# DanMcGann/loam

Measured on AMD Instinct MI355X. Metric: scan-pair registrations/sec (64x1024 Ouster), higher is better.
Workload: dtype f64; 1 GPU; batch of 1024 independent 64x1024 scan pairs per GPU (BASELINE configs[2]/[3]); step = extractFeatures x2 + registerFeatures per pair, inputs resident in HBM; pairs_per_gpu=1024, scan=64x1024, seed=20240311, input_scalar=f64, arithmetic=f64 (float input is widened on load)

## Files before the change

loam_amd/csrc/loamx_api.hip:

```cpp
#include <math.h>
#include <stdio.h>
#include <stdlib.h>
#include <string.h>

#include <mutex>
#include <utility>
#include <string>
#include <vector>

#include <dlfcn.h>
#include <rccl/rccl.h>

#include "loamx_internal.h"
#include "synth.h"

using namespace loamx;

namespace {

enum WsId {
  WS_XYZ = 0, WS_CURV, WS_MASK, WS_EDGE_STAGE, WS_PLANAR_STAGE, WS_EDGE_CNT, WS_PLANAR_CNT,
  WS_EDGE_IDX, WS_PLANAR_IDX, WS_N_EDGE, WS_N_PLANAR, WS_EDGE_XYZ, WS_PLANAR_XYZ,
  WS_GRID_DESC_E, WS_GRID_DESC_P, WS_CELLS_E, WS_CELLS_P, WS_SORTED_E, WS_SORTED_P, WS_REL_E, WS_REL_P,
  WS_SGRID_DESC_E, WS_SGRID_DESC_P, WS_SCELLS_E, WS_SCELLS_P, WS_SSORTED_E, WS_SSORTED_P, WS_SORT_SCRATCH, WS_SORT_SCRATCH_SRC, WS_ASSOC_E, WS_ASSOC_P, WS_NN_E, WS_NN_P, WS_RNN_E, WS_RNN_P, WS_NEAREST_E, WS_NEAREST_P, WS_REST_E, WS_REST_P, WS_EXACT_E, WS_EXACT_P, WS_NASSOC, WS_STATE, WS_PARTIALS, WS_MOM_PARTIALS, WS_MOMENTS, WS_FLAGGED_LIST, WS_FLAGGED_COUNT, WS_LINE_TOT, WS_EXTRACT_EVENTS, WS_BOX, WS_FINITE_FLAG,
  WS_COUNTERS, WS_ITERINFO, WS_STREAM_IN0, WS_STREAM_IN1, WS_STREAM_RES, WS_DUMP_E, WS_DUMP_P, WS_FIT_IN, WS_FIT_OUT, WS_SRC_E, WS_SRC_P, WS_TGT_E, WS_TGT_P, WS_FCOUNTS, WS_RESULTS, WS_INIT, WS_STREAM_INIT,
  WS_COUNT
};

struct Buf {
  void* p = nullptr;
  size_t cap = 0;
};

struct PendingEvent {
  int kernel;
  hipEvent_t e0, e1;
  double bytes;
  bool own_e0;
};

}

struct loamx_ctx {
  int device = 0;
  hipStream_t own_stream = nullptr, stream = nullptr;
  bool max_counts_clean = false;
  hipStream_t aux_stream = nullptr;
  hipEvent_t ev_fork = nullptr, ev_mid = nullptr, ev_join = nullptr;
  hipEvent_t ev_counts = nullptr;
  hipStream_t aux2_stream = nullptr;
  hipEvent_t ev_join2 = nullptr;
  std::string last_error;
  Buf ws[WS_COUNT];
  uint32_t* h_pinned = nullptr;
  bool timing = false;
  std::vector<PendingEvent> pending;
  std::vector<hipEvent_t> event_pool;
  hipEvent_t tail_event = nullptr;
  bool tail_fresh = false;
  loamx_kernel_stat stats[LOAMX_K_COUNT] = {};

  uint32_t extract_flags = 0;
  uint32_t reg_flags = 0;
  int map_cells_log2 = 0;
  int stream_chunk_pairs = 0;
  hipStream_t copy_stream = nullptr;
  hipEvent_t ev_up[2] = {nullptr, nullptr}, ev_free[2] = {nullptr, nullptr};

  uint32_t last_extract_route = 0;

  unsigned long long sweep_slots_base[2] = {0, 0};
  unsigned long long features_base = 0;
  std::mutex mu;
};

struct loamx_target_index {
  GridDesc* desc[2] = {nullptr, nullptr};
  uint32_t* cells[2] = {nullptr, nullptr};
  GridPoint* sorted[2] = {nullptr, nullptr};
  float* rel[2] = {nullptr, nullptr};
  double* pts[2] = {nullptr, nullptr};
  size_t n[2] = {0, 0};
  size_t cap[2] = {0, 0};
  double radius[2] = {0, 0};
  uint32_t* counts = nullptr;
  void* scratch = nullptr;
  uint32_t cells_cap[2] = {0, 0};
  size_t cells_alloc[2] = {0, 0}, scratch_alloc = 0;
  GridPoint* sorted2[2] = {nullptr, nullptr};
  float* rel2[2] = {nullptr, nullptr};
  size_t n_at_build[2] = {0, 0};
  bool grid_valid[2] = {false, false};
  uint64_t full_builds = 0, merges = 0;
};

namespace loamx {
thread_local LaunchScope* g_launch_scope = nullptr;
int g_debug_sync = getenv("LOAMX_DEBUG_SYNC") ? 1 : 0;
thread_local uint32_t g_extract_route = 0;
}

namespace {

const char* kKernelNames[LOAMX_K_COUNT] = {"curvature_valid_kernel", "select_kernel", "compact_kernel",
                                           "grid_build_kernel",      "associate_kernel", "sweep_kernel",
                                           "lm_kernels",             "moment_kernel",    "knn_plane_kernel",
                                           "extract_fused_kernel"};

struct OptionName {
  const char* name;
  bool extract;
  uint32_t bit;
};
const OptionName kOptionNames[] = {
    {"FORCE_TIE_REPLAY", true, kFlagForceReplay}, {"FORCE_SCAN_GIVEUP", true, kFlagForceGiveUp}, {"CURV_V1", true, kFlagCurvV1},
    {"NO_FUSED_COMPACT", true, kFlagNoFusedCompact}, {"NO_MIS_SELECT", true, kFlagNoMisSelect}, {"FUSED_EXTRACT", true, kFlagFusedExtract},
    {"NO_ROW_SELECT", true, kFlagNoRowSelect}, {"FUSED_ROWS", true, kFlagFusedRows}, {"NO_SPLIT_CURV", true, kFlagNoSplitCurv}, {"STAGE_ALWAYS", true, kFlagStageAlways},
    {"NO_MOMENTS", false, kRegFlagNoMoments}, {"NO_PACKED_GRID", false, kRegFlagNoPackedGrid}, {"NO_BIG_GRID", false, kRegFlagNoBigGrid},
    {"NO_GRID_SIDE", false, kRegFlagNoGridSide}, {"DEBUG_POISON", false, kRegFlagPoison},
    {"QUEUE_TWO_STAGE", false, kRegFlagQueueTwoStage}, {"QUEUE_ONE_STAGE", false, kRegFlagQueueOneStage},
    {"NO_MIXED_ASSOC", false, kRegFlagNoMixedAssoc}, {"FORCE_RCCL", false, kRegFlagForceRccl},
    {"NO_COOP_LEFT", false, kRegFlagNoCoopLeft}, {"NO_REF_MOMENTS", false, kRegFlagNoRefMoments},
    {"NO_EXTRACT_BOXES", false, kRegFlagNoExtractBoxes}, {"CHECK_FINITE", false, kRegFlagCheckFinite},
    {"NO_SMALL_SETS", false, kRegFlagNoSmallSets}};

int fail(loamx_ctx* ctx, int code, const std::string& msg) {
  if (ctx) ctx->last_error = msg;
  return code;
}

#define HIP_TRY(ctx, expr)                                                                          \
  do {                                                                                              \
    hipError_t e_ = (expr);                                                                         \
    if (e_ != hipSuccess)                                                                           \
      return fail(ctx, LOAMX_ERR_HIP, std::string(#expr) + ": " + hipGetErrorString(e_));           \
  } while (0)

int ensure(loamx_ctx* ctx, int id, size_t bytes) {
  Buf& b = ctx->ws[id];
  if (bytes == 0) bytes = 8;
  if (b.cap >= bytes) return LOAMX_OK;
  if (b.p) {
    HIP_TRY(ctx, hipStreamSynchronize(ctx->stream));
    HIP_TRY(ctx, hipFree(b.p));
    b.p = nullptr, b.cap = 0;
  }
  HIP_TRY(ctx, hipMalloc(&b.p, bytes));
  b.cap = bytes;
  return LOAMX_OK;
}
#define ENSURE(ctx, id, bytes)                       \
  do {                                               \
    int rc_ = ensure(ctx, id, bytes);                \
    if (rc_ != LOAMX_OK) return rc_;                 \
  } while (0)

const char* const kNonFiniteMsg = "non-finite coordinate in the input (the reference's behaviour is undefined there)";
bool host_all_finite(const void* p, bool f32, size_t n_scalars) {
  if (!p) return true;
  if (f32) {
    const float* v = static_cast<const float*>(p);
    float acc = 0.0f;
    for (size_t i = 0; i < n_scalars; i++) acc += v[i] * 0.0f;
    return acc == 0.0f;
  }
  const double* v = static_cast<const double*>(p);
  double acc = 0.0;
  for (size_t i = 0; i < n_scalars; i++) acc += v[i] * 0.0;
  return acc == 0.0;
}
template <typename T>
T* wsp(loamx_ctx* ctx, int id) {
  return reinterpret_cast<T*>(ctx->ws[id].p);
}

hipEvent_t take_event(loamx_ctx* ctx) {
  if (!ctx->event_pool.empty()) {
    hipEvent_t e = ctx->event_pool.back();
    ctx->event_pool.pop_back();
    return e;
  }
  hipEvent_t e = nullptr;
  (void)hipEventCreate(&e);
  return e;
}

struct TimedScope {
  loamx_ctx* ctx;
  PendingEvent pe;
  bool on, attach;
  LaunchScope ls;
  TimedScope(loamx_ctx* c, int kernel, double bytes, bool attach_ = false) : ctx(c), on(c->timing), attach(attach_) {
    if (on) {
      pe.kernel = kernel, pe.bytes = bytes;
      if (attach) {
        pe.own_e0 = true;
        pe.e0 = take_event(ctx), pe.e1 = take_event(ctx);
        ls = LaunchScope{pe.e0, pe.e1, true};
        g_launch_scope = &ls;
        return;
      }
      pe.own_e0 = !(ctx->tail_fresh && ctx->tail_event);
      pe.e0 = pe.own_e0 ? take_event(ctx) : ctx->tail_event;
      pe.e1 = take_event(ctx);
      if (pe.own_e0) (void)hipEventRecord(pe.e0, ctx->stream);
    }
  }
  ~TimedScope() {
    if (on) {
      if (attach) {
        g_launch_scope = nullptr;
        if (ls.first) {
          ctx->event_pool.push_back(pe.e0), ctx->event_pool.push_back(pe.e1);
        } else {
          ctx->pending.push_back(pe);
        }
        ctx->tail_fresh = false;
        return;
      }
      (void)hipEventRecord(pe.e1, ctx->stream);
      ctx->pending.push_back(pe);
      ctx->tail_event = pe.e1, ctx->tail_fresh = true;
    }
  }
};
inline void untimed(loamx_ctx* ctx) { ctx->tail_fresh = false; }

int finite_begin(loamx_ctx* ctx) {
  ENSURE(ctx, WS_FINITE_FLAG, 16);
  untimed(ctx);
  HIP_TRY(ctx, hipMemsetAsync(ctx->ws[WS_FINITE_FLAG].p, 0, 16, ctx->stream));
  return LOAMX_OK;
}
void finite_add(loamx_ctx* ctx, const void* d_pts, bool f32, const uint32_t* d_n, size_t n_sets, size_t stride, uint32_t pitch) {
  if (d_pts && n_sets && stride) launch_check_finite(d_pts, f32, d_n, n_sets, stride, pitch, static_cast<uint32_t*>(ctx->ws[WS_FINITE_FLAG].p), ctx->stream);
}
int finite_end(loamx_ctx* ctx) {
  uint32_t bad = 0;
  HIP_TRY(ctx, hipMemcpyAsync(&bad, ctx->ws[WS_FINITE_FLAG].p, 4, hipMemcpyDeviceToHost, ctx->stream));
  HIP_TRY(ctx, hipStreamSynchronize(ctx->stream));
  return bad ? fail(ctx, LOAMX_ERR_BAD_PARAM, kNonFiniteMsg) : LOAMX_OK;
}
int dev_check_finite(loamx_ctx* ctx, const void* d_pts, bool f32, const uint32_t* d_n, size_t n_sets, size_t stride, uint32_t pitch, bool force = false) {
  if ((!force && !(ctx->reg_flags & kRegFlagCheckFinite)) || !d_pts || n_sets == 0 || stride == 0) return LOAMX_OK;
  int rc = finite_begin(ctx);
  if (rc != LOAMX_OK) return rc;
  finite_add(ctx, d_pts, f32, d_n, n_sets, stride, pitch);
  return finite_end(ctx);
}


int check_launch(loamx_ctx* ctx, const char* what) {
  hipError_t e = hipGetLastError();
  if (e != hipSuccess) return fail(ctx, LOAMX_ERR_HIP, std::string(what) + ": " + hipGetErrorString(e));
  return LOAMX_OK;
}
#define CHECK_LAUNCH(ctx, what)                      \
  do {                                               \
    int rc_ = check_launch(ctx, what);               \
    if (rc_ != LOAMX_OK) return rc_;                 \
  } while (0)

int make_extract_params(loamx_ctx* ctx, const loamx_lidar_params* lidar, const loamx_fe_params* fe, ExtractParams& P) {
  if (!lidar || !fe) return fail(ctx, LOAMX_ERR_BAD_PARAM, "null parameter struct");
  if (fe->number_sectors == 0) return fail(ctx, LOAMX_ERR_BAD_PARAM, "number_sectors must be >= 1");
  if (fe->neighbor_points == 0)
    return fail(ctx, LOAMX_ERR_BAD_PARAM, "neighbor_points must be >= 1 (the reference reads point idx-1)");
  if (fe->neighbor_points > (uint64_t)kMaxNeighborPoints)
    return fail(ctx, LOAMX_ERR_UNSUPPORTED, "neighbor_points > 16 not supported by the kernels");
  if (lidar->points_per_line > (uint64_t)kMaxLineWidth)
    return fail(ctx, LOAMX_ERR_UNSUPPORTED, "points_per_line > 4096 not supported by the kernels");
  if (lidar->scan_lines * lidar->points_per_line > 0xFFFFFFFFull / 4)
// ... 131 lines not shown
  if (launch_extract_split_ok(P, n_scans)) Pk.flags |= kFlagSplitCurv, g_extract_route |= LOAMX_ROUTE_SPLIT_CURV;
  const bool split = (Pk.flags & kFlagSplitCurv) != 0u;
  {
    TimedScope t(ctx, LOAMX_K_CURVATURE, (double)n_scans * (double)N * ((f32 ? 21.0 : 33.0) - (split ? 1.0 : 0.0)), true);
    launch_curvature_valid(d_xyz, f32, n_scans, Pk, wsp<double>(ctx, WS_CURV), wsp<uint8_t>(ctx, WS_MASK), ctx->stream);
  }
  CHECK_LAUNCH(ctx, "curvature_valid_kernel");
  bool fused = false, rows_ran = false;
  {
    TimedScope t(ctx, LOAMX_K_SELECT, (double)n_scans * (double)N * (split ? 4.0 : 9.0), true);
    fused = launch_select(wsp<double>(ctx, WS_CURV), wsp<uint8_t>(ctx, WS_MASK), n_scans, Pk, st, &fz, ctx->stream, &rows_ran);
    launch_replay(wsp<double>(ctx, WS_CURV), wsp<uint8_t>(ctx, WS_MASK), n_scans, Pk, st, fz, ctx->stream);
    if (fused) {
      launch_compact(d_xyz, f32, n_scans, P, st, d_edge_idx, d_n_edge, d_edge_xyz, edge_capacity(P), d_planar_idx, d_n_planar,
                     d_planar_xyz, planar_capacity(P), ctx->stream, d_gave_up, d_events + 1);
      g_extract_route |= LOAMX_ROUTE_FUSED_COMPACT;
    }
  }
  CHECK_LAUNCH(ctx, "select_kernel");
  if (split && !rows_ran) return fail(ctx, LOAMX_ERR_UNSUPPORTED, "internal: split curvature form without the row selection");
  if (fused && rows_ran && boxes && fz.box_min)
    boxes->min = fz.box_min, boxes->max = fz.box_max, boxes->bad = d_gave_up, g_extract_route |= LOAMX_ROUTE_BOXES;
  if (fused) return LOAMX_OK;
  {
    TimedScope t(ctx, LOAMX_K_COMPACT, 0.0, true);
    launch_compact(d_xyz, f32, n_scans, P, st, d_edge_idx, d_n_edge, d_edge_xyz, edge_capacity(P), d_planar_idx,
                   d_n_planar, d_planar_xyz, planar_capacity(P), ctx->stream);
    g_extract_route |= LOAMX_ROUTE_COMPACT;
  }
  CHECK_LAUNCH(ctx, "compact_kernel");
  return LOAMX_OK;
}

struct RegInputs {
  size_t n_pairs, edge_stride, planar_stride;
  uint32_t in_pitch;
  const double *src_edge, *src_planar, *tgt_edge, *tgt_planar;
  const uint32_t *n_src_edge, *n_src_planar, *n_tgt_edge, *n_tgt_planar;
  const double* init;
  ExtractBoxes boxes;
  uint32_t src_box_offset;
};

typedef int (*AfterAssocHook)(loamx_ctx*, const RegBatch&, uint32_t it, void* user);

int enqueue_association(loamx_ctx* ctx, const RegBatch& B, const RegConfig& C, uint32_t what = kAssocEdges | kAssocPlanes) {
  hipStream_t s = ctx->stream;
    {
      TimedScope t(ctx, LOAMX_K_ASSOC, 0.0);
      const bool side = (size_t)B.n_pairs * B.assoc_blocks_plane >= 128;
      PendingEvent knn{};
      LaunchScope knn_ls{nullptr, nullptr, true};
      if (ctx->timing) {
        knn.kernel = LOAMX_K_KNN_PLANE, knn.bytes = 0.0, knn.own_e0 = true;
        knn.e0 = take_event(ctx), knn.e1 = take_event(ctx);
        knn_ls = LaunchScope{knn.e0, knn.e1, true};
      }
      launch_associate(B, C, s, side ? ctx->aux_stream : nullptr, side ? ctx->aux2_stream : nullptr, ctx->ev_fork, ctx->ev_mid, ctx->ev_join,
                       ctx->ev_join2, ctx->timing ? &knn_ls : nullptr, what);
      if (ctx->timing) {
        if (knn_ls.first) ctx->event_pool.push_back(knn.e0), ctx->event_pool.push_back(knn.e1);
        else ctx->pending.push_back(knn);
      }
    }
    CHECK_LAUNCH(ctx, "associate_kernel");
  return LOAMX_OK;
}

int enqueue_icf_iteration(loamx_ctx* ctx, const RegBatch& B, const RegConfig& C, uint32_t it, AfterAssocHook hook, void* hook_user) {
  hipStream_t s = ctx->stream;
    {
      const int rc_assoc = enqueue_association(ctx, B, C);
      if (rc_assoc != LOAMX_OK) return rc_assoc;
    }
#ifdef LOAMX_NN_SAME_STATS
    debug_nn_same(B, it, s);
#endif
    if (hook) {
      untimed(ctx);
      int rc = hook(ctx, B, it, hook_user);
      if (rc != LOAMX_OK) return rc;
    }
    {
      TimedScope t(ctx, LOAMX_K_LM, 0.0, true);
      launch_lm_begin(B, C, s);
    }
    const bool ref_first = it == 0 && B.ref_moments != 0u;
    if (ref_first) {
      {
        TimedScope t(ctx, LOAMX_K_SWEEP, 0.0, true);
        launch_sweep(B, s);
      }
      TimedScope t(ctx, LOAMX_K_LM, 0.0, true);
      launch_lm_step(B, s);
    }
    if (it > 0 || ref_first) {
      TimedScope t(ctx, LOAMX_K_MOMENT, 0.0, true);
      launch_moments(B, s);
    }
    if (it > 0 || ref_first) {
      TimedScope t(ctx, LOAMX_K_LM, 0.0, true);
      launch_lm_pair_loop(B, C, s);
    } else {
      for (int k = 0; k < 5; k++) {
        {
          TimedScope t(ctx, LOAMX_K_SWEEP, 0.0, true);
          launch_sweep(B, s);
        }
        {
          TimedScope t(ctx, LOAMX_K_LM, 0.0, true);
          launch_lm_step(B, s);
        }
      }
    }
    CHECK_LAUNCH(ctx, "sweep/lm kernels");
    if (it == 0 && !ref_first) {
      TimedScope t(ctx, LOAMX_K_LM, 0.0, true);
      launch_outer_update(B, C, s);
    }
    CHECK_LAUNCH(ctx, "outer_update_kernel");
  return LOAMX_OK;
}

int register_dev(loamx_ctx* ctx, const RegInputs& in, const RegConfig& C_in, loamx_reg_result* d_results, bool want_iter_info,
                 AfterAssocHook hook, void* hook_user, const loamx_target_index* prebuilt = nullptr, const loamx_assoc_dump* dump = nullptr,
                 size_t dump_n_se = 0, size_t dump_n_sp = 0) {
  if (in.n_pairs == 0) return LOAMX_OK;
  RegConfig C = C_in;
  if (dump && C.max_iterations == 0) C.max_iterations = 1;
  untimed(ctx);
  if (in.n_pairs > 0x7FFFFFFFull / 128) return fail(ctx, LOAMX_ERR_UNSUPPORTED, "too many pairs in one call");
  const size_t np = in.n_pairs, es = in.edge_stride ? in.edge_stride : 1, ps = in.planar_stride ? in.planar_stride : 1;
  if (es > 0x3FFFFFFFull || ps > 0x3FFFFFFFull) return fail(ctx, LOAMX_ERR_UNSUPPORTED, "feature set too large");
  RegBatch B{};
  B.n_pairs = np, B.edge_stride = es, B.planar_stride = ps, B.in_pitch = in.in_pitch;
  B.src_edge = in.src_edge, B.n_src_edge = in.n_src_edge, B.src_planar = in.src_planar, B.n_src_planar = in.n_src_planar;
  B.tgt_edge = in.tgt_edge, B.n_tgt_edge = in.n_tgt_edge, B.tgt_planar = in.tgt_planar, B.n_tgt_planar = in.n_tgt_planar;
  B.init = in.init;
  if (!(C.flags & kRegFlagNoExtractBoxes)) B.box_min = in.boxes.min, B.box_max = in.boxes.max, B.box_bad = in.boxes.bad, B.src_box_offset = in.src_box_offset;
  ENSURE(ctx, WS_GRID_DESC_E, np * sizeof(GridDesc));
  ENSURE(ctx, WS_GRID_DESC_P, np * sizeof(GridDesc));
  ENSURE(ctx, WS_CELLS_E, (np * (size_t)(kGridCellsCap + 1) + 4) * sizeof(uint32_t));
  ENSURE(ctx, WS_CELLS_P, (np * (size_t)(kGridCellsCap + 1) + 4) * sizeof(uint32_t));
  ENSURE(ctx, WS_SORTED_E, np * (es + kGridPad) * sizeof(GridPoint));
  ENSURE(ctx, WS_SORTED_P, np * (ps + kGridPad) * sizeof(GridPoint));
  ENSURE(ctx, WS_REL_E, np * 3 * (es + kGridPad) * sizeof(float));
  ENSURE(ctx, WS_REL_P, np * 3 * (ps + kGridPad) * sizeof(float));
  ENSURE(ctx, WS_SGRID_DESC_E, np * sizeof(GridDesc));
  ENSURE(ctx, WS_SGRID_DESC_P, np * sizeof(GridDesc));
  ENSURE(ctx, WS_SCELLS_E, np * (size_t)(kGridCellsCap + 1) * sizeof(uint32_t));
  ENSURE(ctx, WS_SCELLS_P, np * (size_t)(kGridCellsCap + 1) * sizeof(uint32_t));
  ENSURE(ctx, WS_SSORTED_E, np * es * sizeof(GridPoint));
  ENSURE(ctx, WS_SSORTED_P, np * ps * sizeof(GridPoint));
  ENSURE(ctx, WS_SORT_SCRATCH, np * (es > ps ? es : ps) * sizeof(GridPoint));
  ENSURE(ctx, WS_SORT_SCRATCH_SRC, grid_small(es > ps ? es : ps, C.flags) ? sizeof(GridPoint) : np * (es > ps ? es : ps) * sizeof(GridPoint));
  ENSURE(ctx, WS_ASSOC_E, 9 * np * es * sizeof(double));
  ENSURE(ctx, WS_ASSOC_P, 7 * np * ps * sizeof(double));
  const size_t km_e = C.k_edge <= 5 ? 5 : (C.k_edge <= 8 ? 8 : kMaxK), km_p = C.k_plane <= 5 ? 5 : (C.k_plane <= 8 ? 8 : kMaxK);
  ENSURE(ctx, WS_NN_E, (1 + km_e) * np * es * sizeof(uint32_t));
  ENSURE(ctx, WS_NN_P, (1 + km_p) * np * ps * sizeof(uint32_t));
  ENSURE(ctx, WS_RNN_E, (1 + km_e) * np * es * sizeof(uint32_t));
  ENSURE(ctx, WS_RNN_P, (1 + km_p) * np * ps * sizeof(uint32_t));
  ENSURE(ctx, WS_NEAREST_E, np * es * sizeof(uint32_t));
  ENSURE(ctx, WS_NEAREST_P, np * ps * sizeof(uint32_t));
  ENSURE(ctx, WS_REST_E, np * es * sizeof(uint32_t));
  ENSURE(ctx, WS_REST_P, np * ps * sizeof(uint32_t));
  ENSURE(ctx, WS_EXACT_E, np * es * sizeof(uint32_t));
  ENSURE(ctx, WS_EXACT_P, np * ps * sizeof(uint32_t));
  ENSURE(ctx, WS_NASSOC, np * 8 * sizeof(uint32_t));
  ENSURE(ctx, WS_STATE, np * sizeof(PairState));
  B.blocks_per_pair = (uint32_t)((es + ps + kSweepChunk - 1) / kSweepChunk);
  ENSURE(ctx, WS_PARTIALS, np * B.blocks_per_pair * kAccSize * sizeof(double));
  B.mom_blocks_per_pair = (uint32_t)((ps + kSweepChunk - 1) / kSweepChunk);
  ENSURE(ctx, WS_MOM_PARTIALS, np * B.mom_blocks_per_pair * 4 * (size_t)(kMomSize + 2) * sizeof(double));
  ENSURE(ctx, WS_MOMENTS, np * (size_t)(kMomSize + 2) * sizeof(double));
  ENSURE(ctx, WS_FLAGGED_LIST, np * (size_t)B.mom_blocks_per_pair * kSweepChunk * sizeof(uint32_t));
  ENSURE(ctx, WS_FLAGGED_COUNT, np * (size_t)B.mom_blocks_per_pair * 4 * sizeof(uint32_t));
  {
    const bool fresh = ctx->ws[WS_COUNTERS].cap == 0;
    ENSURE(ctx, WS_COUNTERS, 128);
    untimed(ctx);
    if (fresh) HIP_TRY(ctx, hipMemsetAsync(ctx->ws[WS_COUNTERS].p, 0, 128, ctx->stream));
  }
  if (C.flags & kRegFlagPoison) {
    static const int kScratch[] = {WS_GRID_DESC_E, WS_GRID_DESC_P, WS_CELLS_E, WS_CELLS_P, WS_SORTED_E, WS_SORTED_P, WS_REL_E, WS_REL_P,
                                   WS_SGRID_DESC_E, WS_SGRID_DESC_P, WS_SCELLS_E, WS_SCELLS_P, WS_SSORTED_E, WS_SSORTED_P, WS_SORT_SCRATCH, WS_SORT_SCRATCH_SRC,
                                   WS_ASSOC_E, WS_ASSOC_P, WS_NN_E, WS_NN_P, WS_RNN_E, WS_RNN_P, WS_NEAREST_E, WS_NEAREST_P, WS_REST_E,
                                   WS_REST_P, WS_EXACT_E, WS_EXACT_P, WS_NASSOC, WS_STATE, WS_PARTIALS, WS_MOM_PARTIALS, WS_MOMENTS,
                                   WS_FLAGGED_LIST, WS_FLAGGED_COUNT};
    for (int id : kScratch)
      if (ctx->ws[id].p) HIP_TRY(ctx, hipMemsetAsync(ctx->ws[id].p, 0xFF, ctx->ws[id].cap, ctx->stream));
  }
  if (want_iter_info) ENSURE(ctx, WS_ITERINFO, np * (size_t)(C.max_iterations ? C.max_iterations : 1) * sizeof(loamx_iter_info));
  B.grid_edge = GridSet{wsp<GridDesc>(ctx, WS_GRID_DESC_E), wsp<uint32_t>(ctx, WS_CELLS_E), wsp<GridPoint>(ctx, WS_SORTED_E), es + kGridPad,
                        wsp<float>(ctx, WS_REL_E)};
  B.grid_plane = GridSet{wsp<GridDesc>(ctx, WS_GRID_DESC_P), wsp<uint32_t>(ctx, WS_CELLS_P), wsp<GridPoint>(ctx, WS_SORTED_P), ps + kGridPad,
                         wsp<float>(ctx, WS_REL_P)};
  B.src_grid_edge = GridSet{wsp<GridDesc>(ctx, WS_SGRID_DESC_E), wsp<uint32_t>(ctx, WS_SCELLS_E), wsp<GridPoint>(ctx, WS_SSORTED_E), es, nullptr};
  B.src_grid_plane = GridSet{wsp<GridDesc>(ctx, WS_SGRID_DESC_P), wsp<uint32_t>(ctx, WS_SCELLS_P), wsp<GridPoint>(ctx, WS_SSORTED_P), ps, nullptr};
  B.sort_scratch = wsp<GridPoint>(ctx, WS_SORT_SCRATCH);
  B.sort_scratch_src = wsp<GridPoint>(ctx, WS_SORT_SCRATCH_SRC);
  B.assoc = AssocBuffers{wsp<double>(ctx, WS_ASSOC_E), wsp<double>(ctx, WS_ASSOC_P), wsp<uint32_t>(ctx, WS_NN_E),
                         wsp<uint32_t>(ctx, WS_NN_P), wsp<uint32_t>(ctx, WS_RNN_E), wsp<uint32_t>(ctx, WS_RNN_P),
                         wsp<uint32_t>(ctx, WS_NEAREST_E),
                         wsp<uint32_t>(ctx, WS_NEAREST_P), wsp<uint32_t>(ctx, WS_REST_E), wsp<uint32_t>(ctx, WS_REST_P),
                         wsp<uint32_t>(ctx, WS_EXACT_E), wsp<uint32_t>(ctx, WS_EXACT_P),
                         wsp<uint32_t>(ctx, WS_NASSOC)};
  B.state = wsp<PairState>(ctx, WS_STATE);
  B.partials = wsp<double>(ctx, WS_PARTIALS);
  B.mom_partials = wsp<double>(ctx, WS_MOM_PARTIALS);
  B.moments = wsp<double>(ctx, WS_MOMENTS);
  B.flagged_list = wsp<uint32_t>(ctx, WS_FLAGGED_LIST);
  B.flagged_count = wsp<uint32_t>(ctx, WS_FLAGGED_COUNT);
  B.n_active = wsp<uint32_t>(ctx, WS_COUNTERS);
  B.sweep_slots = reinterpret_cast<unsigned long long*>(wsp<unsigned char>(ctx, WS_COUNTERS) + 8);
  B.assoc_slots = B.sweep_slots + 2;
  B.grid_bytes = B.sweep_slots + 5;
  B.iter_info = want_iter_info ? wsp<loamx_iter_info>(ctx, WS_ITERINFO) : nullptr;
  B.want_nearest = hook ? 1u : 0u;
  B.ref_moments = (C.flags & (kRegFlagNoMoments | kRegFlagNoRefMoments)) ? 0u : 1u;
  B.max_counts = wsp<uint32_t>(ctx, WS_COUNTERS) + 16;
  B.assoc_blocks_edge = B.assoc_blocks_plane = 0xFFFFFFFFu;
  B.knn_mode_edge = B.knn_mode_plane = 0u;
  B.small_edge_sets = (C.flags & kRegFlagNoSmallSets) ? 0u : (!prebuilt ? 1u : (prebuilt->n[0] <= kBruteMax ? 2u : 0u));
  hipStream_t s = ctx->stream;
  untimed(ctx);
  if (!ctx->max_counts_clean) {
    const uint32_t init[6] = {0u, 0u, 0u, 0u, 0xFFFFFFFFu, 0xFFFFFFFFu};
    memcpy(&ctx->h_pinned[8], init, sizeof(init));
    HIP_TRY(ctx, hipMemcpyAsync(B.max_counts, &ctx->h_pinned[8], sizeof(init), hipMemcpyHostToDevice, s));
  }
  ctx->max_counts_clean = false;
  launch_state_init(B, C, s);
  CHECK_LAUNCH(ctx, "state_init_kernel");
  if (!ctx->ev_counts) HIP_TRY(ctx, hipEventCreateWithFlags(&ctx->ev_counts, hipEventDisableTiming));
  HIP_TRY(ctx, hipMemcpyAsync(&ctx->h_pinned[16], B.max_counts, 6 * sizeof(uint32_t), hipMemcpyDeviceToHost, s));
  HIP_TRY(ctx, hipEventRecord(ctx->ev_counts, s));

  if (prebuilt) {
    B.grid_edge = GridSet{prebuilt->desc[0], prebuilt->cells[0], prebuilt->sorted[0], prebuilt->cap[0] + kGridPad, prebuilt->rel[0], prebuilt->cells_cap[0]};
    B.grid_plane = GridSet{prebuilt->desc[1], prebuilt->cells[1], prebuilt->sorted[1], prebuilt->cap[1] + kGridPad, prebuilt->rel[1], prebuilt->cells_cap[1]};
  }
  {
    TimedScope t(ctx, LOAMX_K_GRID, 0.0);
    const bool side = !(C.flags & kRegFlagNoGridSide) && ctx->aux_stream && !prebuilt && hipStreamWaitEvent(ctx->aux_stream, ctx->ev_counts, 0) == hipSuccess;
    if (!prebuilt) launch_grid_build_targets(B, C, s);
    launch_grid_build_sources(B, C, side ? ctx->aux_stream : s);
    if (side && hipEventRecord(ctx->ev_join, ctx->aux_stream) == hipSuccess) (void)hipStreamWaitEvent(s, ctx->ev_join, 0);
  }
  CHECK_LAUNCH(ctx, "grid_build_kernel");
  HIP_TRY(ctx, hipEventSynchronize(ctx->ev_counts));
  B.assoc_blocks_edge = (ctx->h_pinned[16] + 255u) / 256u;
  B.assoc_blocks_plane = (ctx->h_pinned[17] + 255u) / 256u;
  {
    uint32_t tmax[2] = {ctx->h_pinned[18], ctx->h_pinned[19]}, tmin[2] = {ctx->h_pinned[20], ctx->h_pinned[21]};
    if (prebuilt) tmax[0] = tmin[0] = (uint32_t)prebuilt->n[0], tmax[1] = tmin[1] = (uint32_t)prebuilt->n[1];
    uint32_t* mode[2] = {&B.knn_mode_edge, &B.knn_mode_plane};
    for (int k = 0; k < 2; k++) *mode[k] = tmin[k] > tmax[k] ? 0u : (tmin[k] > kBruteMax ? 1u : (tmax[k] <= kBruteMax ? 2u : 0u));
  }
  if (dump) {
    if (np != 1) return fail(ctx, LOAMX_ERR_BAD_PARAM, "association dump: one pair at a time");
    int rc_a = enqueue_association(ctx, B, C);
    if (rc_a != LOAMX_OK) return rc_a;
    untimed(ctx);
    const size_t n[2] = {dump_n_se, dump_n_sp}, kq[2] = {(size_t)C.k_edge, (size_t)C.k_plane}, pw[2] = {6, 4};
    AssocDumpSet D[2] = {};
    for (int kind = 0; kind < 2; kind++) {
      const size_t bytes = n[kind] * (24 + 8 * pw[kind] + 4 + 4 * kq[kind] + 1) + 64;
      ENSURE(ctx, kind ? WS_DUMP_P : WS_DUMP_E, bytes);
      unsigned char* base = wsp<unsigned char>(ctx, kind ? WS_DUMP_P : WS_DUMP_E);
      HIP_TRY(ctx, hipMemsetAsync(base, 0, bytes, s));
      D[kind].moved = reinterpret_cast<double*>(base);
      D[kind].prim = D[kind].moved + 3 * n[kind];
      D[kind].nn_count = reinterpret_cast<uint32_t*>(D[kind].prim + pw[kind] * n[kind]);
      D[kind].nn_idx = D[kind].nn_count + n[kind];
      D[kind].valid = reinterpret_cast<uint8_t*>(D[kind].nn_idx + kq[kind] * n[kind]);
      if (n[kind] == 0) D[kind].nn_count = nullptr;
    }
    launch_assoc_dump(B, C, D[0], D[1], s);
    CHECK_LAUNCH(ctx, "assoc_dump_kernel");
    struct Out { void* host; const void* dev; size_t bytes; };
    const Out outs[10] = {
        {dump->edge_nn_count, D[0].nn_count, 4 * n[0]}, {dump->edge_nn_idx, D[0].nn_idx, 4 * kq[0] * n[0]}, {dump->edge_valid, D[0].valid, n[0]},
        {dump->edge_moved, D[0].moved, 24 * n[0]}, {dump->edge_lines, D[0].prim, 48 * n[0]},
        {dump->plane_nn_count, D[1].nn_count, 4 * n[1]}, {dump->plane_nn_idx, D[1].nn_idx, 4 * kq[1] * n[1]}, {dump->plane_valid, D[1].valid, n[1]},
        {dump->plane_moved, D[1].moved, 24 * n[1]}, {dump->plane_planes, D[1].prim, 32 * n[1]}};
    for (const Out& o : outs)
      if (o.host && o.bytes && o.dev) HIP_TRY(ctx, hipMemcpyAsync(o.host, o.dev, o.bytes, hipMemcpyDeviceToHost, s));
    if (dump->queue_lengths) HIP_TRY(ctx, hipMemcpyAsync(dump->queue_lengths, B.assoc.n_assoc + 2, 4 * sizeof(uint32_t), hipMemcpyDeviceToHost, s));
    HIP_TRY(ctx, hipStreamSynchronize(s));
    return LOAMX_OK;
  }
  for (uint32_t it = 0; it < C.max_iterations; it++) {
    {
      const int rc_body = enqueue_icf_iteration(ctx, B, C, it, hook, hook_user);
      if (rc_body != LOAMX_OK) return rc_body;
    }
    if (it + 1 < C.max_iterations && it > (B.n_pairs >= 256 ? 1u : 0u)) {
      untimed(ctx);
      HIP_TRY(ctx, hipMemcpyAsync(ctx->h_pinned, B.n_active, sizeof(uint32_t), hipMemcpyDeviceToHost, s));
      launch_write_results(B, d_results, s);
      CHECK_LAUNCH(ctx, "write_results_kernel");
      HIP_TRY(ctx, hipStreamSynchronize(s));
      if (ctx->h_pinned[0] == 0) {
        ctx->max_counts_clean = true;
        return LOAMX_OK;
      }
    }
  }
  untimed(ctx);
  launch_write_results(B, d_results, s);
  CHECK_LAUNCH(ctx, "write_results_kernel");
  ctx->max_counts_clean = true;
  return LOAMX_OK;
}

int resolve_events(loamx_ctx* ctx) {
  if (ctx->pending.empty()) return LOAMX_OK;
  HIP_TRY(ctx, hipStreamSynchronize(ctx->stream));
  for (PendingEvent& pe : ctx->pending) {
    float ms = 0.f;
    if (hipEventElapsedTime(&ms, pe.e0, pe.e1) == hipSuccess) {
      ctx->stats[pe.kernel].launches++;
      ctx->stats[pe.kernel].total_ms += (double)ms;
      ctx->stats[pe.kernel].algorithmic_bytes += pe.bytes;
    }
    if (pe.own_e0) ctx->event_pool.push_back(pe.e0);
    ctx->event_pool.push_back(pe.e1);
  }
  ctx->pending.clear();
  ctx->tail_fresh = false;
  return LOAMX_OK;
}

}

extern "C" {

void loamx_default_fe_params(loamx_fe_params* p) { *p = loamx_fe_params{3, 6, 10, 50, 100.0, 1.0, 0.5, 1.0}; }
void loamx_default_reg_params(loamx_reg_params* p) {
  *p = loamx_reg_params{5, 1.0, 3, 10.0, 5, 2.0, 4, 0.1, 10, 1e-3, 1e-2, 100};
}

const char* loamx_status_string(int status) {
  switch (status) {
    case LOAMX_OK: return "ok";
    case LOAMX_ERR_SCAN_SIZE: return "LOAM: provided lidar scan size does not match provided lidar parameters";
    case LOAMX_ERR_BAD_PARAM: return "bad parameter";
    case LOAMX_ERR_HIP: return "HIP error";
    case LOAMX_ERR_CAPACITY: return "output capacity too small";
    case LOAMX_ERR_UNSUPPORTED: return "unsupported parameter combination";
    case LOAMX_ERR_NO_DEVICE: return "no usable HIP device";
// ... 1329 lines not shown
```

loam_amd/csrc/loamx_internal.h:

```cpp
#pragma once
#include <hip/hip_runtime.h>
#include <hip/hip_ext.h>
#include <stdint.h>
#include <stdio.h>

#include "../../include/loamx.h"
#include "extract_math.h"
#include "reg_math.h"

namespace loamx {

struct LaunchScope {
  hipEvent_t start, stop;
  bool first;
};
extern thread_local LaunchScope* g_launch_scope;
extern int g_debug_sync;
template <typename F, typename... Args>
inline void launch_kernel_named(const char* name, F kernel, const dim3& grid, const dim3& block, size_t shmem, hipStream_t s, Args... args) {
  LaunchScope* sc = g_launch_scope;
  if (g_debug_sync) fprintf(stderr, "[loamx] launch %s grid %u x %u block %u\n", name, grid.x, grid.y, block.x), fflush(stderr);
  if (sc) {
    hipExtLaunchKernelGGL(kernel, grid, block, (uint32_t)shmem, s, sc->first ? sc->start : nullptr, sc->stop, 0, args...);
    sc->first = false;
  } else {
    hipLaunchKernelGGL(kernel, grid, block, shmem, s, args...);
  }
  if (g_debug_sync) {
    const hipError_t e = hipStreamSynchronize(s);
    fprintf(stderr, "[loamx]   done %s: %s\n", name, hipGetErrorString(e)), fflush(stderr);
  }
}
#define launch_kernel(kernel, ...) launch_kernel_named(#kernel, kernel, __VA_ARGS__)

constexpr int kMaxNeighborPoints = 16;
constexpr int kMaxLineWidth = 4096;

extern thread_local uint32_t g_extract_route;

struct ExtractStage {
  uint32_t* edge_stage;
  uint32_t* planar_stage;
  uint32_t* edge_cnt;
  uint32_t* planar_cnt;
};

struct ExtractFused {
  unsigned long long* line_tot;
  uint32_t fuse;
  const void* xyz;
  uint32_t f32;
  uint32_t* edge_idx;
  uint32_t* n_edge;
  double* edge_xyz;
  size_t edge_stride;
  uint32_t* planar_idx;
  uint32_t* n_planar;
  double* planar_xyz;
  size_t planar_stride;
  uint32_t* error;
  unsigned long long* events;
  unsigned long long* box_min;
  unsigned long long* box_max;
  uint32_t no_stage;
  const uint32_t* only_if;
};
__device__ __forceinline__ unsigned long long dbl_key(double v) {
  const unsigned long long u = (unsigned long long)__double_as_longlong(v);
  return (u >> 63) ? ~u : (u | 0x8000000000000000ull);
}
__device__ __forceinline__ double key_dbl(unsigned long long k) {
  return __longlong_as_double((long long)((k >> 63) ? (k & 0x7FFFFFFFFFFFFFFFull) : ~k));
}

void launch_curvature_valid(const void* d_xyz, bool f32, size_t n_scans, const ExtractParams& P, double* d_curv,
                            uint8_t* d_mask, hipStream_t s);
bool launch_select(const double* d_curv, const uint8_t* d_mask, size_t n_scans, const ExtractParams& P,
                   const ExtractStage& st, const ExtractFused* fz, hipStream_t s, bool* rows_ran = nullptr);
bool launch_select_takes_boxes(const ExtractParams& P);
bool launch_extract_fused(const void* d_xyz, bool f32, size_t n_scans, const ExtractParams& P, const ExtractStage& st,
                          const ExtractFused& fz, double* d_curv, uint8_t* d_mask, hipStream_t s);
bool launch_extract_rows_fused(const void* d_xyz, bool f32, size_t n_scans, const ExtractParams& P, const ExtractStage& st,
                               const ExtractFused& fz, double* d_curv, uint8_t* d_mask, hipStream_t s);
bool launch_extract_split_ok(const ExtractParams& P, size_t n_scans);
void launch_extract_init(unsigned long long* line_tot, size_t n_tot, unsigned long long* box_min, unsigned long long* box_max, size_t n_box,
                         hipStream_t s);
void launch_replay(const double* d_curv, const uint8_t* d_mask, size_t n_scans, const ExtractParams& P, const ExtractStage& st,
                   const ExtractFused& fz, hipStream_t s);
void launch_compact(const void* d_xyz, bool f32, size_t n_scans, const ExtractParams& P, const ExtractStage& st,
                    uint32_t* d_edge_idx, uint32_t* d_n_edge, double* d_edge_xyz, size_t edge_stride,
                    uint32_t* d_planar_idx, uint32_t* d_n_planar, double* d_planar_xyz, size_t planar_stride,
                    hipStream_t s, const uint32_t* only_if = nullptr, unsigned long long* fallback_counter = nullptr);

struct RegConfig {
  int k_edge, k_plane;
  int min_line_pts, min_plane_pts;
  double r_edge, r_plane;
  double pass_edge, pass_plane;
  double min_line_cond, max_avg_plane_dist;
  uint32_t max_iterations;
  double rot_thresh, pos_thresh;
  uint32_t min_associations;
  uint32_t flags;
};
constexpr uint32_t kRegFlagNoMoments = 1u;
constexpr uint32_t kRegFlagNoPackedGrid = 2u;
constexpr uint32_t kRegFlagNoBigGrid = 4u;
constexpr uint32_t kRegFlagNoGridSide = 8u;
constexpr uint32_t kRegFlagPoison = 16u;
constexpr uint32_t kRegFlagQueueTwoStage = 32u;
constexpr uint32_t kRegFlagQueueOneStage = 64u;
constexpr uint32_t kRegFlagForceRccl = 256u;
constexpr uint32_t kRegFlagNoCoopLeft = 512u;
constexpr uint32_t kRegFlagNoRefMoments = 1024u;
constexpr uint32_t kRegFlagNoSmallSets = 8192u;
constexpr uint32_t kRegFlagCheckFinite = 4096u;
constexpr uint32_t kRegFlagNoExtractBoxes = 2048u;
constexpr uint32_t kRegFlagNoMixedAssoc = 128u;

struct GridSet {
  GridDesc* desc;
  uint32_t* cell_start;
  GridPoint* sorted;
  size_t stride;
  float* rel;
  uint32_t cells_cap;
};

struct AssocBuffers {
  double* edge;
  double* plane;
  uint32_t* nn_edge;
  uint32_t* nn_plane;
  uint32_t* rnn_edge;
  uint32_t* rnn_plane;
  uint32_t* nearest_edge;
  uint32_t* nearest_plane;
  uint32_t* rest_edge;
  uint32_t* rest_plane;
  uint32_t* exact_edge;
  uint32_t* exact_plane;
  uint32_t* n_assoc;
};

struct PairState {
  double est[7];
  LmState lm;
  uint32_t active;
  uint32_t termination;
  uint32_t iterations;
  uint32_t first_sweep;
  uint32_t stream_planes;
  uint32_t use_moments;
  uint32_t mom_ref_on;
  double mom_ref[7];
};

constexpr int kSweepThreads = 256;
#ifndef LOAMX_SWEEP_ITEMS
#define LOAMX_SWEEP_ITEMS 16
#endif
constexpr int kSweepItems = LOAMX_SWEEP_ITEMS;
constexpr int kSweepChunk = kSweepThreads * kSweepItems;

struct RegBatch {
  size_t n_pairs;
  size_t edge_stride, planar_stride;
  uint32_t in_pitch;
  const double* src_edge;
  const uint32_t* n_src_edge;
  const double* src_planar;
  const uint32_t* n_src_planar;
  const double* tgt_edge;
  const uint32_t* n_tgt_edge;
  const double* tgt_planar;
  const uint32_t* n_tgt_planar;
  const double* init;
  GridSet grid_edge, grid_plane;
  GridSet src_grid_edge, src_grid_plane;
  GridPoint* sort_scratch;
  GridPoint* sort_scratch_src;
  AssocBuffers assoc;
  PairState* state;
  double* partials;
  double* mom_partials;
  double* moments;
  uint32_t mom_blocks_per_pair;
  uint32_t* flagged_list;
  uint32_t* flagged_count;
  uint32_t blocks_per_pair;
  uint32_t* n_active;
  unsigned long long* sweep_slots;
  unsigned long long* assoc_slots;
  unsigned long long* grid_bytes;
  loamx_iter_info* iter_info;
  uint32_t* max_counts;
  uint32_t knn_mode_edge, knn_mode_plane;
  uint32_t assoc_blocks_edge, assoc_blocks_plane;
  uint32_t want_nearest;
  uint32_t ref_moments;
  const unsigned long long* box_min;
  const unsigned long long* box_max;
  const uint32_t* box_bad;
  uint32_t src_box_offset;
  uint32_t small_edge_sets;
};

constexpr size_t kGridBigScratchBytes = 64 + ((size_t)kGridCellsCap + kGridCellsCap / 4096 + 8) * sizeof(uint32_t);
constexpr uint32_t kGridSmallCap = 20480;
constexpr uint32_t kBruteMax = 512;
constexpr uint32_t kGridMapCellsCap = 1u << 18;
inline bool grid_small(size_t stride, uint32_t reg_flags) { return stride <= kGridSmallCap && !(reg_flags & kRegFlagNoPackedGrid); }
void launch_grid_build_targets(const RegBatch& B, const RegConfig& C, hipStream_t s);
void launch_grid_build_sources(const RegBatch& B, const RegConfig& C, hipStream_t s);
void launch_grid_build_target(const RegBatch& B, const RegConfig& C, bool plane, hipStream_t s);
void launch_grid_build_source(const RegBatch& B, const RegConfig& C, bool plane, hipStream_t s);
void launch_state_init(const RegBatch& B, const RegConfig& C, hipStream_t s);
constexpr uint32_t kAssocEdges = 1u, kAssocPlanes = 2u;
void launch_associate(const RegBatch& B, const RegConfig& C, hipStream_t s, hipStream_t aux, hipStream_t aux2, hipEvent_t ev_fork,
                      hipEvent_t ev_mid, hipEvent_t ev_join, hipEvent_t ev_join2, LaunchScope* knn_scope = nullptr,
                      uint32_t what = kAssocEdges | kAssocPlanes);
#ifdef LOAMX_NN_SAME_STATS
void debug_nn_same(const RegBatch& B, uint32_t it, hipStream_t s);
#endif
void launch_lm_begin(const RegBatch& B, const RegConfig& C, hipStream_t s);
void launch_sweep(const RegBatch& B, hipStream_t s);
void launch_lm_pair_loop(const RegBatch& B, const RegConfig& C, hipStream_t s);
void launch_lm_step(const RegBatch& B, hipStream_t s);
void launch_moments(const RegBatch& B, hipStream_t s);
void launch_outer_update(const RegBatch& B, const RegConfig& C, hipStream_t s);
void launch_write_results(const RegBatch& B, loamx_reg_result* d_results, hipStream_t s);

size_t index_insert_ws_bytes(size_t cells, size_t n_add);
void launch_index_insert_count(const GridSet& gs, size_t cells, const double* d_add, uint32_t n_add, void* ws, hipStream_t s);
void launch_index_insert_merge(const GridSet& gs, size_t cells, uint32_t n_old, const double* d_add, uint32_t n_add, void* ws,
                               GridPoint* sorted2, float* rel2, hipStream_t s);

constexpr int kFitMaxK = 32;
struct AssocDumpSet {
  uint32_t* nn_count;
  uint32_t* nn_idx;
  uint8_t* valid;
  double* moved;
  double* prim;
};
void launch_fit_sets(bool plane, const double* d_pts, size_t n_sets, int k, double* d_prim, double* d_aux, hipStream_t s);
void launch_knn_queries(const GridSet& gs, const double* d_q, size_t n_q, int k, double max_dist, uint32_t* d_idx, uint32_t* d_count,
                        hipStream_t s);
void launch_assoc_dump(const RegBatch& B, const RegConfig& C, const AssocDumpSet& edge, const AssocDumpSet& plane, hipStream_t s);

void launch_check_finite(const void* d_pts, bool f32, const uint32_t* d_n, size_t n_sets, size_t stride, uint32_t pitch, uint32_t* d_flag,
                         hipStream_t s);
void launch_check_finite_scalars(const double* d_v, size_t n_scalars, uint32_t* d_flag, hipStream_t s);

void launch_deskew(const void* d_xyz, void* d_out, bool f32, size_t n_scans, uint32_t H, uint32_t W, const double* d_motion, double rho,
                   hipStream_t s);
void launch_trajectory(const loamx_reg_result* d_results, size_t n_pairs, const double origin[7], double* d_world_T_scan, hipStream_t s);

void launch_synth_pairs(uint64_t seed, uint64_t first_pair, size_t n_pairs, uint32_t H, uint32_t W, double sigma,
                        double* d_xyz, hipStream_t s);

}
```

loam_amd/csrc/register_kernels.hip:

```cpp
#include "loamx_internal.h"

namespace loamx {

namespace {

__device__ __forceinline__ double wave_min(double v) {
#pragma unroll
  for (int off = 32; off >= 1; off >>= 1) v = fmin(v, __shfl_xor(v, off));
  return v;
}
__device__ __forceinline__ double wave_max(double v) {
#pragma unroll
  for (int off = 32; off >= 1; off >>= 1) v = fmax(v, __shfl_xor(v, off));
  return v;
}

#ifndef LOAMX_BUILD_THREADS
#define LOAMX_BUILD_THREADS 1024
#endif
constexpr int kBuildThreads = LOAMX_BUILD_THREADS;

template <bool ORDERED, bool PACKED>
__global__ __launch_bounds__(kBuildThreads) void grid_build_kernel(const double* __restrict__ pts_base,
                                                                   const uint32_t* __restrict__ n_pts, size_t stride,
// ... 23 lines not shown
  const uint32_t n = n_raw < stride ? n_raw : (uint32_t)stride;
  const double* __restrict__ pts = pts_base + pair * in_pitch * stride * 3;
#ifdef LOAMX_BUILD_PROFILE
  unsigned long long stamp[12];
  int ns = 0;
#define STAMP() do { __syncthreads(); stamp[ns++] = wall_clock64(); } while (0)
#else
#define STAMP() do {} while (0)
#endif
  STAMP();

  const bool have_box = box_min != nullptr && __hip_atomic_load(box_bad, __ATOMIC_RELAXED, __HIP_MEMORY_SCOPE_AGENT) == 0u;
  if (!have_box) {
    double lx = kDblMax, ly = kDblMax, lz = kDblMax, hx = -kDblMax, hy = -kDblMax, hz = -kDblMax;
#pragma unroll 4
    for (uint32_t i = tid; i < n; i += kBuildThreads) {
      const double x = pts[3 * (size_t)i], y = pts[3 * (size_t)i + 1], z = pts[3 * (size_t)i + 2];
      lx = fmin(lx, x), ly = fmin(ly, y), lz = fmin(lz, z);
      hx = fmax(hx, x), hy = fmax(hy, y), hz = fmax(hz, z);
    }
    lx = wave_min(lx), ly = wave_min(ly), lz = wave_min(lz);
    hx = wave_max(hx), hy = wave_max(hy), hz = wave_max(hz);
    if (lane == 0) {
      s_red[0][wave] = lx, s_red[1][wave] = ly, s_red[2][wave] = lz;
      s_red[3][wave] = hx, s_red[4][wave] = hy, s_red[5][wave] = hz;
    }
  }
  STAMP();
  __syncthreads();
  if (tid == 0) {
    double a[6];
    if (have_box) {
      for (int k = 0; k < 3; k++) {
        a[k] = n ? key_dbl(box_min[(pair * in_pitch) * 6 + k]) : kDblMax;
        a[3 + k] = n ? key_dbl(box_max[(pair * in_pitch) * 6 + k]) : -kDblMax;
      }
    } else {
      for (int k = 0; k < 6; k++) {
        a[k] = s_red[k][0];
        for (int w = 1; w < kBuildThreads / 64; w++) a[k] = k < 3 ? fmin(a[k], s_red[k][w]) : fmax(a[k], s_red[k][w]);
      }
    }
    GridDesc g;
    if (ORDERED) grid_choose_morton(g, v3(a[0], a[1], a[2]), v3(a[3], a[4], a[5]), n);
    else grid_choose(g, v3(a[0], a[1], a[2]), v3(a[3], a[4], a[5]), n, max_dist, kGridCellsCap);
    s_g = g;
    gs.desc[pair] = g;
  }
  __syncthreads();
  const GridDesc g = s_g;
  STAMP();
  const uint32_t ncell = (uint32_t)(g.nx * g.ny * g.nz);
  uint32_t* __restrict__ cs = gs.cell_start + pair * (size_t)(kGridCellsCap + 1);
  GridPoint* __restrict__ sp = gs.sorted + pair * gs.stride;
  GridPoint* __restrict__ dst = ORDERED ? scratch + pair * gs.stride : sp;
  uint32_t carry = 0;
  if (PACKED) {
#pragma unroll 4
    for (uint32_t i = tid; i < n; i += kBuildThreads) {
      const Vec3 pt = v3(pts[3 * (size_t)i], pts[3 * (size_t)i + 1], pts[3 * (size_t)i + 2]);
      s_cellof[i] = (uint16_t)(ORDERED ? grid_morton_of_point(g, pt) : grid_cell_of_point(g, pt));
    }
  }
  for (uint32_t c_lo = 0; c_lo < ncell; c_lo += kGridLdsCells) {
    const uint32_t nc = ncell - c_lo < kGridLdsCells ? ncell - c_lo : kGridLdsCells;
    for (uint32_t c = tid; c < (PACKED ? (nc + 1) / 2 : nc); c += kBuildThreads) s_cells[c] = 0;
    __syncthreads();
    if (PACKED) {
      for (uint32_t i = tid; i < n; i += kBuildThreads) {
        const uint32_t cell = (uint32_t)s_cellof[i] - c_lo;
        if (cell < nc) (void)cell_add(cell);
      }
    } else {
#pragma unroll 4
      for (uint32_t i = tid; i < n; i += kBuildThreads) {
        const Vec3 pt = v3(pts[3 * (size_t)i], pts[3 * (size_t)i + 1], pts[3 * (size_t)i + 2]);
        const uint32_t cell = (ORDERED ? grid_morton_of_point(g, pt) : grid_cell_of_point(g, pt)) - c_lo;
        if (cell < nc) (void)cell_add(cell);
      }
    }
    __syncthreads();
    STAMP();
    const uint32_t per = PACKED ? 2u * (((nc + 2 * kBuildThreads - 1) / (2 * kBuildThreads)) | 1u) : ((nc + kBuildThreads - 1) / kBuildThreads) | 1u;
    const uint32_t c0 = tid * per < nc ? tid * per : nc, c1 = c0 + per < nc ? c0 + per : nc;
    uint32_t local = 0;
    if (PACKED) {
      for (uint32_t w = c0 >> 1; c0 < c1 && 2 * w < c1; w++) local += (s_cells[w] & 0xFFFFu) + (s_cells[w] >> 16);
    } else {
      for (uint32_t c = c0; c < c1; c++) local += s_cells[c];
    }
    uint32_t incl = local;
#pragma unroll
    for (int off = 1; off < 64; off <<= 1) {
      const uint32_t t = __shfl_up(incl, off);
      if (lane >= off) incl += t;
    }
    if (lane == 63) s_wave_sum[wave] = incl;
    __syncthreads();
    uint32_t wave_off = carry;
    for (int w = 0; w < wave; w++) wave_off += s_wave_sum[w];
    uint32_t pass_total = 0;
    for (int w = 0; w < kBuildThreads / 64; w++) pass_total += s_wave_sum[w];
    uint32_t run = wave_off + incl - local;
    if (PACKED) {
      for (uint32_t w = c0 >> 1; c0 < c1 && 2 * w < c1; w++) {
        const uint32_t v = s_cells[w], lo = v & 0xFFFFu, hi = v >> 16;
        s_cells[w] = run | ((run + lo) << 16);
        run += lo + hi;
      }
    } else {
      for (uint32_t c = c0; c < c1; c++) {
        const uint32_t cnt = s_cells[c];
        s_cells[c] = run;
        run += cnt;
      }
    }
    __syncthreads();
    STAMP();
    if (!(ORDERED && PACKED) && (ORDERED || n > kBruteMax))
      for (uint32_t c = tid; c < nc; c += kBuildThreads) cs[c_lo + c] = cell_get(c);
    __syncthreads();
    STAMP();
    if (PACKED) {
      for (uint32_t i = tid; i < n; i += kBuildThreads) {
        const uint32_t cell = (uint32_t)s_cellof[i] - c_lo;
        if (cell < nc) s_inv[cell_add(cell)] = (uint16_t)i;
      }
    } else {
#pragma unroll 4
      for (uint32_t i = tid; i < n; i += kBuildThreads) {
        const double x = pts[3 * (size_t)i], y = pts[3 * (size_t)i + 1], z = pts[3 * (size_t)i + 2];
        const uint32_t cell = (ORDERED ? grid_morton_of_point(g, v3(x, y, z)) : grid_cell_of_point(g, v3(x, y, z))) - c_lo;
        if (cell < nc) dst[cell_add(cell)] = GridPoint{x, y, z, i, 0u};
      }
    }
    carry += pass_total;
    __syncthreads();
    STAMP();
  }
  if (tid == 0) cs[ncell] = n;
  if (tid == 0 && bytes)
    atomicAdd(bytes, (unsigned long long)n * (ORDERED ? 56ull : (gs.rel ? 68ull : 56ull)) +
                         ((!(ORDERED && PACKED) && (ORDERED || n > kBruteMax)) ? 4ull * (ncell + 1) : 0ull));
  if (PACKED && ORDERED) {
#pragma unroll 2
    for (uint32_t p = tid; p < n; p += kBuildThreads) {
      const uint32_t i = s_inv[p];
      const uint32_t cell = s_cellof[i];
      const uint32_t b = cell ? cell_get(cell - 1) : 0u, en = cell_get(cell);
      const double x = pts[3 * (size_t)i], y = pts[3 * (size_t)i + 1], z = pts[3 * (size_t)i + 2];
      uint32_t rank = 0;
      for (uint32_t j = b; j < en; j++) rank += s_inv[j] < i ? 1u : 0u;
      sp[b + rank] = GridPoint{x, y, z, i, 0u};
    }
  } else if (PACKED) {
    const uint16_t* order = s_inv;
    STAMP();
    float* __restrict__ rel = gs.rel ? gs.rel + pair * 3 * gs.stride : nullptr;
#pragma unroll 4
    for (uint32_t p = tid; p < n; p += kBuildThreads) {
      const uint32_t i = order[p];
      const double x = pts[3 * (size_t)i], y = pts[3 * (size_t)i + 1], z = pts[3 * (size_t)i + 2];
      sp[p] = GridPoint{x, y, z, i, 0u};
      if (!ORDERED && rel) rel[p] = (float)(x - g.ox), rel[gs.stride + p] = (float)(y - g.oy), rel[2 * gs.stride + p] = (float)(z - g.oz);
    }
    if (!ORDERED && rel && (uint32_t)tid < kGridPad) rel[n + tid] = kRelPad, rel[gs.stride + n + tid] = kRelPad, rel[2 * gs.stride + n + tid] = kRelPad;
  } else if (!ORDERED && gs.rel) {
    __syncthreads();
    __threadfence_block();
    float* __restrict__ rel = gs.rel + pair * 3 * gs.stride;
    for (uint32_t p = tid; p < n; p += kBuildThreads) {
      const GridPoint e = sp[p];
      rel[p] = (float)(e.x - g.ox), rel[gs.stride + p] = (float)(e.y - g.oy), rel[2 * gs.stride + p] = (float)(e.z - g.oz);
    }
    if ((uint32_t)tid < kGridPad) rel[n + tid] = kRelPad, rel[gs.stride + n + tid] = kRelPad, rel[2 * gs.stride + n + tid] = kRelPad;
  }
#ifdef LOAMX_BUILD_PROFILE
  STAMP();
  if (tid == 0 && pair == 700 && n > 2000 && ns >= 8)
    printf("build ORDERED=%d n=%u ncell=%u ns=%d: bbox %llu choice %llu count %llu scan %llu table %llu scatter %llu rank %llu out %llu (x10 ns)\n", (int)ORDERED, n, ncell, ns,
           stamp[1] - stamp[0], stamp[2] - stamp[1], stamp[3] - stamp[2], stamp[4] - stamp[3], stamp[5] - stamp[4], stamp[6] - stamp[5], stamp[ns - 2] - stamp[ns - 3], stamp[ns - 1] - stamp[ns - 2]);
#endif
#undef STAMP
}

constexpr int kSmallThreads = 256;
__global__ __launch_bounds__(kSmallThreads) void small_sets_build_kernel(const double* __restrict__ tgt_base, const uint32_t* __restrict__ n_tgt,
                                                                         const double* __restrict__ src_base, const uint32_t* __restrict__ n_src,
                                                                         size_t stride, uint32_t in_pitch, double max_dist, GridSet tgt_gs, GridSet src_gs,
                                                                         unsigned long long* __restrict__ bytes, const unsigned long long* __restrict__ box_min,
                                                                         const unsigned long long* __restrict__ box_max, const uint32_t* __restrict__ box_bad) {
  __shared__ double s_red[6][kSmallThreads / 64];
  __shared__ GridDesc s_g;
  const int tid = threadIdx.x, lane = tid & 63, wave = tid >> 6;
  const size_t pair = blockIdx.x;
  if (n_tgt == nullptr) {
    const uint32_t ns_raw = n_src[pair * in_pitch];
    const uint32_t ns = ns_raw < stride ? ns_raw : (uint32_t)stride;
    const double* __restrict__ qp = src_base + pair * in_pitch * stride * 3;
    GridPoint* __restrict__ ssp = src_gs.sorted + pair * src_gs.stride;
    for (uint32_t i = tid; i < ns; i += kSmallThreads) ssp[i] = GridPoint{qp[3 * (size_t)i], qp[3 * (size_t)i + 1], qp[3 * (size_t)i + 2], i, 0u};
    if (tid == 0 && bytes) atomicAdd(bytes, (unsigned long long)ns * 56ull);
    return;
  }
  const uint32_t nt_raw = n_tgt[pair * in_pitch];
  if (nt_raw > kBruteMax) return;
  const uint32_t nt = nt_raw < stride ? nt_raw : (uint32_t)stride;
  const double* __restrict__ tp = tgt_base + pair * in_pitch * stride * 3;
  const bool have_box = box_min != nullptr && __hip_atomic_load(box_bad, __ATOMIC_RELAXED, __HIP_MEMORY_SCOPE_AGENT) == 0u;
  if (!have_box) {
    double lx = kDblMax, ly = kDblMax, lz = kDblMax, hx = -kDblMax, hy = -kDblMax, hz = -kDblMax;
    for (uint32_t i = tid; i < nt; i += kSmallThreads) {
      const double x = tp[3 * (size_t)i], y = tp[3 * (size_t)i + 1], z = tp[3 * (size_t)i + 2];
      lx = fmin(lx, x), ly = fmin(ly, y), lz = fmin(lz, z);
      hx = fmax(hx, x), hy = fmax(hy, y), hz = fmax(hz, z);
    }
    lx = wave_min(lx), ly = wave_min(ly), lz = wave_min(lz);
    hx = wave_max(hx), hy = wave_max(hy), hz = wave_max(hz);
    if (lane == 0) {
      s_red[0][wave] = lx, s_red[1][wave] = ly, s_red[2][wave] = lz;
      s_red[3][wave] = hx, s_red[4][wave] = hy, s_red[5][wave] = hz;
    }
  }
  __syncthreads();
  if (tid == 0) {
    double a[6];
    if (have_box) {
      for (int k = 0; k < 3; k++) {
        a[k] = nt ? key_dbl(box_min[(pair * in_pitch) * 6 + k]) : kDblMax;
        a[3 + k] = nt ? key_dbl(box_max[(pair * in_pitch) * 6 + k]) : -kDblMax;
      }
    } else {
      for (int k = 0; k < 6; k++) {
        a[k] = s_red[k][0];
        for (int w = 1; w < kSmallThreads / 64; w++) a[k] = k < 3 ? fmin(a[k], s_red[k][w]) : fmax(a[k], s_red[k][w]);
      }
    }
    GridDesc g;
    grid_choose(g, v3(a[0], a[1], a[2]), v3(a[3], a[4], a[5]), nt, max_dist, kGridCellsCap);
    s_g = g;
    tgt_gs.desc[pair] = g;
  }
  __syncthreads();
  const GridDesc g = s_g;
  GridPoint* __restrict__ sp = tgt_gs.sorted + pair * tgt_gs.stride;
  float* __restrict__ rel = tgt_gs.rel ? tgt_gs.rel + pair * 3 * tgt_gs.stride : nullptr;
  for (uint32_t p = tid; p < nt; p += kSmallThreads) {
    const double x = tp[3 * (size_t)p], y = tp[3 * (size_t)p + 1], z = tp[3 * (size_t)p + 2];
    sp[p] = GridPoint{x, y, z, p, 0u};
    if (rel) rel[p] = (float)(x - g.ox), rel[tgt_gs.stride + p] = (float)(y - g.oy), rel[2 * tgt_gs.stride + p] = (float)(z - g.oz);
  }
  if (rel && (uint32_t)tid < kGridPad) rel[nt + tid] = kRelPad, rel[tgt_gs.stride + nt + tid] = kRelPad, rel[2 * tgt_gs.stride + nt + tid] = kRelPad;
  const uint32_t ns_raw = n_src[pair * in_pitch];
  const uint32_t ns = ns_raw < stride ? ns_raw : (uint32_t)stride;
  const double* __restrict__ qp = src_base + pair * in_pitch * stride * 3;
  GridPoint* __restrict__ ssp = src_gs.sorted + pair * src_gs.stride;
  for (uint32_t i = tid; i < ns; i += kSmallThreads) ssp[i] = GridPoint{qp[3 * (size_t)i], qp[3 * (size_t)i + 1], qp[3 * (size_t)i + 2], i, 0u};
  if (tid == 0 && bytes) atomicAdd(bytes, (unsigned long long)nt * (rel ? 68ull : 56ull) + (unsigned long long)ns * 56ull);
}

constexpr int kBigThreads = 256, kBigItems = 16, kBigChunk = kBigThreads * kBigItems;
constexpr size_t kBigScratchBytes = kGridBigScratchBytes;

__device__ __forceinline__ unsigned char* big_scratch(GridPoint* scratch, size_t pair, size_t stride) {
  return reinterpret_cast<unsigned char*>(scratch + pair * stride);
}

__global__ void gridbig_init_kernel(GridPoint* scratch, size_t stride) {
  unsigned long long* box = reinterpret_cast<unsigned long long*>(big_scratch(scratch, blockIdx.x, stride));
  if (threadIdx.x < 6) box[threadIdx.x] = threadIdx.x < 3 ? ~0ull : 0ull;
}

__global__ __launch_bounds__(kBigThreads) void gridbig_bbox_kernel(const double* __restrict__ pts_base, const uint32_t* __restrict__ n_pts,
                                                                   size_t stride, uint32_t in_pitch, GridPoint* scratch) {
  const size_t pair = blockIdx.y;
  const uint32_t n_raw = n_pts[pair * in_pitch], n = n_raw < stride ? n_raw : (uint32_t)stride;
  const uint32_t base = blockIdx.x * kBigChunk;
  if (base >= n) return;
  const double* __restrict__ pts = pts_base + pair * in_pitch * stride * 3;
  double lx = kDblMax, ly = kDblMax, lz = kDblMax, hx = -kDblMax, hy = -kDblMax, hz = -kDblMax;
#pragma unroll 4
  for (int k = 0; k < kBigItems; k++) {
    const uint32_t i = base + k * kBigThreads + threadIdx.x;
    if (i < n) {
      const double x = pts[3 * (size_t)i], y = pts[3 * (size_t)i + 1], z = pts[3 * (size_t)i + 2];
      lx = fmin(lx, x), ly = fmin(ly, y), lz = fmin(lz, z);
      hx = fmax(hx, x), hy = fmax(hy, y), hz = fmax(hz, z);
    }
  }
  lx = wave_min(lx), ly = wave_min(ly), lz = wave_min(lz);
  hx = wave_max(hx), hy = wave_max(hy), hz = wave_max(hz);
  if ((threadIdx.x & 63) == 0) {
    unsigned long long* box = reinterpret_cast<unsigned long long*>(big_scratch(scratch, pair, stride));
    atomicMin(&box[0], dbl_key(lx)), atomicMin(&box[1], dbl_key(ly)), atomicMin(&box[2], dbl_key(lz));
    atomicMax(&box[3], dbl_key(hx)), atomicMax(&box[4], dbl_key(hy)), atomicMax(&box[5], dbl_key(hz));
  }
}

__global__ void gridbig_choose_kernel(const uint32_t* __restrict__ n_pts, size_t stride, uint32_t in_pitch, double max_dist,
                                      GridSet gs, GridPoint* scratch, size_t n_pairs) {
  const size_t pair = (size_t)blockIdx.x * blockDim.x + threadIdx.x;
  if (pair >= n_pairs) return;
  const uint32_t n_raw = n_pts[pair * in_pitch], n = n_raw < stride ? n_raw : (uint32_t)stride;
  const unsigned long long* box = reinterpret_cast<const unsigned long long*>(big_scratch(scratch, pair, stride));
  GridDesc g;
  grid_choose(g, v3(key_dbl(box[0]), key_dbl(box[1]), key_dbl(box[2])), v3(key_dbl(box[3]), key_dbl(box[4]), key_dbl(box[5])), n, max_dist,
// ... 93 lines not shown
  uint32_t cnt[kScanPer], local = 0;
#pragma unroll
  for (uint32_t u = 0; u < kScanPer; u++) cnt[u] = c0 + u < ncell ? cs[c0 + u] : 0u, local += cnt[u];
  const uint32_t tile_base = blockIdx.x * kScanTile < ncell ? big_tile_sums(scratch, pair, stride, gs)[blockIdx.x] : n;
  uint32_t run = tile_base + block_incl_scan_256(local, s_wave, nullptr) - local;
#pragma unroll
  for (uint32_t u = 0; u < kScanPer; u++) {
    const uint32_t c = c0 + u;
    if (c < ncell) cs[c] = run, cursor[c] = run;
    else if (c == ncell) cs[c] = n;
    run += cnt[u];
  }
}

__global__ __launch_bounds__(kBigThreads) void gridbig_rel_kernel(const uint32_t* __restrict__ n_pts, size_t stride, uint32_t in_pitch,
                                                                  GridSet gs) {
  const size_t pair = blockIdx.y;
  const uint32_t n_raw = n_pts[pair * in_pitch], n = n_raw < stride ? n_raw : (uint32_t)stride;
  const uint32_t p = blockIdx.x * kBigThreads + threadIdx.x;
  float* __restrict__ rel = gs.rel + pair * 3 * gs.stride;
  if (p >= n) {
    if (p < n + kGridPad) rel[p] = kRelPad, rel[gs.stride + p] = kRelPad, rel[2 * gs.stride + p] = kRelPad;
    return;
  }
  const GridDesc g = gs.desc[pair];
  const GridPoint e = gs.sorted[pair * gs.stride + p];
  rel[p] = (float)(e.x - g.ox), rel[gs.stride + p] = (float)(e.y - g.oy), rel[2 * gs.stride + p] = (float)(e.z - g.oz);
}

__global__ __launch_bounds__(256) void index_insert_count_kernel(const double* __restrict__ add, uint32_t n_add, const GridDesc* __restrict__ desc,
                                                                 uint32_t* __restrict__ flag, uint32_t* __restrict__ add_count,
                                                                 uint32_t* __restrict__ cell_of) {
  const uint32_t i = blockIdx.x * 256 + threadIdx.x;
  if (i >= n_add) return;
  const GridDesc g = *desc;
  const Vec3 p = v3(add[3 * (size_t)i], add[3 * (size_t)i + 1], add[3 * (size_t)i + 2]);
  const int32_t cx = grid_cell_coord(p.x, g.ox, g.inv_h), cy = grid_cell_coord(p.y, g.oy, g.inv_h), cz = grid_cell_coord(p.z, g.oz, g.inv_h);
  const bool inside = cx >= 0 && cx < g.nx && cy >= 0 && cy < g.ny && cz >= 0 && cz < g.nz && p.x - p.x == 0.0 && p.y - p.y == 0.0 && p.z - p.z == 0.0;
  if (!inside) {
    atomicOr(flag, 1u);
    cell_of[i] = 0u;
    return;
  }
  const uint32_t cell = (uint32_t)((cz * g.ny + cy) * g.nx + cx);
  cell_of[i] = cell;
  atomicAdd(&add_count[cell], 1u);
}

__global__ __launch_bounds__(kScanThreads) void index_insert_tile_sum_kernel(const GridDesc* __restrict__ desc, const uint32_t* __restrict__ shift,
                                                                             uint32_t* __restrict__ tile_sum) {
  __shared__ uint32_t s_wave[kScanThreads / 64];
  const uint32_t ncell = (uint32_t)(desc->nx * desc->ny * desc->nz);
  const uint32_t c0 = blockIdx.x * kScanTile + threadIdx.x * kScanPer;
  uint32_t local = 0;
#pragma unroll
  for (uint32_t u = 0; u < kScanPer; u++)
    if (c0 + u < ncell) local += shift[c0 + u];
  uint32_t total = 0;
  (void)block_incl_scan_256(local, s_wave, &total);
  if (threadIdx.x == 0) tile_sum[blockIdx.x] = total;
}
__global__ __launch_bounds__(kScanThreads) void index_insert_tile_scan_kernel(uint32_t* __restrict__ tile_sum, uint32_t n_tiles) {
  __shared__ uint32_t s_wave[kScanThreads / 64];
  uint32_t carry = 0;
  for (uint32_t t0 = 0; t0 < n_tiles; t0 += kScanThreads) {
    const uint32_t t = t0 + threadIdx.x;
    const uint32_t v = t < n_tiles ? tile_sum[t] : 0u;
    uint32_t total = 0;
    const uint32_t incl = block_incl_scan_256(v, s_wave, &total);
    if (t < n_tiles) tile_sum[t] = carry + incl - v;
    carry += total;
  }
}
__global__ __launch_bounds__(kScanThreads) void index_insert_scan_kernel(const GridDesc* __restrict__ desc, const uint32_t* __restrict__ cell_start,
                                                                         const uint32_t* __restrict__ tile_sum, uint32_t* __restrict__ shift,
                                                                         uint32_t* __restrict__ cursor) {
  __shared__ uint32_t s_wave[kScanThreads / 64];
  const uint32_t ncell = (uint32_t)(desc->nx * desc->ny * desc->nz);
  const uint32_t c0 = blockIdx.x * kScanTile + threadIdx.x * kScanPer;
  uint32_t cnt[kScanPer], local = 0;
#pragma unroll
  for (uint32_t u = 0; u < kScanPer; u++) cnt[u] = c0 + u < ncell ? shift[c0 + u] : 0u, local += cnt[u];
  uint32_t run = tile_sum[blockIdx.x] + block_incl_scan_256(local, s_wave, nullptr) - local;
#pragma unroll
  for (uint32_t u = 0; u < kScanPer; u++) {
    const uint32_t c = c0 + u;
    if (c < ncell) {
      shift[c] = run;
      cursor[c] = cell_start[c + 1] + run;
    } else if (c == ncell) {
      shift[c] = run;
    }
    run += cnt[u];
  }
}

__global__ __launch_bounds__(256) void index_insert_move_kernel(const GridDesc* __restrict__ desc, uint32_t n_old, size_t stride,
                                                                const GridPoint* __restrict__ sorted, const float* __restrict__ rel,
                                                                const uint32_t* __restrict__ shift, GridPoint* __restrict__ sorted2,
                                                                float* __restrict__ rel2) {
  const uint32_t p = blockIdx.x * 256 + threadIdx.x;
  if (p >= n_old) return;
  const GridDesc g = *desc;
  const GridPoint e = sorted[p];
  const uint32_t np = p + shift[grid_cell_of_point(g, v3(e.x, e.y, e.z))];
  sorted2[np] = e;
  rel2[np] = rel[p], rel2[stride + np] = rel[stride + p], rel2[2 * stride + np] = rel[2 * stride + p];
}

__global__ __launch_bounds__(256) void index_insert_scatter_kernel(const double* __restrict__ add, uint32_t n_add, uint32_t first_index,
                                                                   const GridDesc* __restrict__ desc, size_t stride,
                                                                   const uint32_t* __restrict__ cell_of, uint32_t* __restrict__ cursor,
                                                                   GridPoint* __restrict__ sorted2, float* __restrict__ rel2) {
  const uint32_t i = blockIdx.x * 256 + threadIdx.x;
  if (i >= n_add) return;
  const GridDesc g = *desc;
  const double x = add[3 * (size_t)i], y = add[3 * (size_t)i + 1], z = add[3 * (size_t)i + 2];
  const uint32_t pos = atomicAdd(&cursor[cell_of[i]], 1u);
  sorted2[pos] = GridPoint{x, y, z, first_index + i, 0u};
  rel2[pos] = (float)(x - g.ox), rel2[stride + pos] = (float)(y - g.oy), rel2[2 * stride + pos] = (float)(z - g.oz);
}

__global__ __launch_bounds__(256) void index_insert_table_kernel(GridDesc* __restrict__ desc, uint32_t* __restrict__ cell_start,
                                                                 const uint32_t* __restrict__ shift, uint32_t n_new, size_t stride,
                                                                 float* __restrict__ rel2) {
  const uint32_t ncell = (uint32_t)(desc->nx * desc->ny * desc->nz);
  const uint32_t c = blockIdx.x * 256 + threadIdx.x;
  if (c <= ncell) cell_start[c] += shift[c];
  if (c < kGridPad) rel2[n_new + c] = kRelPad, rel2[stride + n_new + c] = kRelPad, rel2[2 * stride + n_new + c] = kRelPad;
  if (c == 0) desc->n_points = n_new;
}

constexpr int kRankThreads = 256;
__global__ __launch_bounds__(kRankThreads) void grid_rank_kernel(const uint32_t* __restrict__ n_pts, size_t stride,
                                                                 uint32_t in_pitch, GridSet gs,
                                                                 const GridPoint* __restrict__ scratch, const uint32_t* __restrict__ small_if) {
  const size_t pair = blockIdx.y;
  if (small_if && small_if[pair * in_pitch] <= kBruteMax) return;
  const uint32_t n_raw = n_pts[pair * in_pitch];
  const uint32_t n = n_raw < stride ? n_raw : (uint32_t)stride;
  const uint32_t p = blockIdx.x * kRankThreads + threadIdx.x;
  if (p >= n) return;
  const GridDesc g = gs.desc[pair];
  const uint32_t* __restrict__ cs = gs.cell_start + pair * (size_t)(kGridCellsCap + 1);
  const GridPoint* __restrict__ src = scratch + pair * gs.stride;
  GridPoint* __restrict__ sp = gs.sorted + pair * gs.stride;
  const GridPoint e = src[p];
  const uint32_t cell = grid_morton_of_point(g, v3(e.x, e.y, e.z));
  const uint32_t b = cs[cell], en = cs[cell + 1];
  uint32_t rank = 0;
#pragma unroll 4
  for (uint32_t j = b; j < en; j++) rank += src[j].orig < e.orig ? 1u : 0u;
  sp[b + rank] = e;
}

__global__ void state_init_kernel(RegBatch B, RegConfig C) {
  const size_t pair = (size_t)blockIdx.x * blockDim.x + threadIdx.x;
  if (pair >= B.n_pairs) return;
  PairState& S = B.state[pair];
  for (int i = 0; i < 7; i++) S.est[i] = B.init ? B.init[pair * 7 + i] : (i == 3 ? 1.0 : 0.0);
  S.active = C.max_iterations > 0 ? 1u : 0u;
  S.termination = LOAMX_MAX_ITER;
  S.iterations = 0;
  S.first_sweep = 0;
  S.stream_planes = 1;
  S.use_moments = 0;
  S.mom_ref_on = 0;
  S.lm.active = 0;
  for (int c = 0; c < 6; c++) B.assoc.n_assoc[8 * pair + c] = 0;
  if (B.max_counts) {
    const uint32_t ne = B.n_src_edge[pair * B.in_pitch], np = B.n_src_planar[pair * B.in_pitch];
    atomicMax(&B.max_counts[0], ne < B.edge_stride ? ne : (uint32_t)B.edge_stride);
    atomicMax(&B.max_counts[1], np < B.planar_stride ? np : (uint32_t)B.planar_stride);
    if (B.n_tgt_edge && B.n_tgt_planar) {
      uint32_t te = B.n_tgt_edge[pair * B.in_pitch], tp = B.n_tgt_planar[pair * B.in_pitch];
      te = te < B.edge_stride ? te : (uint32_t)B.edge_stride, tp = tp < B.planar_stride ? tp : (uint32_t)B.planar_stride;
      atomicMax(&B.max_counts[2], te), atomicMax(&B.max_counts[3], tp);
      atomicMin(&B.max_counts[4], te), atomicMin(&B.max_counts[5], tp);
    }
  }
}

constexpr int kAssocThreads = 256;
#ifndef LOAMX_ASSOC_WAVES
#define LOAMX_ASSOC_WAVES 4
#endif
#ifndef LOAMX_KNN_REQUERY
#define LOAMX_KNN_REQUERY 1
#endif
#ifndef LOAMX_ASSOC_WAVES5
#define LOAMX_ASSOC_WAVES5 (LOAMX_KNN_REQUERY ? 6 : 4)
#endif

__device__ __forceinline__ bool xcd_pair_map(uint32_t block, uint32_t blocks_per_pair, size_t n_pairs, size_t& pair,
                                             uint32_t& chunk) {
  if (n_pairs < 8) {
    pair = block / blocks_per_pair;
    chunk = block % blocks_per_pair;
  } else {
    const uint32_t xcd = block & 7u, slot = block >> 3;
    pair = (size_t)xcd + 8u * (size_t)(slot / blocks_per_pair);
    chunk = slot % blocks_per_pair;
  }
  return pair < n_pairs;
}

constexpr int kBruteTile = 256;
constexpr size_t kBruteLdsBytes = (kBruteTile + kGridPad) * sizeof(GridPoint) + ((3 * (kBruteTile + kGridPad) * sizeof(float) + 31) / 32) * 32;

template <class Coll>
__device__ __forceinline__ void brute_scan_tile(Coll& c, int k, Vec3 q, const GridPoint* s_tile, uint32_t tile, uint32_t tn) {
  for (uint32_t u = 0; u < tn; u += 4) {
    const GridPoint t0 = s_tile[u], t1 = s_tile[u + 1], t2 = s_tile[u + 2], t3 = s_tile[u + 3];
    double dx = q.x - t0.x, dy = q.y - t0.y, dz = q.z - t0.z;
    const double d0 = dx * dx + dy * dy + dz * dz;
    dx = q.x - t1.x, dy = q.y - t1.y, dz = q.z - t1.z;
    const double d1 = dx * dx + dy * dy + dz * dz;
    dx = q.x - t2.x, dy = q.y - t2.y, dz = q.z - t2.z;
    const double d2 = dx * dx + dy * dy + dz * dz;
    dx = q.x - t3.x, dy = q.y - t3.y, dz = q.z - t3.z;
    const double d3 = dx * dx + dy * dy + dz * dz;
    knn_offer4(c, k, d0, d1, d2, d3, tile + u, tn - u, t0.orig, t1.orig, t2.orig, t3.orig);
  }
}

template <bool PLANE, int KM>
__device__ __forceinline__ void knn_brute_body(const RegBatch& B, const RegConfig& C, uint32_t blocks_per_pair, uint32_t block,
                                               GridPoint* s_tile) {
  size_t pair;
  uint32_t chunk;
  if (!xcd_pair_map(block, blocks_per_pair, B.n_pairs, pair, chunk)) return;
  const PairState& S = B.state[pair];
  if (!S.active) return;
  const GridSet& gs = PLANE ? B.grid_plane : B.grid_edge;
  const uint32_t n_tgt = gs.desc[pair].n_points;
  if (n_tgt > kBruteMax) return;
  const size_t stride = PLANE ? B.planar_stride : B.edge_stride;
  const uint32_t n_src = PLANE ? B.n_src_planar[pair * B.in_pitch] : B.n_src_edge[pair * B.in_pitch];
  if ((PLANE ? B.knn_mode_plane : B.knn_mode_edge) == 2u && chunk == 0 && threadIdx.x == 0 && B.assoc_slots)
    atomicAdd(&B.assoc_slots[PLANE ? 1 : 0], (unsigned long long)(n_src < stride ? n_src : stride));
  if (chunk * kAssocThreads >= n_src || chunk * kAssocThreads >= stride) return;
  const uint32_t i = chunk * kAssocThreads + threadIdx.x;
  const bool has = i < n_src && i < stride;
  const GridSet& src_gs = PLANE ? B.src_grid_plane : B.src_grid_edge;
  const GridPoint* __restrict__ sp = gs.sorted + pair * gs.stride;
  Vec3 p = v3(0, 0, 0);
  if (has) {
    const GridPoint sq = src_gs.sorted[pair * src_gs.stride + i];
    p = pose_act(S.est, v3(sq.x, sq.y, sq.z));
  }
  int k = PLANE ? C.k_plane : C.k_edge;
  k = k < KM ? k : KM;
  const double max_dist = PLANE ? C.r_plane : C.r_edge;
  uint32_t pos[KM];
#pragma unroll
  for (int j = 0; j < KM; j++) pos[j] = 0;
  int kept = 0;
  if (k > 0 && n_tgt > 0) {
    const double pass_max = PLANE ? C.pass_plane : C.pass_edge;
    kept = has ? -1 : 0;
    const GridDesc g = gs.desc[pair];
    if (gs.rel != nullptr && g.h > 0.0) {
      float* s_f = reinterpret_cast<float*>(s_tile + kBruteTile + kGridPad);
      constexpr int kRow = kBruteTile + kGridPad;
      const float* __restrict__ rel = gs.rel + pair * 3 * gs.stride;
      const double a = knn_f32_err_unit(g);
      const bool inside = has && grid_outside_distance(g, grid_cell_coord(p.x, g.ox, g.inv_h), grid_cell_coord(p.y, g.oy, g.inv_h),
                                                       grid_cell_coord(p.z, g.oz, g.inv_h)) <= 1;
      const float qx = (float)(p.x - g.ox), qy = (float)(p.y - g.oy), qz = (float)(p.z - g.oz);
      constexpr uint32_t imask = 0x1FFu;
      static_assert(kBruteMax <= 512, "nine position bits");
      KnnKeys32<KM> c;
      knn_init(c, k);
      for (uint32_t tile = 0; tile < n_tgt; tile += kBruteTile) {
        const uint32_t tn = n_tgt - tile < (uint32_t)kBruteTile ? n_tgt - tile : (uint32_t)kBruteTile;
        __syncthreads();
        for (uint32_t t = threadIdx.x; t < tn + kGridPad; t += kAssocThreads) {
          s_f[t] = rel[tile + t], s_f[kRow + t] = rel[gs.stride + tile + t], s_f[2 * kRow + t] = rel[2 * gs.stride + tile + t];
        }
        __syncthreads();
        if (inside)
          for (uint32_t u = 0; u < tn; u += 4)
            knn_collect_batch_f32<KM>(c, qx, qy, qz, *reinterpret_cast<const KnnF4*>(s_f + u), *reinterpret_cast<const KnnF4*>(s_f + kRow + u),
                                      *reinterpret_cast<const KnnF4*>(s_f + 2 * kRow + u), tn - u, tile + u, ~imask);
      }
      if (inside) {
        int count = 0, kk = 0;
        bool undecided = false, open = true;
        double prev = -1.0, d5 = 0.0;
        GridPoint tp[KM];
#pragma unroll
        for (int j = 0; j < KM; j++) {
          const uint32_t pp = c.key[j] & imask;
          pos[j] = j >= KM - k && c.key[j] != 0xFFFFFFFFu ? pp : 0u;
          tp[j] = sp[pp < n_tgt ? pp : 0u];
        }
#pragma unroll
        for (int j = 0; j < KM; j++) {
          const uint32_t key = c.key[j];
          if (j >= KM - k && key != 0xFFFFFFFFu) {
            if (key >= 0x7F800000u) undecided = true;
            const double dx = p.x - tp[j].x, dy = p.y - tp[j].y, dz = p.z - tp[j].z;
            const double d2 = dx * dx + dy * dy + dz * dz;
            if (!(d2 > prev) || !(d2 <= kDblMax)) undecided = true;
            prev = d2, d5 = d2;
            count++;
            if (open) {
              if (d2 <= pass_max) kk++;
              else open = false;
            }
          }
        }
        const uint32_t k6 = c.key[KM];
        if (count == k && k6 != 0xFFFFFFFFu) {
          const double t6 = (double)knn_bits_f32(k6 & ~imask);
          const double err = 2.0 * (3.4641016151377544 * a * sqrt(d5) + 3.0 * a * a + 2.384185791015625e-7 * d5);
          if (!(t6 > d5 + err)) undecided = true;
        }
        if (!undecided) kept = kk;
      }
    }
    if (__syncthreads_or(kept < 0)) {
      KnnKeys<KM> c;
      knn_init(c, k, n_tgt);
      for (uint32_t tile = 0; tile < n_tgt; tile += kBruteTile) {
        const uint32_t tn = n_tgt - tile < (uint32_t)kBruteTile ? n_tgt - tile : (uint32_t)kBruteTile;
        __syncthreads();
        for (uint32_t t = threadIdx.x; t < tn + kGridPad; t += kAssocThreads) s_tile[t] = sp[tile + t];
        __syncthreads();
        if (kept < 0) brute_scan_tile(c, k, p, s_tile, tile, tn);
      }
      if (kept < 0) kept = knn_keys_finish(c, k, pass_max, pos);
    }
    if (__syncthreads_or(kept < 0)) {
      KnnResult<KM> r;
      knn_init(r);
      for (uint32_t tile = 0; tile < n_tgt; tile += kBruteTile) {
        const uint32_t tn = n_tgt - tile < (uint32_t)kBruteTile ? n_tgt - tile : (uint32_t)kBruteTile;
        __syncthreads();
        for (uint32_t t = threadIdx.x; t < tn + kGridPad; t += kAssocThreads) s_tile[t] = sp[tile + t];
        __syncthreads();
        if (kept < 0) brute_scan_tile(r, k, p, s_tile, tile, tn);
      }
      if (kept < 0) {
        kept = knn_finish(r, k, max_dist);
        knn_shift_positions<KM>(r.pos, k, pos);
      }
    }
  }
  if (!has) return;
  const size_t field = B.n_pairs * stride, slot = pair * stride + i;
  uint32_t* __restrict__ nn = PLANE ? B.assoc.nn_plane : B.assoc.nn_edge;
  nn[slot] = (uint32_t)kept;
#pragma unroll
  for (int j = 0; j < KM; j++) nn[(1 + j) * field + slot] = pos[j];
}
template <bool PLANE, int KM>
__global__ __launch_bounds__(kAssocThreads) void associate_knn_brute_kernel(RegBatch B, RegConfig C, uint32_t blocks_per_pair) {
  __shared__ GridPoint s_tile[kBruteLdsBytes / sizeof(GridPoint)];
  knn_brute_body<PLANE, KM>(B, C, blocks_per_pair, blockIdx.x, s_tile);
}

constexpr uint32_t kQueueIndex = 0x3FFFFFFFu, kQueueWide = 0x80000000u, kQueueTied = 0x40000000u;

template <bool PLANE, int KM>
__device__ __forceinline__ void knn_round1_body(const RegBatch& B, const RegConfig& C, uint32_t blocks_per_pair, uint32_t block,
                                                uint32_t* s_rows) {
  size_t pair;
  uint32_t chunk;
  if (!xcd_pair_map(block, blocks_per_pair, B.n_pairs, pair, chunk)) return;
  const uint32_t i = chunk * kAssocThreads + threadIdx.x;
  const PairState& S = B.state[pair];
  if (!S.active) return;
  const size_t stride = PLANE ? B.planar_stride : B.edge_stride;
  const uint32_t n_src = PLANE ? B.n_src_planar[pair * B.in_pitch] : B.n_src_edge[pair * B.in_pitch];
  const GridSet& gs = PLANE ? B.grid_plane : B.grid_edge;
  const GridSet& src_gs = PLANE ? B.src_grid_plane : B.src_grid_edge;
  if (chunk == 0 && threadIdx.x == 0 && B.assoc_slots)
    atomicAdd(&B.assoc_slots[PLANE ? 1 : 0], (unsigned long long)(n_src < stride ? n_src : stride));
  const GridDesc g = gs.desc[pair];
  if (g.n_points <= kBruteMax) return;
  if (i >= n_src || i >= stride) return;
  const GridPoint sq = src_gs.sorted[pair * src_gs.stride + i];
  const Vec3 p = pose_act(S.est, v3(sq.x, sq.y, sq.z));
  const uint32_t* __restrict__ cs = gs.cell_start + pair * (size_t)(kGridCellsCap + 1);
  const GridPoint* __restrict__ sp = gs.sorted + pair * gs.stride;
  uint32_t pos[KM];
  const float* __restrict__ rel = gs.rel + pair * 3 * gs.stride;
#if LOAMX_KNN_REQUERY
  const GridPoint* __restrict__ src_pts = src_gs.sorted + pair * src_gs.stride;
  auto requery = [&](const Vec3&) -> Vec3 {
    uint32_t ii = i;
    asm volatile("" : "+v"(ii));
    const GridPoint s2 = src_pts[ii];
    return pose_act(S.est, v3(s2.x, s2.y, s2.z));
  };
  const int kept = knn_search_f32_round1<KM, false, decltype(requery)>(g, cs, sp, rel, (uint32_t)gs.stride, p, PLANE ? C.k_plane : C.k_edge,
                                             PLANE ? C.r_plane : C.r_edge, PLANE ? C.pass_plane : C.pass_edge, pos,
                                             s_rows + threadIdx.x, kAssocThreads, requery);
#else
  const int kept = knn_search_f32_round1<KM>(g, cs, sp, rel, (uint32_t)gs.stride, p, PLANE ? C.k_plane : C.k_edge,
                                             PLANE ? C.r_plane : C.r_edge, PLANE ? C.pass_plane : C.pass_edge, pos,
                                             s_rows + threadIdx.x, kAssocThreads);
#endif
  const size_t field = B.n_pairs * stride, slot = pair * stride + i;
  uint32_t* __restrict__ nn = PLANE ? B.assoc.nn_plane : B.assoc.nn_edge;
  nn[slot] = kept < 0 ? 0xFFFFFFFFu : (uint32_t)kept;
  if (kept < 0) {
    const uint32_t at = atomicAdd(&B.assoc.n_assoc[8 * pair + (PLANE ? 3 : 2)], 1u);
    (PLANE ? B.assoc.rest_plane : B.assoc.rest_edge)[pair * stride + at] = i | (kept == -2 ? kQueueWide : kept == -3 ? kQueueTied : 0u);
  }
#pragma unroll
  for (int j = 0; j < KM; j++) nn[(1 + j) * field + slot] = pos[j];
}
template <bool PLANE, int KM>
__global__ __launch_bounds__(kAssocThreads, KM <= 5 ? LOAMX_ASSOC_WAVES5 : LOAMX_ASSOC_WAVES) void associate_knn_kernel(RegBatch B, RegConfig C,
                                                                                         uint32_t blocks_per_pair) {
  __shared__ uint32_t s_rows[kLeanRowWords * kAssocThreads];
  knn_round1_body<PLANE, KM>(B, C, blocks_per_pair, blockIdx.x, s_rows);
}
template <int KME, int KMP>
__global__ __launch_bounds__(kAssocThreads, (KME <= 5 && KMP <= 5) ? LOAMX_ASSOC_WAVES5 : LOAMX_ASSOC_WAVES) void associate_knn_mixed_kernel(RegBatch B, RegConfig C, uint32_t blocks_edge,
                                                                                               uint32_t blocks_plane, uint32_t edge_blocks) {
  constexpr size_t kRowBytes = sizeof(uint32_t) * kLeanRowWords * kAssocThreads, kTileBytes = kBruteLdsBytes;
  __shared__ __attribute__((aligned(16))) unsigned char s_raw[kRowBytes > kTileBytes ? kRowBytes : kTileBytes];
  if (blockIdx.x < edge_blocks) knn_brute_body<false, KME>(B, C, blocks_edge, blockIdx.x, reinterpret_cast<GridPoint*>(s_raw));
  else knn_round1_body<true, KMP>(B, C, blocks_plane, blockIdx.x - edge_blocks, reinterpret_cast<uint32_t*>(s_raw));
}

#ifndef LOAMX_REST_THREADS
#define LOAMX_REST_THREADS 64
#endif
constexpr int kRestThreads = LOAMX_REST_THREADS;
__host__ __device__ inline bool queue_leftovers_coop(const RegConfig& C, bool plane) {
  return !(C.flags & kRegFlagNoCoopLeft) && (plane ? C.r_plane : C.r_edge) > 0.0;
}
#ifndef LOAMX_COOP_WAVES
#define LOAMX_COOP_WAVES 4
#endif
#ifndef LOAMX_REST_WAVES
#define LOAMX_REST_WAVES(KM) ((KM) <= 8 ? 3 : 2)
#endif
template <bool PLANE, int KM, bool ONE_STAGE>
__global__ __launch_bounds__(kRestThreads, LOAMX_REST_WAVES(KM)) void associate_knn_rest_kernel(RegBatch B, RegConfig C,
                                                                                              uint32_t blocks_per_pair) {
  constexpr bool one_stage = ONE_STAGE;
  size_t pair;
  uint32_t chunk0;
  if (!xcd_pair_map(blockIdx.x, blocks_per_pair, B.n_pairs, pair, chunk0)) return;
  const PairState& S = B.state[pair];
  if (!S.active) return;
  const uint32_t queued = B.assoc.n_assoc[8 * pair + (PLANE ? 3 : 2)];
  if (queued == 0u) return;
  __shared__ uint32_t s_rows[(ONE_STAGE ? kLeanRowWords : kLean2RowWords) * kRestThreads];
  const size_t stride = PLANE ? B.planar_stride : B.edge_stride;
  const size_t field = B.n_pairs * stride;
  uint32_t* __restrict__ rnn = PLANE ? B.assoc.rnn_plane : B.assoc.rnn_edge;
  const uint32_t* __restrict__ rest = (PLANE ? B.assoc.rest_plane : B.assoc.rest_edge) + pair * stride;
  uint32_t* __restrict__ left = (PLANE ? B.assoc.exact_plane : B.assoc.exact_edge) + pair * stride;
  const GridSet& gs = PLANE ? B.grid_plane : B.grid_edge;
  const GridSet& src_gs = PLANE ? B.src_grid_plane : B.src_grid_edge;
  const GridDesc g = gs.desc[pair];
  const uint32_t* __restrict__ cs = gs.cell_start + pair * (size_t)(kGridCellsCap + 1);
  const GridPoint* __restrict__ sp = gs.sorted + pair * gs.stride;
  const bool spread = B.n_pairs < 8 && (size_t)queued * 4 <= (size_t)blocks_per_pair * kRestThreads;
  const uint32_t t0 = spread ? chunk0 + blocks_per_pair * threadIdx.x : chunk0 * kRestThreads + threadIdx.x;
  const uint32_t dt = spread ? 0xFFFFFFFFu - t0 : blocks_per_pair * kRestThreads;
  const bool lean_set = g.n_points <= kLeanMaxPoints;
  const int kq = PLANE ? C.k_plane : C.k_edge;
  const double max_dist = PLANE ? C.r_plane : C.r_edge, pass_max = PLANE ? C.pass_plane : C.pass_edge;
  for (uint32_t t = t0; t < queued; t += dt) {
    const uint32_t entry = rest[t], i = entry & kQueueIndex;
    const size_t slot = pair * stride + t;
    uint32_t pos[KM];
#pragma unroll
    for (int j = 0; j < KM; j++) pos[j] = 0;
    int kept = -1;
    const bool coop = !one_stage && queue_leftovers_coop(C, PLANE);
    if (one_stage || (!(entry & kQueueTied) && ((lean_set && !(entry & kQueueWide)) || ((entry & kQueueWide) && !coop)))) {
      const GridPoint sq = src_gs.sorted[pair * src_gs.stride + i];
      const Vec3 p = pose_act(S.est, v3(sq.x, sq.y, sq.z));
      if (entry & kQueueWide)
        kept = knn_search_f32_round1<KM, true>(g, cs, sp, gs.rel + pair * 3 * gs.stride, (uint32_t)gs.stride, p, kq, max_dist, pass_max, pos,
                                                s_rows + threadIdx.x, kRestThreads);
      else if (!one_stage)
        kept = knn_lean_round2<KM>(g, cs, sp, gs.rel + pair * 3 * gs.stride, (uint32_t)gs.stride, p, kq, max_dist, pass_max, pos,
                                   s_rows + threadIdx.x, kRestThreads);
      if (one_stage && kept < 0)
        kept = knn_search_keyed<KM>(g, cs, sp, p, kq, max_dist, pass_max, pos, s_rows + threadIdx.x, kRestThreads);
    }
    rnn[slot] = (uint32_t)kept;
    if (kept < 0) left[atomicAdd(&B.assoc.n_assoc[8 * pair + (PLANE ? 5 : 4)], 1u)] = t;
#pragma unroll
    for (int j = 0; j < KM; j++) rnn[(1 + j) * field + slot] = pos[j];
  }
}

template <bool PLANE, int KM>
__global__ __launch_bounds__(kRestThreads, 5) void associate_knn_left_kernel(RegBatch B, RegConfig C,
                                                                                              uint32_t blocks_per_pair) {
  size_t pair;
  uint32_t chunk0;
  if (!xcd_pair_map(blockIdx.x, blocks_per_pair, B.n_pairs, pair, chunk0)) return;
  const PairState& S = B.state[pair];
  if (!S.active) return;
  const uint32_t listed = B.assoc.n_assoc[8 * pair + (PLANE ? 5 : 4)];
  if (listed == 0u) return;
  __shared__ uint32_t s_rows[kLeanRowWords * kRestThreads];
  const size_t stride = PLANE ? B.planar_stride : B.edge_stride;
  const size_t field = B.n_pairs * stride;
  uint32_t* __restrict__ rnn = PLANE ? B.assoc.rnn_plane : B.assoc.rnn_edge;
  const uint32_t* __restrict__ rest = (PLANE ? B.assoc.rest_plane : B.assoc.rest_edge) + pair * stride;
  const uint32_t* __restrict__ left = (PLANE ? B.assoc.exact_plane : B.assoc.exact_edge) + pair * stride;
  const GridSet& gs = PLANE ? B.grid_plane : B.grid_edge;
  const GridSet& src_gs = PLANE ? B.src_grid_plane : B.src_grid_edge;
  const GridDesc g = gs.desc[pair];
  const uint32_t* __restrict__ cs = gs.cell_start + pair * (size_t)(kGridCellsCap + 1);
  const GridPoint* __restrict__ sp = gs.sorted + pair * gs.stride;
  const bool spread = B.n_pairs < 8 && (size_t)listed * 4 <= (size_t)blocks_per_pair * kRestThreads;
  const uint32_t t0 = spread ? chunk0 + blocks_per_pair * threadIdx.x : chunk0 * kRestThreads + threadIdx.x;
  const uint32_t dt = spread ? 0xFFFFFFFFu - t0 : blocks_per_pair * kRestThreads;
  for (uint32_t t = t0; t < listed; t += dt) {
    const uint32_t qpos = left[t], i = rest[qpos] & kQueueIndex;
    const size_t slot = pair * stride + qpos;
    const GridPoint sq = src_gs.sorted[pair * src_gs.stride + i];
    const Vec3 p = pose_act(S.est, v3(sq.x, sq.y, sq.z));
    uint32_t pos[KM];
    const int kept = knn_search_keyed<KM>(g, cs, sp, p, PLANE ? C.k_plane : C.k_edge, PLANE ? C.r_plane : C.r_edge,
                                          PLANE ? C.pass_plane : C.pass_edge, pos, s_rows + threadIdx.x, kRestThreads);
    rnn[slot] = (uint32_t)kept;
#pragma unroll
    for (int j = 0; j < KM; j++) rnn[(1 + j) * field + slot] = pos[j];
  }
}

constexpr int32_t kCoopMaxShell = 64;

__device__ __forceinline__ double wave_min_all(double v) {
#pragma unroll
  for (int off = 32; off >= 1; off >>= 1) {
    const double o = __shfl_xor(v, off);
    v = knn_key_min(v, o);
  }
  return v;
}

template <int KM>
__device__ __forceinline__ int knn_coop_search(const GridDesc& g, const uint32_t* __restrict__ cell_start, const GridPoint* __restrict__ sp,
                                               Vec3 q, int k, double max_dist, double pass_max, uint32_t pos[KM]) {
  const int lane = threadIdx.x & 63;
#pragma unroll
  for (int j = 0; j < KM; j++) pos[j] = 0;
  if (g.n_points == 0 || k <= 0) return 0;
  if (k > KM) k = KM;
  const int32_t cx = grid_cell_coord(q.x, g.ox, g.inv_h), cy = grid_cell_coord(q.y, g.oy, g.inv_h), cz = grid_cell_coord(q.z, g.oz, g.inv_h);
  const int32_t out = grid_outside_distance(g, cx, cy, cz);
  if (max_dist > 0.0 && out >= 1 && (double)(out - 1) * g.h >= max_dist) return 0;
  int32_t W = 0x7FFFFFFF;
  if (max_dist > 0.0) {
    const double wf = ceil(max_dist * g.inv_h) + 1.0 + (double)out;
    if (wf < 1.0e6) W = (int32_t)wf;
  }
  if (W > kCoopMaxShell) {
    const int32_t span = (g.nx > g.ny ? (g.nx > g.nz ? g.nx : g.nz) : (g.ny > g.nz ? g.ny : g.nz)) + out;
    if (span > kCoopMaxShell) return -2;
    W = span;
  }
  const double r2 = knn_radius_bound(max_dist);
  double bound = r2;
  KnnKeys<KM> c;
  knn_init(c, k, g.n_points);
  bool done = false;
  double kth = knn_key_empty();
  bool fresh = false;
  for (int32_t w = 1; w <= W && !done; w++) {
    const int ring_rows = w == 1 ? 9 : 8 * w;
    const int inner_rows = w == 1 ? 0 : (2 * w - 1) * (2 * w - 1);
    const int pieces = ring_rows + 2 * inner_rows;
    for (int u0 = 0; u0 < pieces; u0 += 64) {
      uint32_t rb = 0, re = 0;
      double s2 = kDblMax;
      {
        const int u = u0 + lane;
        int32_t dy = 0, dz = 0, xlo = cx - w, xhi = cx + w;
        bool cap = false;
        if (w == 1) {
          constexpr int kOrder[9] = {4, 1, 3, 5, 7, 0, 2, 6, 8};
          const int j = kOrder[u < 9 ? u : 0];
          dy = j % 3 - 1, dz = j / 3 - 1;
        } else if (u < ring_rows) {
          const int side = 2 * w + 1, inner = 2 * w - 1;
          if (u < side) dy = u - w, dz = -w;
          else if (u < 2 * side) dy = u - side - w, dz = w;
          else if (u < 2 * side + inner) dy = -w, dz = u - 2 * side - (w - 1);
          else dy = w, dz = u - 2 * side - inner - (w - 1);
        } else {
          const int v = u - ring_rows, ri = v >> 1, inner = 2 * w - 1;
          dy = ri % inner - (w - 1), dz = ri / inner - (w - 1);
          xlo = xhi = (v & 1) ? cx + w : cx - w;
          cap = true;
        }
        const int32_t iy = cy + dy, iz = cz + dz;
        if (u < pieces && iy >= 0 && iy <= g.ny - 1 && iz >= 0 && iz <= g.nz - 1) {
          const double sy = dy == 0 ? 0.0 : slab_dist(q.y, g.oy, g.h, iy), sz = dz == 0 ? 0.0 : slab_dist(q.z, g.oz, g.h, iz);
          double pmin2 = sy * sy + sz * sz;
          if (cap) {
            const double sx = slab_dist(q.x, g.ox, g.h, xlo);
            pmin2 += sx * sx;
          }
          if (pmin2 <= bound) {
            if (!cap) {
              if (xlo < 0) xlo = 0;
              if (xhi > g.nx - 1) xhi = g.nx - 1;
              if (bound < kDblMax) {
                const double reach = sqrt(bound - pmin2) + 1e-9 * g.h;
                const int32_t xl = grid_cell_coord(q.x - reach, g.ox, g.inv_h), xh = grid_cell_coord(q.x + reach, g.ox, g.inv_h);
                if (xl > xlo) xlo = xl;
                if (xh < xhi) xhi = xh;
              }
            }
            if (xlo <= xhi && xlo >= 0 && xhi <= g.nx - 1) {
              const uint32_t row = (uint32_t)((iz * g.ny + iy) * g.nx);
              rb = cell_start_at(cell_start, row + (uint32_t)xlo);
              re = cell_start_at(cell_start, row + (uint32_t)xhi + 1u);
              s2 = pmin2;
            }
          }
        }
      }
      unsigned long long rows = __ballot(rb < re);
      while (rows) {
        const int b = __ffsll(rows) - 1;
        rows &= rows - 1;
        const uint32_t begin = (uint32_t)__builtin_amdgcn_readlane((int)rb, b), end = (uint32_t)__builtin_amdgcn_readlane((int)re, b);
        const double rs2 = __hiloint2double(__builtin_amdgcn_readlane(__double2hiint(s2), b), __builtin_amdgcn_readlane(__double2loint(s2), b));
        if (rs2 > bound) continue;
        fresh = true;
        for (uint32_t p0 = begin; p0 < end; p0 += 64) {
          const uint32_t p = p0 + (uint32_t)lane;
          const bool real = p < end;
          const GridPoint t = sp[real ? p : begin];
          const double dx = q.x - t.x, dy = q.y - t.y, dz = q.z - t.z;
          const double d2 = dx * dx + dy * dy + dz * dz;
          knn_key_insert(c, knn_key_pack(d2, p, c.mask, real));
        }
        if (end - begin >= 256u) {
          const double wb = wave_min_all(knn_bound(c, k));
          bound = wb < bound ? wb : bound;
        }
      }
    }
    {
      if (fresh) {
      fresh = false;
      KnnKeys<KM> cc = c;
      kth = knn_key_empty();
      for (int t = 0; t < k; t++) {
        double head = knn_key_empty();
#pragma unroll
        for (int j = KM; j >= 0; j--)
          if (j >= KM - k) head = cc.key[j] < head ? cc.key[j] : head;
        const double best = wave_min_all(head);
        kth = best;
        if (head == best && best < knn_key_empty()) {
#pragma unroll
          for (int j = 0; j < KM; j++)
            if (j >= KM - k) cc.key[j] = cc.key[j + 1];
          cc.key[KM] = knn_key_empty();
        }
      }
      }
      KnnKeys<KM> probe;
      probe.mask = c.mask;
#pragma unroll
      for (int j = 0; j <= KM; j++) probe.key[j] = kth;
      if (kth < knn_key_empty()) {
        const double ub = knn_bound(probe, k);
        bound = ub < bound ? ub : bound;
      }
      done = knn_done(g, q, k, max_dist, cx, cy, cz, probe, w);
    }
  }
  if (!done) return -1;
  KnnKeys<KM> m;
  knn_init(m, k, g.n_points);
#pragma unroll
  for (int t = 0; t <= KM; t++) {
    if (t >= KM - k) {
      double head = knn_key_empty();
#pragma unroll
      for (int j = KM; j >= 0; j--)
        if (j >= KM - k) head = c.key[j] < head ? c.key[j] : head;
      const double best = wave_min_all(head);
      m.key[t] = best;
      if (head == best && best < knn_key_empty()) {
#pragma unroll
        for (int j = 0; j < KM; j++)
          if (j >= KM - k) c.key[j] = c.key[j + 1];
        c.key[KM] = knn_key_empty();
      }
    }
  }
  return knn_keys_finish(m, k, pass_max, pos);
}

static_assert(kRestThreads == 64, "associate_knn_coop_kernel is written for one wavefront per workgroup");
template <bool PLANE, int KM>
__global__ __launch_bounds__(kRestThreads, LOAMX_COOP_WAVES) void associate_knn_coop_kernel(RegBatch B, RegConfig C, uint32_t blocks_per_pair) {
  size_t pair;
  uint32_t chunk0;
  if (!xcd_pair_map(blockIdx.x, blocks_per_pair, B.n_pairs, pair, chunk0)) return;
  const PairState& S = B.state[pair];
  if (!S.active) return;
  const uint32_t listed = B.assoc.n_assoc[8 * pair + (PLANE ? 5 : 4)];
  if (listed == 0u) return;
  __shared__ uint32_t s_rows[kLeanRowWords];
  const size_t stride = PLANE ? B.planar_stride : B.edge_stride;
  const size_t field = B.n_pairs * stride;
  uint32_t* __restrict__ rnn = PLANE ? B.assoc.rnn_plane : B.assoc.rnn_edge;
  const uint32_t* __restrict__ rest = (PLANE ? B.assoc.rest_plane : B.assoc.rest_edge) + pair * stride;
  const uint32_t* __restrict__ left = (PLANE ? B.assoc.exact_plane : B.assoc.exact_edge) + pair * stride;
  const GridSet& gs = PLANE ? B.grid_plane : B.grid_edge;
  const GridSet& src_gs = PLANE ? B.src_grid_plane : B.src_grid_edge;
  const GridDesc g = gs.desc[pair];
  const uint32_t* __restrict__ cs = gs.cell_start + pair * (size_t)(kGridCellsCap + 1);
  const GridPoint* __restrict__ sp = gs.sorted + pair * gs.stride;
  const int kq = PLANE ? C.k_plane : C.k_edge;
  const double max_dist = PLANE ? C.r_plane : C.r_edge, pass_max = PLANE ? C.pass_plane : C.pass_edge;
  for (uint32_t t = chunk0; t < listed; t += blocks_per_pair) {
    const uint32_t qpos = left[t], i = rest[qpos] & kQueueIndex;
    const size_t slot = pair * stride + qpos;
    const GridPoint sq = src_gs.sorted[pair * src_gs.stride + i];
    const Vec3 p = pose_act(S.est, v3(sq.x, sq.y, sq.z));
    uint32_t pos[KM];
    int kept = knn_coop_search<KM>(g, cs, sp, p, kq, max_dist, pass_max, pos);
    if (kept == -2) {
      if ((threadIdx.x & 63) == 0) kept = knn_search_keyed<KM>(g, cs, sp, p, kq, max_dist, pass_max, pos, s_rows, 1);
      kept = __builtin_amdgcn_readfirstlane(kept);
#pragma unroll
      for (int j = 0; j < KM; j++) pos[j] = (uint32_t)__builtin_amdgcn_readfirstlane((int)pos[j]);
    }
    if ((threadIdx.x & 63) == 0) {
      rnn[slot] = (uint32_t)kept;
#pragma unroll
      for (int j = 0; j < KM; j++) rnn[(1 + j) * field + slot] = pos[j];
    }
  }
}

template <bool PLANE, int KM>
__device__ __forceinline__ void knn_exact_one(const RegBatch& B, const RegConfig& C, const PairState& S, size_t pair, uint32_t i,
                                              size_t slot, uint32_t* rnn, uint32_t* s_rows, int rows_stride) {
  const size_t stride = PLANE ? B.planar_stride : B.edge_stride;
  const size_t field = B.n_pairs * stride;
  const GridSet& gs = PLANE ? B.grid_plane : B.grid_edge;
  const GridSet& src_gs = PLANE ? B.src_grid_plane : B.src_grid_edge;
  const GridDesc g = gs.desc[pair];
  const uint32_t* __restrict__ cs = gs.cell_start + pair * (size_t)(kGridCellsCap + 1);
  const GridPoint* __restrict__ sp = gs.sorted + pair * gs.stride;
  int k = PLANE ? C.k_plane : C.k_edge;
  k = k < KM ? k : KM;
  const GridPoint sq = src_gs.sorted[pair * src_gs.stride + i];
  const Vec3 p = pose_act(S.est, v3(sq.x, sq.y, sq.z));
  KnnResult<KM> r;
  const int kept = knn_search(g, cs, sp, p, k, PLANE ? C.r_plane : C.r_edge, r, s_rows, rows_stride);
  uint32_t pos[KM];
  knn_shift_positions<KM>(r.pos, k, pos);
  rnn[slot] = (uint32_t)kept;
#pragma unroll
  for (int j = 0; j < KM; j++) rnn[(size_t)(1 + j) * field + slot] = pos[j];
}

template <bool PLANE, int KM, bool QUEUED = false>
__device__ __forceinline__ bool fit_one(const RegBatch& B, const RegConfig& C, const PairState& S, size_t pair, uint32_t i,
                                        const uint32_t* __restrict__ nnsrc, size_t nidx) {
  const size_t stride = PLANE ? B.planar_stride : B.edge_stride;
  const GridSet& gs = PLANE ? B.grid_plane : B.grid_edge;
  const GridSet& src_gs = PLANE ? B.src_grid_plane : B.src_grid_edge;
  const GridPoint sq = src_gs.sorted[pair * src_gs.stride + i];
  const Vec3 p = pose_act(S.est, v3(sq.x, sq.y, sq.z));
  const GridPoint* __restrict__ sp = gs.sorted + pair * gs.stride;
  const size_t field = B.n_pairs * stride, slot = pair * stride + i;
  const int kept = (int)nnsrc[nidx];
  const int kq = PLANE ? C.k_plane : C.k_edge;
  const int shift = KM - (kq < KM ? kq : KM);
  double prim[6] = {0, 0, 0, 0, 0, 0};
  uint32_t nearest = 0xFFFFFFFFu;
  bool valid = false;
  uint32_t at[KM];
#pragma unroll
  for (int j = 0; j < KM; j++) at[j] = shift + j < KM ? nnsrc[(size_t)(1 + shift + j) * field + nidx] : 0u;
  if (!QUEUED && kept == -1) return false;
  GridPoint tp[KM];
#pragma unroll
  for (int j = 0; j < KM; j++) tp[j] = sp[at[j] < (uint32_t)gs.stride ? at[j] : 0u];
  if (kept >= (PLANE ? C.min_plane_pts : C.min_line_pts)) {
    Vec3 nb[KM];
#pragma unroll
    for (int j = 0; j < KM; j++) nb[j] = j < kept ? v3(tp[j].x, tp[j].y, tp[j].z) : v3(0, 0, 0);
    if (kept > 0) nearest = tp[0].orig;
    if (PLANE) {
      Vec3 nrm;
      double d;
      const double avg = fit_plane<KM>(nb, kept, nrm, d);
      valid = !(avg > C.max_avg_plane_dist);
      prim[0] = nrm.x, prim[1] = nrm.y, prim[2] = nrm.z, prim[3] = d;
    } else {
      Vec3 a, b;
      fit_line<KM>(nb, kept, a, b);
      valid = !(kDblMax < C.min_line_cond);
      prim[0] = a.x, prim[1] = a.y, prim[2] = a.z, prim[3] = b.x, prim[4] = b.y, prim[5] = b.z;
    }
  }
  double* __restrict__ rec = PLANE ? B.assoc.plane : B.assoc.edge;
  rec[slot] = valid ? p.x : __longlong_as_double(0x7FF8000000000000ll);
  rec[field + slot] = p.y;
  rec[2 * field + slot] = p.z;
#pragma unroll
  for (int f = 0; f < (PLANE ? 4 : 6); f++) rec[(3 + f) * field + slot] = prim[f];
  if (B.want_nearest) (PLANE ? B.assoc.nearest_plane : B.assoc.nearest_edge)[pair * stride + sq.orig] = valid ? nearest : 0xFFFFFFFFu;
  return valid;
}

#ifndef LOAMX_FIT_WAVES
#define LOAMX_FIT_WAVES 4
#endif
template <bool PLANE, int KM>
__device__ __forceinline__ void fit_body(const RegBatch& B, const RegConfig& C, uint32_t blocks_per_pair, uint32_t block) {
  size_t pair;
  uint32_t chunk;
  if (!xcd_pair_map(block, blocks_per_pair, B.n_pairs, pair, chunk)) return;
  const uint32_t i = chunk * kAssocThreads + threadIdx.x;
  const PairState& S = B.state[pair];
  if (!S.active) return;
  const size_t stride = PLANE ? B.planar_stride : B.edge_stride;
  const uint32_t n_src = PLANE ? B.n_src_planar[pair * B.in_pitch] : B.n_src_edge[pair * B.in_pitch];
  const uint32_t* __restrict__ nn = PLANE ? B.assoc.nn_plane : B.assoc.nn_edge;
  bool valid = false;
  if (i < n_src && i < stride) valid = fit_one<PLANE, KM>(B, C, S, pair, i, nn, pair * stride + i);
  const unsigned long long m = __ballot(valid);
  if ((threadIdx.x & 63) == 0 && m) atomicAdd(&B.assoc.n_assoc[8 * pair + (PLANE ? 1 : 0)], (uint32_t)__popcll(m));
}
template <bool PLANE, int KM>
__global__ __launch_bounds__(kAssocThreads, LOAMX_FIT_WAVES) void associate_fit_kernel(RegBatch B, RegConfig C,
                                                                                        uint32_t blocks_per_pair) {
  fit_body<PLANE, KM>(B, C, blocks_per_pair, blockIdx.x);
}
template <int KME, int KMP>
__global__ __launch_bounds__(kAssocThreads, LOAMX_FIT_WAVES) void associate_fit_mixed_kernel(RegBatch B, RegConfig C, uint32_t blocks_edge,
                                                                                              uint32_t blocks_plane, uint32_t edge_blocks) {
  if (blockIdx.x < edge_blocks) fit_body<false, KME>(B, C, blocks_edge, blockIdx.x);
  else fit_body<true, KMP>(B, C, blocks_plane, blockIdx.x - edge_blocks);
}

template <bool PLANE, int KM>
__global__ __launch_bounds__(kRestThreads, 3) void associate_fit_queued_kernel(RegBatch B, RegConfig C, uint32_t blocks_per_pair) {
  size_t pair;
  uint32_t chunk0;
  if (!xcd_pair_map(blockIdx.x, blocks_per_pair, B.n_pairs, pair, chunk0)) return;
  const PairState& S = B.state[pair];
  if (!S.active) return;
  const uint32_t queued = B.assoc.n_assoc[8 * pair + (PLANE ? 3 : 2)];
  if (queued == 0u) return;
  __shared__ uint32_t s_rows[18 * kRestThreads];
  const size_t stride = PLANE ? B.planar_stride : B.edge_stride;
  uint32_t* rnn = PLANE ? B.assoc.rnn_plane : B.assoc.rnn_edge;
  const uint32_t* __restrict__ rest = (PLANE ? B.assoc.rest_plane : B.assoc.rest_edge) + pair * stride;
  uint32_t count = 0;
  for (uint32_t t = chunk0 * kRestThreads + threadIdx.x; t < queued; t += blocks_per_pair * kRestThreads) {
    const uint32_t i = rest[t] & kQueueIndex;
    if ((int)rnn[pair * stride + t] < 0)
      knn_exact_one<PLANE, KM>(B, C, S, pair, i, pair * stride + t, rnn, s_rows + threadIdx.x, kRestThreads);
    count += fit_one<PLANE, KM, true>(B, C, S, pair, i, rnn, pair * stride + t) ? 1u : 0u;
  }
#pragma unroll
  for (int off = 32; off >= 1; off >>= 1) count += __shfl_xor(count, off);
  if ((threadIdx.x & 63) == 0 && count) atomicAdd(&B.assoc.n_assoc[8 * pair + (PLANE ? 1 : 0)], count);
}

__global__ __launch_bounds__(64) void lm_begin_kernel(RegBatch B, RegConfig C) {
  const size_t pair = (size_t)blockIdx.x * blockDim.x + threadIdx.x;
  if (pair >= B.n_pairs) return;
  if (pair == 0) *B.n_active = 0u;
  PairState& S = B.state[pair];
  if (!S.active) return;
  const uint32_t iteration = S.iterations;
  const uint32_t ne = B.assoc.n_assoc[8 * pair], np = B.assoc.n_assoc[8 * pair + 1];
  for (int c = 0; c < 6; c++) B.assoc.n_assoc[8 * pair + c] = 0;
  if ((uint64_t)ne + np < C.min_associations) {
    S.termination = LOAMX_INSUFFICIENT_ASSOCIATIONS;
    S.active = 0;
    S.lm.active = 0;
    return;
  }
  lm_init(S.lm);
  S.first_sweep = 1;
  S.mom_ref_on = 0;
  if (B.iter_info) {
    loamx_iter_info& I = B.iter_info[pair * C.max_iterations + iteration];
    for (int i = 0; i < 7; i++) I.target_T_source_init[i] = S.est[i];
    I.n_edge_associations = ne;
    I.n_plane_associations = np;
  }
}

#ifndef LOAMX_SWEEP_WAVES
#define LOAMX_SWEEP_WAVES 3
#endif
__global__ __launch_bounds__(kSweepThreads, LOAMX_SWEEP_WAVES) void sweep_kernel(RegBatch B) {
  __shared__ double s_part[kSweepThreads / 64][kAccSize];
  const size_t pair = blockIdx.x / B.blocks_per_pair;
  const uint32_t blk = blockIdx.x % B.blocks_per_pair;
  const PairState& S = B.state[pair];
  if (!S.active || !S.lm.active) return;
  double x[7];
#pragma unroll
  for (int i = 0; i < 7; i++) x[i] = S.lm.xeval[i];
  const uint32_t n_se_raw = B.n_src_edge[pair * B.in_pitch], n_sp_raw = B.n_src_planar[pair * B.in_pitch];
  const uint32_t n_se = n_se_raw < B.edge_stride ? n_se_raw : (uint32_t)B.edge_stride;
  const uint32_t n_sp = n_sp_raw < B.planar_stride ? n_sp_raw : (uint32_t)B.planar_stride;
  const size_t efield = B.n_pairs * B.edge_stride, pfield = B.n_pairs * B.planar_stride;
  const double* __restrict__ E = B.assoc.edge + pair * B.edge_stride;
  const double* __restrict__ Pl = B.assoc.plane + pair * B.planar_stride;
  double acc[kAccSize];
#pragma unroll
  for (int j = 0; j < kAccSize; j++) acc[j] = 0.0;
  if (S.stream_planes == 0u) return;
  const uint32_t total = n_se + n_sp;
  const uint32_t base = blk * kSweepChunk;
  if (base >= total) return;
  if (blk == 0 && threadIdx.x == 0 && B.sweep_slots) {
    atomicAdd(&B.sweep_slots[0], (unsigned long long)n_se);
    atomicAdd(&B.sweep_slots[1], (unsigned long long)n_sp);
  }
  {
  struct Rec {
    double f[9];
    int kind;
  };
  auto load_rec = [&](uint32_t v) {
    Rec R;
    R.kind = 0;
#pragma unroll
    for (int f = 0; f < 9; f++) R.f[f] = 0.0;
    if (v < total) {
      if (v < n_se) {
        R.kind = 1;
#pragma unroll
        for (int f = 0; f < 9; f++) R.f[f] = E[f * efield + v];
      } else {
        const uint32_t q = v - n_se;
        R.kind = 2;
#pragma unroll
        for (int f = 0; f < 7; f++) R.f[f] = Pl[f * pfield + q];
      }
    }
    return R;
  };
  Rec cur = load_rec(base + threadIdx.x);
#pragma unroll 1
  for (int it = 0; it < kSweepItems; it++) {
    const Rec nxt = (it + 1 < kSweepItems) ? load_rec(base + (it + 1) * kSweepThreads + threadIdx.x) : Rec{{0, 0, 0, 0, 0, 0, 0, 0, 0}, 0};
    if (cur.kind != 0 && cur.f[0] == cur.f[0]) {
      double prim[6];
#pragma unroll
      for (int f = 0; f < 6; f++) prim[f] = cur.f[3 + f];
      residual_accumulate(cur.kind == 2, v3(cur.f[0], cur.f[1], cur.f[2]), prim, x, acc);
    }
    cur = nxt;
  }
  }
#pragma unroll
  for (int j = 0; j < kAccSize; j++) {
    double v = acc[j];
#pragma unroll
    for (int off = 32; off >= 1; off >>= 1) v += __shfl_down(v, off);
    acc[j] = v;
  }
  const int lane = threadIdx.x & 63, wave = threadIdx.x >> 6;
  if (lane == 0) {
#pragma unroll
    for (int j = 0; j < kAccSize; j++) s_part[wave][j] = acc[j];
  }
  __syncthreads();
  if (threadIdx.x < kAccSize) {
    double v = s_part[0][threadIdx.x];
    for (int w = 1; w < kSweepThreads / 64; w++) v += s_part[w][threadIdx.x];
    B.partials[(pair * B.blocks_per_pair + blk) * kAccSize + threadIdx.x] = v;
  }
}

struct LightLds {
  double T[kMomDim][7], Z[kMomDim][7];
};
__device__ __forceinline__ void wave_lds_fence() { __builtin_amdgcn_fence(__ATOMIC_ACQ_REL, "wavefront"); __builtin_amdgcn_wave_barrier(); }
constexpr uint32_t kEdgeCache = 320;
constexpr uint32_t kListCache = 64;
constexpr uint32_t kFlatCache = 192;
__device__ __forceinline__ double light_eval(const RegBatch& B, size_t pair, const double x[7], uint32_t n_se, uint32_t n_sp,
                                             const double* mom, LightLds& L, const double (*s_edge)[kEdgeCache], const uint32_t* s_listed,
                                             const double (*s_frec)[kFlatCache], uint32_t n_flat) {
  const int lane = threadIdx.x;
  const size_t efield = B.n_pairs * B.edge_stride, pfield = B.n_pairs * B.planar_stride;
  const double* __restrict__ E = B.assoc.edge + pair * B.edge_stride;
  const double* __restrict__ Pl = B.assoc.plane + pair * B.planar_stride;
  double acc[kAccSize];
#pragma unroll
  for (int j = 0; j < kAccSize; j++) acc[j] = 0.0;
  for (uint32_t v = lane; v < n_se; v += 64) {
    const bool cached = v < kEdgeCache;
    const double f0 = cached ? s_edge[0][v] : E[v];
    if (f0 == f0) {
      double prim[6];
#pragma unroll
      for (int f = 0; f < 6; f++) prim[f] = cached ? s_edge[3 + f][v] : E[(3 + f) * efield + v];
      residual_accumulate(false, v3(f0, cached ? s_edge[1][v] : E[efield + v], cached ? s_edge[2][v] : E[2 * efield + v]), prim, x, acc);
    }
  }
  if (n_flat != 0xFFFFFFFFu) {
    for (uint32_t e = lane; e < n_flat; e += 64) {
      const double prim[6] = {s_frec[3][e], s_frec[4][e], s_frec[5][e], s_frec[6][e], 0.0, 0.0};
      residual_accumulate(true, v3(s_frec[0][e], s_frec[1][e], s_frec[2][e]), prim, x, acc);
    }
  } else {
    uint32_t off = 0;
    for (uint32_t lb = 0; lb < B.mom_blocks_per_pair * 4 && (lb / 4) * kSweepChunk < n_sp; lb++) {
      const uint32_t cnt = lb < kListCache ? s_listed[lb] : B.flagged_count[pair * B.mom_blocks_per_pair * 4 + lb];
      if (cnt == 0u) continue;
      const uint32_t* __restrict__ fl = B.flagged_list + (pair * B.mom_blocks_per_pair * 4 + lb) * (size_t)(kSweepChunk / 4);
      for (uint32_t k = ((uint32_t)lane + 64u - (off & 63u)) & 63u; k < cnt; k += 64) {
        const uint32_t q = fl[k];
        const double prim[6] = {Pl[3 * pfield + q], Pl[4 * pfield + q], Pl[5 * pfield + q], Pl[6 * pfield + q], 0.0, 0.0};
        residual_accumulate(true, v3(Pl[q], Pl[pfield + q], Pl[2 * pfield + q]), prim, x, acc);
      }
      off += cnt;
    }
  }
#pragma unroll
  for (int j = 0; j < kAccSize; j++) {
    double v = acc[j];
#pragma unroll
    for (int off = 32; off >= 1; off >>= 1) v += __shfl_xor(v, off);
    acc[j] = v;
  }
  wave_lds_fence();
  for (int idx = lane; idx < kMomDim * 7; idx += 64) {
    const int j = idx / 7, a = idx % 7;
    const double ux = x[0], uy = x[1], uz = x[2], w = x[3];
    double val;
    if (a == 6) {
      const double phi[kMomDim] = {1.0, 2.0 * w * ux, 2.0 * w * uy, 2.0 * w * uz, ux * ux, uy * uy, uz * uz,
                                   ux * uy, ux * uz, uy * uz, x[4], x[5], x[6]};
      val = 0.0;
#pragma unroll
      for (int jj = 0; jj < kMomDim; jj++)
        if (jj == j) val = phi[jj];
    } else {
      double A[kMomDim][4];
#pragma unroll
      for (int jj = 0; jj < kMomDim; jj++) A[jj][0] = A[jj][1] = A[jj][2] = A[jj][3] = 0.0;
      A[1][0] = 2.0 * w, A[1][3] = 2.0 * ux;
      A[2][1] = 2.0 * w, A[2][3] = 2.0 * uy;
      A[3][2] = 2.0 * w, A[3][3] = 2.0 * uz;
      A[4][0] = 2.0 * ux, A[5][1] = 2.0 * uy, A[6][2] = 2.0 * uz;
      A[7][0] = uy, A[7][1] = ux;
      A[8][0] = uz, A[8][2] = ux;
      A[9][1] = uz, A[9][2] = uy;
      double g[4] = {0, 0, 0, 0};
#pragma unroll
      for (int jj = 0; jj < kMomDim; jj++)
        if (jj == j) g[0] = A[jj][0], g[1] = A[jj][1], g[2] = A[jj][2], g[3] = A[jj][3];
      const double W = x[0], X = x[1], Y = x[2], Zq = x[3];
      const double z0 = g[0] * (-X) + g[1] * W + g[2] * (-Zq) + g[3] * Y;
      const double z1 = g[0] * (-Y) + g[1] * Zq + g[2] * W + g[3] * (-X);
      const double z2 = g[0] * (-Zq) + g[1] * (-Y) + g[2] * X + g[3] * W;
      val = a == 0 ? z0 : (a == 1 ? z1 : (a == 2 ? z2 : ((j == 10 + (a - 3)) ? 1.0 : 0.0)));
    }
    L.Z[j][a] = val;
  }
  wave_lds_fence();
  for (int idx = lane; idx < kMomDim * 7; idx += 64) {
    const int i = idx / 7, a = idx % 7;
    double t = 0.0;
#pragma unroll
    for (int j = 0; j < kMomDim; j++) t += mom[i * kMomStride + j] * L.Z[j][a];
    L.T[i][a] = t;
  }
  wave_lds_fence();
  double v = 0.0;
  if (lane < kAccSize) {
    const int o = lane;
    v = 0.0;
#pragma unroll
    for (int j = 0; j < kAccSize; j++)
      if (j == o) v = acc[j];
    if (o < 21) {
      int a = 0, rem = o;
      while (rem >= 6 - a) rem -= 6 - a, a++;
      const int b = a + rem;
      double sum = 0.0;
#pragma unroll
      for (int i = 0; i < kMomDim; i++) sum += L.Z[i][a] * L.T[i][b];
      v += sum;
    } else if (o < 27) {
      const int a = o - 21;
      double sum = 0.0;
#pragma unroll
      for (int i = 0; i < kMomDim; i++) sum += L.Z[i][a] * L.T[i][6];
      v += sum;
    } else {
      double cost = 0.0;
#pragma unroll
      for (int i = 0; i < kMomDim; i++) cost += L.Z[i][6] * L.T[i][6];
      if (o == 27) v += 0.5 * cost;
      else if (!(cost - cost == 0.0)) v += 1.0;
    }
  }
  return v;
}

__device__ __forceinline__ double stream_eval_wave(const RegBatch& B, size_t pair, const double x[7], uint32_t n_se, uint32_t n_sp) {
  const int lane = threadIdx.x;
  const size_t efield = B.n_pairs * B.edge_stride, pfield = B.n_pairs * B.planar_stride;
  const double* __restrict__ E = B.assoc.edge + pair * B.edge_stride;
  const double* __restrict__ Pl = B.assoc.plane + pair * B.planar_stride;
  double acc[kAccSize];
#pragma unroll
  for (int j = 0; j < kAccSize; j++) acc[j] = 0.0;
  for (uint32_t v = lane; v < n_se; v += 64) {
    const double f0 = E[v];
    if (f0 == f0) {
      double prim[6];
#pragma unroll
      for (int f = 0; f < 6; f++) prim[f] = E[(3 + f) * efield + v];
      residual_accumulate(false, v3(f0, E[efield + v], E[2 * efield + v]), prim, x, acc);
    }
  }
  for (uint32_t q = lane; q < n_sp; q += 64) {
    const double f0 = Pl[q];
    if (f0 == f0) {
      const double prim[6] = {Pl[3 * pfield + q], Pl[4 * pfield + q], Pl[5 * pfield + q], Pl[6 * pfield + q], 0.0, 0.0};
      residual_accumulate(true, v3(f0, Pl[pfield + q], Pl[2 * pfield + q]), prim, x, acc);
    }
  }
  double mine = 0.0;
#pragma unroll
  for (int j = 0; j < kAccSize; j++) {
    double v = acc[j];
#pragma unroll
    for (int off = 32; off >= 1; off >>= 1) v += __shfl_xor(v, off);
    if (lane == j) mine = v;
  }
  return mine;
}

__device__ __forceinline__ void lm_step_pair(const RegBatch& B, size_t pair, PairState& S, const double* acc) {
  const double* __restrict__ mom = B.moments + pair * (size_t)(kMomSize + 2);
  LmState lm = S.lm;
  const bool first = S.first_sweep != 0;
  lm_consume(lm, acc, first);
  S.lm = lm;
  S.first_sweep = 0;
  if (first && B.ref_moments && !S.use_moments && lm.active) {
    S.use_moments = 1u, S.mom_ref_on = 1u;
    for (int i = 0; i < 7; i++) S.mom_ref[i] = lm.xeval[i];
    S.stream_planes = 1u;
    return;
  }
  const bool valid = S.mom_ref_on ? plane_moments_valid_rel(mom[kMomSize], mom[kMomSize + 1], lm.xeval, S.mom_ref)
                                  : plane_moments_valid_at(mom[kMomSize], mom[kMomSize + 1], lm.xeval);
  S.stream_planes = (!S.use_moments || (lm.active && !valid)) ? 1u : 0u;
}

__global__ __launch_bounds__(64) void lm_step_kernel(RegBatch B) {
  const size_t pair = (size_t)blockIdx.x * blockDim.x + threadIdx.x;
  if (pair >= B.n_pairs) return;
  PairState& S = B.state[pair];
  if (!S.active || !S.lm.active) return;
  const uint32_t n_se_raw = B.n_src_edge[pair * B.in_pitch], n_sp_raw = B.n_src_planar[pair * B.in_pitch];
  const uint32_t n_se = n_se_raw < B.edge_stride ? n_se_raw : (uint32_t)B.edge_stride;
  const uint32_t n_sp = n_sp_raw < B.planar_stride ? n_sp_raw : (uint32_t)B.planar_stride;
  const uint32_t used = S.stream_planes ? (n_se + n_sp + kSweepChunk - 1) / kSweepChunk : 1u;
  double acc[kAccSize];
  for (int j = 0; j < kAccSize; j++) acc[j] = 0.0;
  for (uint32_t b = 0; b < used && b < B.blocks_per_pair; b++) {
    const double* __restrict__ p = B.partials + (pair * B.blocks_per_pair + b) * kAccSize;
    for (int j = 0; j < kAccSize; j++) acc[j] += p[j];
  }
  lm_step_pair(B, pair, S, acc);
}

__device__ __forceinline__ void outer_update_pair(const RegBatch& B, const RegConfig& C, size_t pair, PairState& S) {
  const uint32_t iteration = S.iterations;
  double upd[7];
  for (int i = 0; i < 7; i++) upd[i] = S.lm.x_user[i];
  if (B.iter_info) {
    loamx_iter_info& I = B.iter_info[pair * C.max_iterations + iteration];
    for (int i = 0; i < 7; i++) I.estimate_update[i] = upd[i];
  }
  S.iterations = iteration + 1;
  double est[7];
  for (int i = 0; i < 7; i++) est[i] = S.est[i];
  const bool converged = outer_update(est, upd, C.rot_thresh, C.pos_thresh);
  S.use_moments = (C.flags & kRegFlagNoMoments) ? 0u : 1u;
  for (int i = 0; i < 7; i++) S.est[i] = est[i];
  if (converged) {
    S.termination = LOAMX_CONVERGED;
    S.active = 0;
  } else if (iteration + 1 >= C.max_iterations) {
    S.active = 0;
  } else {
    atomicAdd(B.n_active, 1u);
  }
}

__global__ __launch_bounds__(64) void lm_pair_loop_kernel(RegBatch B, RegConfig C) {
  __shared__ LightLds L;
  __shared__ double s_mom[kMomSize + 2];
  __shared__ double s_acc[kAccSize];
  __shared__ double s_edge[9][kEdgeCache];
  __shared__ double s_frec[7][kFlatCache];
  __shared__ uint32_t s_listed[kListCache], s_pref[kListCache];
  const int lane = threadIdx.x;
  const size_t pair = blockIdx.x;
  PairState& S_global = B.state[pair];
  if (!S_global.active) return;
  if (!S_global.lm.active) {
    if (lane == 0) outer_update_pair(B, C, pair, S_global);
    return;
  }
  __shared__ PairState s_S;
  static_assert(sizeof(PairState) % 8 == 0, "copied as 64-bit words");
  {
    const unsigned long long* __restrict__ src = reinterpret_cast<const unsigned long long*>(&S_global);
    unsigned long long* dst = reinterpret_cast<unsigned long long*>(&s_S);
    for (int w = lane; w < (int)(sizeof(PairState) / 8); w += 64) dst[w] = src[w];
  }
  wave_lds_fence();
  PairState& S = s_S;
  const uint32_t n_se_raw = B.n_src_edge[pair * B.in_pitch], n_sp_raw = B.n_src_planar[pair * B.in_pitch];
  const uint32_t n_se = n_se_raw < B.edge_stride ? n_se_raw : (uint32_t)B.edge_stride;
  const uint32_t n_sp = n_sp_raw < B.planar_stride ? n_sp_raw : (uint32_t)B.planar_stride;
  {
    const size_t efield = B.n_pairs * B.edge_stride;
    const double* __restrict__ E = B.assoc.edge + pair * B.edge_stride;
    const uint32_t nc = n_se < kEdgeCache ? n_se : kEdgeCache;
    for (uint32_t v = lane; v < nc; v += 64) {
#pragma unroll
      for (int f = 0; f < 9; f++) s_edge[f][v] = E[f * efield + v];
    }
    static_assert(kListCache == 64, "one lane per tile");
    s_listed[lane] = (uint32_t)lane < B.mom_blocks_per_pair * 4 ? B.flagged_count[pair * B.mom_blocks_per_pair * 4 + lane] : 0u;
  }
  uint32_t stream = 1u;
  if (S.use_moments) {
    uint32_t used = (n_sp + kSweepChunk - 1) / kSweepChunk;
    used = used < B.mom_blocks_per_pair ? used : B.mom_blocks_per_pair;
    const double* __restrict__ part = B.mom_partials + pair * B.mom_blocks_per_pair * 4 * (size_t)(kMomSize + 2);
    double* __restrict__ mom = B.moments + pair * (size_t)(kMomSize + 2);
    double v[kMomSize / 64];
#pragma unroll
    for (int c = 0; c < kMomSize / 64; c++) v[c] = 0.0;
    double s0max = 0.0, v2max = 0.0;
    constexpr uint32_t kTileBatch = 4;
    for (uint32_t t0 = 0; t0 < used * 4; t0 += kTileBatch) {
      double w[kTileBatch][kMomSize / 64], m0[kTileBatch], m1[kTileBatch];
#pragma unroll
      for (uint32_t b = 0; b < kTileBatch; b++) {
        const bool in = t0 + b < used * 4;
        const size_t off = (in ? t0 + b : t0) * (size_t)(kMomSize + 2);
#pragma unroll
        for (int c = 0; c < kMomSize / 64; c++) w[b][c] = in ? part[off + c * 64 + lane] : 0.0;
        m0[b] = in ? part[off + kMomSize] : 0.0, m1[b] = in ? part[off + kMomSize + 1] : 0.0;
      }
#pragma unroll
      for (uint32_t b = 0; b < kTileBatch; b++) {
#pragma unroll
        for (int c = 0; c < kMomSize / 64; c++) v[c] += w[b][c];
        s0max = fmax(s0max, m0[b]), v2max = fmax(v2max, m1[b]);
      }
    }
#pragma unroll
    for (int c = 0; c < kMomSize / 64; c++) mom[c * 64 + lane] = v[c], s_mom[c * 64 + lane] = v[c];
    if (lane == 0) mom[kMomSize] = s0max, mom[kMomSize + 1] = v2max, s_mom[kMomSize] = s0max, s_mom[kMomSize + 1] = v2max;
    const double ident[7] = {0, 0, 0, 1, 0, 0, 0};
    stream = (S.mom_ref_on ? plane_moments_valid_rel(s0max, v2max, S.lm.xeval, S.mom_ref) : plane_moments_valid_at(s0max, v2max, ident)) ? 0u : 1u;
  }
  if (lane == 0) S.stream_planes = stream;
  uint32_t n_flat = 0xFFFFFFFFu;
  if (S.use_moments && B.mom_blocks_per_pair * 4 <= kListCache) {
    const uint32_t tiles = B.mom_blocks_per_pair * 4;
    const uint32_t mine = ((uint32_t)lane < tiles && ((uint32_t)lane / 4) * kSweepChunk < n_sp) ? s_listed[lane] : 0u;
    uint32_t incl = mine;
#pragma unroll
    for (int off = 1; off < 64; off <<= 1) {
      const uint32_t t = __shfl_up(incl, off);
      if (lane >= off) incl += t;
    }
    const uint32_t total = (uint32_t)__builtin_amdgcn_readlane((int)incl, 63);
    if (total <= kFlatCache) {
      s_pref[lane] = incl - mine;
      wave_lds_fence();
      const size_t pfield = B.n_pairs * B.planar_stride;
      const double* __restrict__ Pl = B.assoc.plane + pair * B.planar_stride;
      for (uint32_t e = lane; e < total; e += 64) {
        uint32_t lb = 0;
        for (uint32_t t = 1; t < tiles; t++) lb = s_pref[t] <= e ? t : lb;
        const uint32_t k = e - s_pref[lb];
        const uint32_t q = B.flagged_list[(pair * B.mom_blocks_per_pair * 4 + lb) * (size_t)(kSweepChunk / 4) + k];
#pragma unroll
        for (int f = 0; f < 7; f++) s_frec[f][e] = Pl[f * pfield + q];
      }
      n_flat = total;
    }
  }
  uint32_t lm_active = 1u;
  double x[7];
#pragma unroll
  for (int i = 0; i < 7; i++) x[i] = S.lm.xeval[i];
  wave_lds_fence();
  for (int k = 0; k < 5 && lm_active; k++) {
    const double v = stream ? stream_eval_wave(B, pair, x, n_se, n_sp) : light_eval(B, pair, x, n_se, n_sp, s_mom, L, s_edge, s_listed, s_frec, n_flat);
    if (lane < kAccSize) s_acc[lane] = 0.0 + v;
    wave_lds_fence();
    if (lane == 0) {
      double acc[kAccSize];
      for (int j = 0; j < kAccSize; j++) acc[j] = s_acc[j];
      lm_step_pair(B, pair, S, acc);
    }
    wave_lds_fence();
    __builtin_amdgcn_fence(__ATOMIC_ACQ_REL, "workgroup");
    lm_active = __builtin_amdgcn_readfirstlane((int)(lane == 0 ? S.lm.active : 0u));
    stream = __builtin_amdgcn_readfirstlane((int)(lane == 0 ? S.stream_planes : 0u));
#pragma unroll
    for (int i = 0; i < 7; i++) {
      const double xi = lane == 0 ? S.lm.xeval[i] : 0.0;
      x[i] = __longlong_as_double(((long long)__builtin_amdgcn_readfirstlane((int)(__double_as_longlong(xi) >> 32)) << 32) |
                                  (unsigned int)__builtin_amdgcn_readfirstlane((int)(__double_as_longlong(xi) & 0xFFFFFFFFll)));
    }
  }
  if (lane == 0) outer_update_pair(B, C, pair, S);
  wave_lds_fence();
  {
    const unsigned long long* src = reinterpret_cast<const unsigned long long*>(&s_S);
    unsigned long long* __restrict__ dst = reinterpret_cast<unsigned long long*>(&S_global);
    for (int w = lane; w < (int)(sizeof(PairState) / 8); w += 64) dst[w] = src[w];
  }
}

typedef double v4f64 __attribute__((ext_vector_type(4)));
constexpr int kMomLdsRow = 65;

__global__ __launch_bounds__(64) void moment_kernel(RegBatch B) {
  __shared__ double s_c[kMomStride][kMomLdsRow];
  const int wave = (int)(blockIdx.x & 3u), lane = (int)threadIdx.x;
  const int tix = wave * 64 + lane;
  const size_t pair = (blockIdx.x >> 2) / B.mom_blocks_per_pair;
  const uint32_t blk = (blockIdx.x >> 2) % B.mom_blocks_per_pair;
  const PairState& S = B.state[pair];
  if (!S.active || !S.lm.active || !S.use_moments) return;
  const uint32_t n_sp_raw = B.n_src_planar[pair * B.in_pitch];
  const uint32_t n_sp = n_sp_raw < B.planar_stride ? n_sp_raw : (uint32_t)B.planar_stride;
  const uint32_t base = blk * kSweepChunk;
  if (base >= n_sp) return;
  if (blk == 0 && tix == 0 && B.sweep_slots) atomicAdd(&B.sweep_slots[4], (unsigned long long)n_sp);
  const size_t pfield = B.n_pairs * B.planar_stride;
  const double* __restrict__ Pl = B.assoc.plane + pair * B.planar_stride;
  double(*tile)[kMomLdsRow] = s_c;
#pragma unroll
  for (int j = kMomDim; j < kMomStride; j++) tile[j][lane] = 0.0;
  v4f64 acc = {0.0, 0.0, 0.0, 0.0};
  double s0max = 0.0, v2max = 0.0;
  const bool ref_on = S.mom_ref_on != 0u;
  double phi_ref[kMomDim];
  {
    double xr[7];
#pragma unroll
    for (int i = 0; i < 7; i++) xr[i] = ref_on ? S.mom_ref[i] : (i == 3 ? 1.0 : 0.0);
    plane_phi(xr, phi_ref);
  }
  uint32_t* __restrict__ flist = B.flagged_list + ((pair * B.mom_blocks_per_pair + blk) * 4 + wave) * (size_t)(kSweepChunk / 4);
  uint32_t n_flagged = 0;
  struct Rec {
    double f[7];
    bool in;
  };
  auto load_rec = [&](uint32_t q) {
    Rec R;
    R.in = q < n_sp;
#pragma unroll
    for (int f = 0; f < 7; f++) R.f[f] = R.in ? Pl[f * pfield + q] : 0.0;
    return R;
  };
  constexpr int kIters = kSweepChunk / kSweepThreads;
  Rec cur = load_rec(base + tix);
#pragma unroll 1
  for (int it = 0; it < kIters; it++) {
    const Rec nxt = (it + 1 < kIters) ? load_rec(base + (it + 1) * kSweepThreads + tix) : Rec{{0, 0, 0, 0, 0, 0, 0}, false};
    double c[kMomDim];
#pragma unroll
    for (int j = 0; j < kMomDim; j++) c[j] = 0.0;
    bool flagged = false;
    if (cur.in && cur.f[0] == cur.f[0]) {
      const Vec3 v = v3(cur.f[0], cur.f[1], cur.f[2]);
      plane_coeffs(v, v3(cur.f[3], cur.f[4], cur.f[5]), cur.f[6], c);
      double sref = c[0];
      if (ref_on) {
        sref = 0.0;
#pragma unroll
        for (int j = 0; j < kMomDim; j++) sref += c[j] * phi_ref[j];
      }
      const double a0 = fabs(sref), vv = vdot(v, v);
      flagged = !(a0 <= kMomInlier);
      if (flagged) {
#pragma unroll
        for (int j = 0; j < kMomDim; j++) c[j] = 0.0;
      } else {
        s0max = a0 > s0max ? a0 : s0max;
        v2max = vv > v2max ? vv : v2max;
      }
    }
    const unsigned long long fm = __ballot(flagged);
    if (flagged) flist[n_flagged + (uint32_t)__popcll(fm & ((1ull << lane) - 1ull))] = base + it * kSweepThreads + tix;
    n_flagged += (uint32_t)__popcll(fm);
    __builtin_amdgcn_fence(__ATOMIC_RELEASE, "wavefront");
    __builtin_amdgcn_wave_barrier();
#pragma unroll
    for (int j = 0; j < kMomDim; j++) tile[j][lane] = c[j];
    __builtin_amdgcn_fence(__ATOMIC_RELEASE, "wavefront");
    __builtin_amdgcn_wave_barrier();
    __builtin_amdgcn_fence(__ATOMIC_ACQUIRE, "wavefront");
#pragma unroll
    for (int t = 0; t < 16; t++) {
      const double a = tile[lane & 15][4 * t + (lane >> 4)];
      acc = __builtin_amdgcn_mfma_f64_16x16x4f64(a, a, acc, 0, 0, 0);
    }
    cur = nxt;
  }
  double* __restrict__ out = B.mom_partials + ((pair * B.mom_blocks_per_pair + blk) * 4 + wave) * (size_t)(kMomSize + 2);
#pragma unroll
  for (int r = 0; r < 4; r++) out[((lane >> 4) + 4 * r) * kMomStride + (lane & 15)] = acc[r];
  s0max = wave_max(s0max), v2max = wave_max(v2max);
  if (lane == 0) out[kMomSize] = s0max, out[kMomSize + 1] = v2max;
  if (lane == 0) B.flagged_count[(pair * B.mom_blocks_per_pair + blk) * 4 + wave] = n_flagged;
}

__global__ void outer_update_kernel(RegBatch B, RegConfig C) {
  const size_t pair = (size_t)blockIdx.x * blockDim.x + threadIdx.x;
  if (pair >= B.n_pairs) return;
  PairState& S = B.state[pair];
  if (!S.active) return;
  outer_update_pair(B, C, pair, S);
}

__global__ void write_results_kernel(RegBatch B, loamx_reg_result* __restrict__ out) {
  const size_t pair = (size_t)blockIdx.x * blockDim.x + threadIdx.x;
  if (pair >= B.n_pairs) return;
  if (pair == 0 && B.max_counts) {
    for (int c = 0; c < 4; c++) B.max_counts[c] = 0u;
    B.max_counts[4] = B.max_counts[5] = 0xFFFFFFFFu;
  }
  const PairState& S = B.state[pair];
  for (int i = 0; i < 7; i++) out[pair].pose[i] = S.est[i];
  out[pair].termination = S.termination;
  out[pair].iterations = S.iterations;
}

inline unsigned per_pair_grid(size_t n_pairs) { return (unsigned)((n_pairs + 63) / 64); }

template <bool PLANE, int KM>
__global__ __launch_bounds__(64) void fit_sets_kernel(const double* __restrict__ pts, size_t n_sets, int k, double* __restrict__ prim_out,
                                                      double* __restrict__ aux_out) {
  const size_t s = (size_t)blockIdx.x * 64 + threadIdx.x;
  if (s >= n_sets) return;
  Vec3 nb[KM];
#pragma unroll
  for (int j = 0; j < KM; j++) {
    const size_t at = (s * (size_t)k + (size_t)(j < k ? j : 0)) * 3;
    nb[j] = j < k ? v3(pts[at], pts[at + 1], pts[at + 2]) : v3(0, 0, 0);
  }
  if (PLANE) {
    Vec3 nrm;
    double d;
    aux_out[s] = fit_plane<KM>(nb, k, nrm, d);
    prim_out[4 * s] = nrm.x, prim_out[4 * s + 1] = nrm.y, prim_out[4 * s + 2] = nrm.z, prim_out[4 * s + 3] = d;
  } else {
    Vec3 a, b;
    fit_line<KM>(nb, k, a, b);
    aux_out[s] = kDblMax;
    prim_out[6 * s] = a.x, prim_out[6 * s + 1] = a.y, prim_out[6 * s + 2] = a.z;
    prim_out[6 * s + 3] = b.x, prim_out[6 * s + 4] = b.y, prim_out[6 * s + 5] = b.z;
  }
}

template <int KM>
__global__ __launch_bounds__(64) void knn_queries_kernel(GridSet gs, const double* __restrict__ q, size_t n_q, int k, double max_dist,
                                                         double pass_max, uint32_t* __restrict__ idx_out, uint32_t* __restrict__ count_out) {
  __shared__ uint32_t s_rows[kLeanRowWords * 64];
  const size_t i = (size_t)blockIdx.x * 64 + threadIdx.x;
  if (i >= n_q) return;
  const GridDesc g = gs.desc[0];
  uint32_t pos[KM];
  const int kk = k < KM ? k : KM;
  const Vec3 p = v3(q[3 * i], q[3 * i + 1], q[3 * i + 2]);
  int kept;
  if (g.n_points <= kBruteMax) {
    KnnResult<KM> r;
    knn_init(r);
    brute_scan_tile(r, kk, p, gs.sorted, 0u, g.n_points);
    kept = knn_finish(r, kk, max_dist);
    knn_shift_positions<KM>(r.pos, kk, pos);
  } else {
    kept = knn_search_positions<KM>(g, gs.cell_start, gs.sorted, p, kk, max_dist, pass_max, pos, s_rows + threadIdx.x, 64);
  }
  count_out[i] = (uint32_t)kept;
#pragma unroll
  for (int u = 0; u < KM; u++) {
    const int j = u - (KM - kk);
    if (j >= 0) idx_out[i * (size_t)k + j] = j < kept ? gs.sorted[pos[u]].orig : 0xFFFFFFFFu;
  }
  for (int j = KM; j < k; j++) idx_out[i * (size_t)k + j] = 0xFFFFFFFFu;
}

template <bool PLANE, int KM>
__global__ __launch_bounds__(256) void assoc_dump_kernel(RegBatch B, RegConfig C, AssocDumpSet D) {
  const size_t stride = PLANE ? B.planar_stride : B.edge_stride;
  const uint32_t n_raw = PLANE ? B.n_src_planar[0] : B.n_src_edge[0];
  const uint32_t n_src = n_raw < stride ? n_raw : (uint32_t)stride;
  const uint32_t queued = B.assoc.n_assoc[PLANE ? 3 : 2];
  const uint32_t t = blockIdx.x * 256 + threadIdx.x;
  if (t >= n_src + queued) return;
  const GridSet& gs = PLANE ? B.grid_plane : B.grid_edge;
  const GridSet& src_gs = PLANE ? B.src_grid_plane : B.src_grid_edge;
  const uint32_t* __restrict__ nn = PLANE ? B.assoc.nn_plane : B.assoc.nn_edge;
  const uint32_t* __restrict__ rnn = PLANE ? B.assoc.rnn_plane : B.assoc.rnn_edge;
  const uint32_t* __restrict__ rest = PLANE ? B.assoc.rest_plane : B.assoc.rest_edge;
  uint32_t i, at;
  const uint32_t* __restrict__ src;
  if (t < n_src) {
    i = t, at = t, src = nn;
    if (nn[t] == 0xFFFFFFFFu) return;
  } else {
    at = t - n_src, i = rest[at] & kQueueIndex, src = rnn;
  }
  const uint32_t orig = src_gs.sorted[i].orig;
  const int kq = PLANE ? C.k_plane : C.k_edge, kk = kq < KM ? kq : KM, shift = KM - kk;
  const uint32_t kept = src[at];
  D.nn_count[orig] = kept;
  for (int j = 0; j < kk; j++) {
    const uint32_t pos = src[(size_t)(1 + shift + j) * stride + at];
    D.nn_idx[(size_t)orig * (size_t)kq + j] = (uint32_t)j < kept && pos < gs.stride ? gs.sorted[pos].orig : 0xFFFFFFFFu;
  }
  const double* __restrict__ rec = PLANE ? B.assoc.plane : B.assoc.edge;
  const double f0 = rec[i];
  D.valid[orig] = f0 == f0 ? 1 : 0;
  const GridPoint sq = src_gs.sorted[i];
  const Vec3 p = pose_act(B.state[0].est, v3(sq.x, sq.y, sq.z));
  D.moved[3 * (size_t)orig] = p.x, D.moved[3 * (size_t)orig + 1] = rec[stride + i], D.moved[3 * (size_t)orig + 2] = rec[2 * stride + i];
  for (int f = 0; f < (PLANE ? 4 : 6); f++) D.prim[(size_t)orig * (PLANE ? 4 : 6) + f] = rec[(size_t)(3 + f) * stride + i];
}

}

void launch_fit_sets(bool plane, const double* d_pts, size_t n_sets, int k, double* d_prim, double* d_aux, hipStream_t s) {
  if (n_sets == 0) return;
  const dim3 grid((unsigned)((n_sets + 63) / 64));
  if (k <= 5) {
    if (plane) launch_kernel((fit_sets_kernel<true, 5>), grid, dim3(64), 0, s, d_pts, n_sets, k, d_prim, d_aux);
    else launch_kernel((fit_sets_kernel<false, 5>), grid, dim3(64), 0, s, d_pts, n_sets, k, d_prim, d_aux);
  } else if (k <= 8) {
    if (plane) launch_kernel((fit_sets_kernel<true, 8>), grid, dim3(64), 0, s, d_pts, n_sets, k, d_prim, d_aux);
    else launch_kernel((fit_sets_kernel<false, 8>), grid, dim3(64), 0, s, d_pts, n_sets, k, d_prim, d_aux);
  } else {
    if (plane) launch_kernel((fit_sets_kernel<true, kFitMaxK>), grid, dim3(64), 0, s, d_pts, n_sets, k, d_prim, d_aux);
    else launch_kernel((fit_sets_kernel<false, kFitMaxK>), grid, dim3(64), 0, s, d_pts, n_sets, k, d_prim, d_aux);
  }
}

void launch_knn_queries(const GridSet& gs, const double* d_q, size_t n_q, int k, double max_dist, uint32_t* d_idx, uint32_t* d_count,
                        hipStream_t s) {
  if (n_q == 0) return;
  const dim3 grid((unsigned)((n_q + 63) / 64));
  const double pass_max = knn_radius_pass_max(max_dist);
  if (k <= 5) launch_kernel((knn_queries_kernel<5>), grid, dim3(64), 0, s, gs, d_q, n_q, k, max_dist, pass_max, d_idx, d_count);
  else if (k <= 8) launch_kernel((knn_queries_kernel<8>), grid, dim3(64), 0, s, gs, d_q, n_q, k, max_dist, pass_max, d_idx, d_count);
  else launch_kernel((knn_queries_kernel<16>), grid, dim3(64), 0, s, gs, d_q, n_q, k, max_dist, pass_max, d_idx, d_count);
}

void launch_assoc_dump(const RegBatch& B, const RegConfig& C, const AssocDumpSet& edge, const AssocDumpSet& plane, hipStream_t s) {
  const dim3 ge((unsigned)((2 * B.edge_stride + 255) / 256)), gp((unsigned)((2 * B.planar_stride + 255) / 256));
  if (edge.nn_count) {
    if (C.k_edge <= 5) launch_kernel((assoc_dump_kernel<false, 5>), ge, dim3(256), 0, s, B, C, edge);
    else if (C.k_edge <= 8) launch_kernel((assoc_dump_kernel<false, 8>), ge, dim3(256), 0, s, B, C, edge);
    else launch_kernel((assoc_dump_kernel<false, 16>), ge, dim3(256), 0, s, B, C, edge);
  }
  if (plane.nn_count) {
    if (C.k_plane <= 5) launch_kernel((assoc_dump_kernel<true, 5>), gp, dim3(256), 0, s, B, C, plane);
    else if (C.k_plane <= 8) launch_kernel((assoc_dump_kernel<true, 8>), gp, dim3(256), 0, s, B, C, plane);
    else launch_kernel((assoc_dump_kernel<true, 16>), gp, dim3(256), 0, s, B, C, plane);
  }
}

static bool grid_big(size_t stride, const GridPoint* scratch, uint32_t flags) {
  return !grid_small(stride, flags) && scratch != nullptr && stride * sizeof(GridPoint) >= kBigScratchBytes && !(flags & kRegFlagNoBigGrid);
}
static void launch_grid_build_big(size_t n_pairs, const double* pts, const uint32_t* n_pts, size_t stride, uint32_t in_pitch,
                                  double max_dist, const GridSet& gs, GridPoint* scratch, hipStream_t s) {
  const dim3 chunks((unsigned)((stride + kBigChunk - 1) / kBigChunk), (unsigned)n_pairs);
  launch_kernel(gridbig_init_kernel, dim3((unsigned)n_pairs), dim3(64), 0, s, scratch, stride);
  launch_kernel(gridbig_bbox_kernel, chunks, dim3(kBigThreads), 0, s, pts, n_pts, stride, in_pitch, scratch);
  launch_kernel(gridbig_choose_kernel, dim3((unsigned)((n_pairs + 63) / 64)), dim3(64), 0, s, n_pts, stride, in_pitch, max_dist, gs,
                     scratch, n_pairs);
  (void)hipMemsetAsync(gs.cell_start, 0, (gs.cells_cap ? (size_t)gs.cells_cap + 1 : n_pairs * (size_t)(kGridCellsCap + 1)) * sizeof(uint32_t), s);
  launch_kernel(gridbig_pass_kernel<false>, chunks, dim3(kBigThreads), 0, s, pts, n_pts, stride, in_pitch, gs, scratch);
  const unsigned n_tiles = (unsigned)(((gs.cells_cap ? gs.cells_cap : kGridCellsCap) + 1 + kScanTile - 1) / kScanTile);
  launch_kernel(gridbig_tile_sum_kernel, dim3(n_tiles, (unsigned)n_pairs), dim3(kScanThreads), 0, s, stride, gs, scratch);
  launch_kernel(gridbig_tile_scan_kernel, dim3((unsigned)n_pairs), dim3(kScanThreads), 0, s, stride, gs, scratch);
  launch_kernel(gridbig_scan_kernel, dim3(n_tiles, (unsigned)n_pairs), dim3(kScanThreads), 0, s, n_pts, stride, in_pitch, gs, scratch);
  launch_kernel(gridbig_pass_kernel<true>, chunks, dim3(kBigThreads), 0, s, pts, n_pts, stride, in_pitch, gs, scratch);
  if (gs.rel)
    launch_kernel(gridbig_rel_kernel, dim3((unsigned)((stride + kGridPad + kBigThreads - 1) / kBigThreads), (unsigned)n_pairs), dim3(kBigThreads), 0,
                       s, n_pts, stride, in_pitch, gs);
}

size_t index_insert_ws_bytes(size_t cells, size_t n_add) {
  return 16 + (2 * (cells + 1) + n_add + (cells + 1 + kScanTile - 1) / kScanTile) * sizeof(uint32_t);
}
void launch_index_insert_count(const GridSet& gs, size_t cells, const double* d_add, uint32_t n_add, void* ws, hipStream_t s) {
  uint32_t* flag = static_cast<uint32_t*>(ws);
  uint32_t* shift = flag + 4;
  uint32_t* cell_of = shift + 2 * (cells + 1);
  (void)hipMemsetAsync(ws, 0, 16 + (cells + 1) * sizeof(uint32_t), s);
  launch_kernel(index_insert_count_kernel, dim3((n_add + 255) / 256), dim3(256), 0, s, d_add, n_add, gs.desc, flag, shift, cell_of);
}
void launch_index_insert_merge(const GridSet& gs, size_t cells, uint32_t n_old, const double* d_add, uint32_t n_add, void* ws,
                               GridPoint* sorted2, float* rel2, hipStream_t s) {
  uint32_t* shift = static_cast<uint32_t*>(ws) + 4;
  uint32_t* cursor = shift + (cells + 1);
  uint32_t* cell_of = shift + 2 * (cells + 1);
  uint32_t* tile_sum = cell_of + n_add;
  const uint32_t n_tiles = (uint32_t)((cells + 1 + kScanTile - 1) / kScanTile);
  launch_kernel(index_insert_tile_sum_kernel, dim3(n_tiles), dim3(kScanThreads), 0, s, gs.desc, shift, tile_sum);
  launch_kernel(index_insert_tile_scan_kernel, dim3(1), dim3(kScanThreads), 0, s, tile_sum, n_tiles);
  launch_kernel(index_insert_scan_kernel, dim3(n_tiles), dim3(kScanThreads), 0, s, gs.desc, gs.cell_start, tile_sum, shift, cursor);
  if (n_old) launch_kernel(index_insert_move_kernel, dim3((n_old + 255) / 256), dim3(256), 0, s, gs.desc, n_old, gs.stride, gs.sorted, gs.rel, shift, sorted2, rel2);
  launch_kernel(index_insert_scatter_kernel, dim3((n_add + 255) / 256), dim3(256), 0, s, d_add, n_add, n_old, gs.desc, gs.stride, cell_of, cursor, sorted2, rel2);
  launch_kernel(index_insert_table_kernel, dim3((unsigned)((cells + 1 + 255) / 256)), dim3(256), 0, s, gs.desc, gs.cell_start, shift, n_old + n_add, gs.stride, rel2);
}

static void debug_ptr(const char* what, const void* p, size_t need) {
  size_t size = 0;
  hipDeviceptr_t base = nullptr;
  const hipError_t e = hipMemGetAddressRange(&base, &size, const_cast<void*>(p));
  const size_t off = e == hipSuccess ? (size_t)((const char*)p - (const char*)base) : 0;
  fprintf(stderr, "[loamx]     %-10s %p need %zu: %s, allocation %p + %zu of %zu%s\n", what, p, need, hipGetErrorString(e), base, off, size,
          (e != hipSuccess || off + need > size) ? "  <-- TOO SMALL / INVALID" : "");
}

template <bool ORDERED>
static void launch_grid_build(size_t n_pairs, const double* pts, const uint32_t* n_pts, size_t stride, uint32_t in_pitch,
                              double max_dist, const GridSet& gs, GridPoint* scratch, uint32_t flags, hipStream_t s, unsigned long long* bytes,
                              const unsigned long long* box_min = nullptr, const unsigned long long* box_max = nullptr, const uint32_t* box_bad = nullptr,
                              const uint32_t* small_if = nullptr) {
  if (g_debug_sync) {
    fprintf(stderr, "[loamx]   grid build ORDERED=%d n_pairs %zu stride %zu in_pitch %u gs.stride %zu\n", (int)ORDERED, n_pairs, stride, in_pitch, gs.stride);
    debug_ptr("pts", pts, n_pairs * in_pitch * stride * 24);
    debug_ptr("n_pts", n_pts, ((n_pairs - 1) * in_pitch + 1) * 4);
    debug_ptr("desc", gs.desc, n_pairs * sizeof(GridDesc));
    debug_ptr("cell_start", gs.cell_start, n_pairs * (size_t)(kGridCellsCap + 1) * 4);
    debug_ptr("sorted", gs.sorted, n_pairs * gs.stride * sizeof(GridPoint));
    if (gs.rel) debug_ptr("rel", gs.rel, n_pairs * 3 * gs.stride * 4);
    if (scratch) debug_ptr("scratch", scratch, n_pairs * gs.stride * sizeof(GridPoint));
  }
  if (!ORDERED && grid_big(stride, scratch, flags)) {
    launch_grid_build_big(n_pairs, pts, n_pts, stride, in_pitch, max_dist, gs, scratch, s);
    return;
  }
  if (grid_small(stride, flags))
    launch_kernel((grid_build_kernel<ORDERED, true>), dim3((unsigned)n_pairs), dim3(kBuildThreads), 0, s, pts, n_pts, stride,
                       in_pitch, max_dist, gs, scratch, bytes, box_min, box_max, box_bad, small_if);
  else
    launch_kernel((grid_build_kernel<ORDERED, false>), dim3((unsigned)n_pairs), dim3(kBuildThreads), 0, s, pts, n_pts, stride,
                       in_pitch, max_dist, gs, scratch, bytes, box_min, box_max, box_bad, small_if);
}

void launch_grid_build_target(const RegBatch& B, const RegConfig& C, bool plane, hipStream_t s) {
  if (B.n_pairs == 0) return;
  const unsigned long long* bmin = B.box_min ? B.box_min + (plane ? 3 : 0) : nullptr;
  const unsigned long long* bmax = B.box_max ? B.box_max + (plane ? 3 : 0) : nullptr;
  if (plane) launch_grid_build<false>(B.n_pairs, B.tgt_planar, B.n_tgt_planar, B.planar_stride, B.in_pitch, C.r_plane, B.grid_plane, B.sort_scratch, C.flags, s, B.grid_bytes, bmin, bmax, B.box_bad);
  else {
    launch_grid_build<false>(B.n_pairs, B.tgt_edge, B.n_tgt_edge, B.edge_stride, B.in_pitch, C.r_edge, B.grid_edge, B.sort_scratch, C.flags, s, B.grid_bytes, bmin, bmax, B.box_bad,
                             B.small_edge_sets == 1u ? B.n_tgt_edge : nullptr);
    if (B.small_edge_sets == 1u)
      launch_kernel(small_sets_build_kernel, dim3((unsigned)B.n_pairs), dim3(kSmallThreads), 0, s, B.tgt_edge, B.n_tgt_edge, B.src_edge, B.n_src_edge, B.edge_stride,
                    B.in_pitch, C.r_edge, B.grid_edge, B.src_grid_edge, B.grid_bytes, bmin, bmax, B.box_bad);
  }
}
void launch_grid_build_targets(const RegBatch& B, const RegConfig& C, hipStream_t s) {
  launch_grid_build_target(B, C, false, s);
  launch_grid_build_target(B, C, true, s);
}

void launch_grid_build_source(const RegBatch& B, const RegConfig& C, bool plane, hipStream_t s) {
  if (B.n_pairs == 0) return;
  const size_t stride = plane ? B.planar_stride : B.edge_stride;
  const uint32_t* n_src = plane ? B.n_src_planar : B.n_src_edge;
  const GridSet& gs = plane ? B.src_grid_plane : B.src_grid_edge;
  if (!plane && B.small_edge_sets == 2u) {
    launch_kernel(small_sets_build_kernel, dim3((unsigned)B.n_pairs), dim3(kSmallThreads), 0, s, static_cast<const double*>(nullptr), static_cast<const uint32_t*>(nullptr),
                  B.src_edge, B.n_src_edge, B.edge_stride, B.in_pitch, C.r_edge, B.grid_edge, B.src_grid_edge, B.grid_bytes, static_cast<const unsigned long long*>(nullptr),
                  static_cast<const unsigned long long*>(nullptr), static_cast<const uint32_t*>(nullptr));
    return;
  }
  const unsigned long long* bmin = (B.box_min && B.src_box_offset) ? B.box_min + 6 * B.src_box_offset + (plane ? 3 : 0) : nullptr;
  const unsigned long long* bmax = (B.box_max && B.src_box_offset) ? B.box_max + 6 * B.src_box_offset + (plane ? 3 : 0) : nullptr;
  launch_grid_build<true>(B.n_pairs, plane ? B.src_planar : B.src_edge, n_src, stride, B.in_pitch, plane ? C.r_plane : C.r_edge, gs,
                          B.sort_scratch_src, C.flags, s, B.grid_bytes, bmin, bmax, B.box_bad, (!plane && B.small_edge_sets == 1u) ? B.n_tgt_edge : nullptr);
  if (stride && !grid_small(stride, C.flags))
    launch_kernel(grid_rank_kernel, dim3((unsigned)((stride + kRankThreads - 1) / kRankThreads), (unsigned)B.n_pairs), dim3(kRankThreads), 0, s,
                  n_src, stride, B.in_pitch, gs, B.sort_scratch_src, (!plane && B.small_edge_sets == 1u) ? B.n_tgt_edge : nullptr);
}
void launch_grid_build_sources(const RegBatch& B, const RegConfig& C, hipStream_t s) {
  launch_grid_build_source(B, C, false, s);
  launch_grid_build_source(B, C, true, s);
}

void launch_state_init(const RegBatch& B, const RegConfig& C, hipStream_t s) {
  if (B.n_pairs == 0) return;
  launch_kernel(state_init_kernel, dim3(per_pair_grid(B.n_pairs)), dim3(64), 0, s, B, C);
}

#ifndef LOAMX_REST_BLOCKS
#define LOAMX_REST_BLOCKS 32u
#endif
constexpr size_t kQueueTwoStageMin = 16u << 20;
static bool queue_one_stage(const RegBatch& B, const RegConfig& C, bool plane) {
  if (C.flags & kRegFlagQueueTwoStage) return false;
  if (C.flags & kRegFlagQueueOneStage) return true;
  if (!(C.flags & kRegFlagNoCoopLeft)) return false;
  return B.n_pairs * (plane ? B.planar_stride : B.edge_stride) < kQueueTwoStageMin;
}
static uint32_t coop_blocks(size_t n_pairs) {
  const size_t want = 32768 / (n_pairs ? n_pairs : 1);
  return (uint32_t)(want < 32 ? 32 : (want > 4096 ? 4096 : want));
}
static uint32_t rest_blocks(size_t n_pairs, uint32_t nblk) {
  const uint32_t cover = nblk * (uint32_t)(kAssocThreads / kRestThreads);
  uint32_t want = (uint32_t)(4096 / (n_pairs ? n_pairs : 1));
  if (want < LOAMX_REST_BLOCKS) want = LOAMX_REST_BLOCKS;
  return want < cover ? want : cover;
}
void launch_associate(const RegBatch& B, const RegConfig& C, hipStream_t s, hipStream_t aux, hipStream_t aux2, hipEvent_t ev_fork,
                      hipEvent_t ev_mid, hipEvent_t ev_join, hipEvent_t ev_join2, LaunchScope* knn_scope, uint32_t what) {
  if (B.n_pairs == 0) return;
  const uint32_t be = B.assoc_blocks_edge != 0xFFFFFFFFu ? B.assoc_blocks_edge : (uint32_t)((B.edge_stride + kAssocThreads - 1) / kAssocThreads);
  const uint32_t bp = B.assoc_blocks_plane != 0xFFFFFFFFu ? B.assoc_blocks_plane : (uint32_t)((B.planar_stride + kAssocThreads - 1) / kAssocThreads);
  const size_t pair_groups = (B.n_pairs + 7) / 8;
#define LOAMX_ASSOC_A1(PL, KMV, nblk, st)                                                                         \
  do {                                                                                                            \
    const dim3 grid_((unsigned)(pair_groups * 8 * (nblk)));                                                       \
    const uint32_t mode_ = (PL) ? B.knn_mode_plane : B.knn_mode_edge;    \
    if (mode_ != 2u) {                                                                                            \
      LaunchScope* outer_ = g_launch_scope;                                                                       \
      if ((PL) && knn_scope) g_launch_scope = knn_scope;                                                          \
      launch_kernel((associate_knn_kernel<PL, KMV>), grid_, dim3(kAssocThreads), 0, (st), B, C, (nblk));     \
      g_launch_scope = outer_;                                                                                    \
    }                                                                                                             \
    if (mode_ != 1u)                                                                                              \
      launch_kernel((associate_knn_brute_kernel<PL, KMV>), grid_, dim3(kAssocThreads), 0, (st), B, C, (nblk)); \
  } while (0)
#define LOAMX_ASSOC_A2(PL, KMV, nblk, st)                                                                         \
  launch_kernel((associate_fit_kernel<PL, KMV>), dim3((unsigned)(pair_groups * 8 * (nblk))), dim3(kAssocThreads), 0, \
                     (st), B, C, (nblk))
#define LOAMX_ASSOC_B(PL, KMV, nblk, st)                                                                          \
  do {                                                                                                            \
    const uint32_t rblk_ = rest_blocks(B.n_pairs, (nblk));                                                        \
    const uint32_t one_ = queue_one_stage(B, C, (PL)) ? 1u : 0u;                                                  \
    if (one_) {                                                                                                   \
      launch_kernel((associate_knn_rest_kernel<PL, KMV, true>), dim3((unsigned)(pair_groups * 8 * rblk_)),   \
                         dim3(kRestThreads), 0, (st), B, C, rblk_);                                               \
    } else {                                                                                                      \
      launch_kernel((associate_knn_rest_kernel<PL, KMV, false>), dim3((unsigned)(pair_groups * 8 * rblk_)),  \
                         dim3(kRestThreads), 0, (st), B, C, rblk_);                                               \
      if (!queue_leftovers_coop(C, (PL))) {                                                                       \
        launch_kernel((associate_knn_left_kernel<PL, KMV>), dim3((unsigned)(pair_groups * 8 * rblk_)),       \
                           dim3(kRestThreads), 0, (st), B, C, rblk_);                                             \
      } else {                                                                                                    \
        const uint32_t cblk_ = coop_blocks(B.n_pairs);                                                            \
        launch_kernel((associate_knn_coop_kernel<PL, KMV>), dim3((unsigned)(pair_groups * 8 * cblk_)),       \
                           dim3(kRestThreads), 0, (st), B, C, cblk_);                                             \
      }                                                                                                           \
    }                                                                                                             \
    launch_kernel((associate_fit_queued_kernel<PL, KMV>), dim3((unsigned)(pair_groups * 8 * rblk_)),         \
                       dim3(kRestThreads), 0, (st), B, C, rblk_);                                                 \
  } while (0)
#define LOAMX_ASSOC_K(STEP, PL, nblk, st)                \
  do {                                                   \
    if ((PL ? C.k_plane : C.k_edge) <= 5) STEP(PL, 5, nblk, st); \
    else if ((PL ? C.k_plane : C.k_edge) <= 8) STEP(PL, 8, nblk, st); \
    else STEP(PL, 16, nblk, st);                         \
  } while (0)
  const bool edges = (what & kAssocEdges) != 0u && be != 0u, planes = (what & kAssocPlanes) != 0u && bp != 0u;
  if (edges && planes && B.knn_mode_edge == 2u && B.knn_mode_plane == 1u && C.k_edge <= 5 && C.k_plane <= 5 &&
      !(C.flags & kRegFlagNoMixedAssoc)) {
    const uint32_t edge_blocks = (uint32_t)(pair_groups * 8 * be);
    const dim3 grid((unsigned)(edge_blocks + pair_groups * 8 * bp));
    LaunchScope* outer = g_launch_scope;
    if (knn_scope) g_launch_scope = knn_scope;
    launch_kernel((associate_knn_mixed_kernel<5, 5>), grid, dim3(kAssocThreads), 0, s, B, C, be, bp, edge_blocks);
    g_launch_scope = outer;
    hipStream_t sb = aux2 ? aux2 : aux;
    const bool fork2 = sb != nullptr && hipEventRecord(ev_mid, s) == hipSuccess && hipStreamWaitEvent(sb, ev_mid, 0) == hipSuccess;
    launch_kernel((associate_fit_mixed_kernel<5, 5>), grid, dim3(kAssocThreads), 0, s, B, C, be, bp, edge_blocks);
    LOAMX_ASSOC_B(true, 5, bp, (fork2 ? sb : s));
    if (fork2 && hipEventRecord(aux2 ? ev_join2 : ev_join, sb) == hipSuccess) (void)hipStreamWaitEvent(s, aux2 ? ev_join2 : ev_join, 0);
    return;
  }
  const bool use_aux = aux != nullptr && planes;
  const bool fork = use_aux && (edges || !aux2) && hipEventRecord(ev_fork, s) == hipSuccess &&
                    hipStreamWaitEvent(aux, ev_fork, 0) == hipSuccess;
  hipStream_t sa = fork ? aux : s;
  if (edges) {
    LOAMX_ASSOC_K(LOAMX_ASSOC_A1, false, be, sa);
    LOAMX_ASSOC_K(LOAMX_ASSOC_A2, false, be, sa);
    if (B.knn_mode_edge != 2u) LOAMX_ASSOC_K(LOAMX_ASSOC_B, false, be, sa);
  }
  if (planes) {
    LOAMX_ASSOC_K(LOAMX_ASSOC_A1, true, bp, s);
    hipStream_t sb = aux2 ? aux2 : aux;
    const bool fork2 = use_aux && (aux2 || fork) && hipEventRecord(ev_mid, s) == hipSuccess && hipStreamWaitEvent(sb, ev_mid, 0) == hipSuccess;
    LOAMX_ASSOC_K(LOAMX_ASSOC_A2, true, bp, s);
    if (B.knn_mode_plane != 2u) LOAMX_ASSOC_K(LOAMX_ASSOC_B, true, bp, (fork2 ? sb : s));
    if (fork2 && aux2 && hipEventRecord(ev_join2, aux2) == hipSuccess) (void)hipStreamWaitEvent(s, ev_join2, 0);
  }
  if (fork && hipEventRecord(ev_join, aux) == hipSuccess) (void)hipStreamWaitEvent(s, ev_join, 0);
#undef LOAMX_ASSOC_A1
#undef LOAMX_ASSOC_A2
#undef LOAMX_ASSOC_B
#undef LOAMX_ASSOC_K
}

#ifdef LOAMX_NN_SAME_STATS
__global__ void nn_same_kernel(RegBatch B, uint32_t* prev, unsigned long long* stats, uint32_t it) {
  const size_t pair = blockIdx.y;
  const uint32_t i = blockIdx.x * blockDim.x + threadIdx.x;
  const uint32_t n = B.n_src_planar[pair * B.in_pitch];
  if (i >= n || i >= B.planar_stride || !B.state[pair].active) return;
  const size_t field = B.n_pairs * B.planar_stride, slot = pair * B.planar_stride + i;
  bool same = it > 0, queued = B.assoc.nn_plane[slot] == 0xFFFFFFFFu;
  for (int f = 0; f < 6; f++) {
    const uint32_t v = B.assoc.nn_plane[f * field + slot];
    if (prev[f * field + slot] != v) same = false;
    prev[f * field + slot] = v;
  }
  atomicAdd(&stats[0], 1ull);
  if (same && !queued) atomicAdd(&stats[1], 1ull);
  if (queued) atomicAdd(&stats[2], 1ull);
}
void debug_nn_same(const RegBatch& B, uint32_t it, hipStream_t s) {
  static uint32_t* prev = nullptr;
  static unsigned long long* stats = nullptr;
  const size_t words = 6 * B.n_pairs * B.planar_stride;
  if (!prev) { (void)hipMalloc(&prev, words * 4); (void)hipMalloc(&stats, 24); }
  (void)hipMemsetAsync(stats, 0, 24, s);
  launch_kernel(nn_same_kernel, dim3((unsigned)((B.planar_stride + 255) / 256), (unsigned)B.n_pairs), dim3(256), 0, s, B, prev, stats, it);
  unsigned long long h[3];
  (void)hipMemcpyAsync(h, stats, 24, hipMemcpyDeviceToHost, s);
  (void)hipStreamSynchronize(s);
  printf("nn_same it=%u: %llu active plane queries, %llu keep their list (%.1f %%), %llu queued (%.1f %%)\n", it, h[0], h[1],
         100.0 * (double)h[1] / (double)(h[0] ? h[0] : 1), h[2], 100.0 * (double)h[2] / (double)(h[0] ? h[0] : 1));
}
#endif

void launch_sweep(const RegBatch& B, hipStream_t s) {
  if (B.n_pairs == 0 || B.blocks_per_pair == 0) return;
  launch_kernel(sweep_kernel, dim3((unsigned)(B.n_pairs * B.blocks_per_pair)), dim3(kSweepThreads), 0, s, B);
}

void launch_lm_pair_loop(const RegBatch& B, const RegConfig& C, hipStream_t s) {
  if (B.n_pairs == 0) return;
  launch_kernel(lm_pair_loop_kernel, dim3((unsigned)B.n_pairs), dim3(64), 0, s, B, C);
}

void launch_moments(const RegBatch& B, hipStream_t s) {
  if (B.n_pairs == 0 || B.mom_blocks_per_pair == 0) return;
  launch_kernel(moment_kernel, dim3((unsigned)(B.n_pairs * B.mom_blocks_per_pair * 4)), dim3(64), 0, s, B);
}

void launch_lm_step(const RegBatch& B, hipStream_t s) {
  if (B.n_pairs == 0) return;
  launch_kernel(lm_step_kernel, dim3(per_pair_grid(B.n_pairs)), dim3(64), 0, s, B);
}

void launch_lm_begin(const RegBatch& B, const RegConfig& C, hipStream_t s) {
  if (B.n_pairs == 0) return;
  launch_kernel(lm_begin_kernel, dim3(per_pair_grid(B.n_pairs)), dim3(64), 0, s, B, C);
}

void launch_outer_update(const RegBatch& B, const RegConfig& C, hipStream_t s) {
  if (B.n_pairs == 0) return;
  launch_kernel(outer_update_kernel, dim3(per_pair_grid(B.n_pairs)), dim3(64), 0, s, B, C);
}

void launch_write_results(const RegBatch& B, loamx_reg_result* d_results, hipStream_t s) {
  if (B.n_pairs == 0) return;
  launch_kernel(write_results_kernel, dim3(per_pair_grid(B.n_pairs)), dim3(64), 0, s, B, d_results);
}

}
```

Before: 102,100 pairs/s.

## Pack planar kNN lists into 16-bit fields and slim planar association records

Planar kNN neighbour lists for k=5 are packed as 16-bit count and positions into three words instead of six when the target set fits the lean cap. Planar association records drop the stored moved point, keeping only four plane fields; moved source points are recomputed from a new double-precision sorted-source xyz buffer wherever the sweep, LM eval, moment and dump paths need them. This is meant to cut HBM traffic for the association buffers, at the cost of extra pose transforms in the consumers, an extra xyz write during source grid sorting, and a NaN marker that now lives in the first plane field.

New measurement: 102,400 pairs/s, median of 6. No clear change (+0.3%).

```diff
diff --git a/loam_amd/csrc/loamx_api.hip b/loam_amd/csrc/loamx_api.hip
--- a/loam_amd/csrc/loamx_api.hip
+++ b/loam_amd/csrc/loamx_api.hip
@@ -22,7 +22,7 @@
   WS_XYZ = 0, WS_CURV, WS_MASK, WS_EDGE_STAGE, WS_PLANAR_STAGE, WS_EDGE_CNT, WS_PLANAR_CNT,
   WS_EDGE_IDX, WS_PLANAR_IDX, WS_N_EDGE, WS_N_PLANAR, WS_EDGE_XYZ, WS_PLANAR_XYZ,
   WS_GRID_DESC_E, WS_GRID_DESC_P, WS_CELLS_E, WS_CELLS_P, WS_SORTED_E, WS_SORTED_P, WS_REL_E, WS_REL_P,
-  WS_SGRID_DESC_E, WS_SGRID_DESC_P, WS_SCELLS_E, WS_SCELLS_P, WS_SSORTED_E, WS_SSORTED_P, WS_SORT_SCRATCH, WS_SORT_SCRATCH_SRC, WS_ASSOC_E, WS_ASSOC_P, WS_NN_E, WS_NN_P, WS_RNN_E, WS_RNN_P, WS_NEAREST_E, WS_NEAREST_P, WS_REST_E, WS_REST_P, WS_EXACT_E, WS_EXACT_P, WS_NASSOC, WS_STATE, WS_PARTIALS, WS_MOM_PARTIALS, WS_MOMENTS, WS_FLAGGED_LIST, WS_FLAGGED_COUNT, WS_LINE_TOT, WS_EXTRACT_EVENTS, WS_BOX, WS_FINITE_FLAG,
+  WS_SGRID_DESC_E, WS_SGRID_DESC_P, WS_SCELLS_E, WS_SCELLS_P, WS_SSORTED_E, WS_SSORTED_P, WS_SXYZ_P, WS_SORT_SCRATCH, WS_SORT_SCRATCH_SRC, WS_ASSOC_E, WS_ASSOC_P, WS_NN_E, WS_NN_P, WS_RNN_E, WS_RNN_P, WS_NEAREST_E, WS_NEAREST_P, WS_REST_E, WS_REST_P, WS_EXACT_E, WS_EXACT_P, WS_NASSOC, WS_STATE, WS_PARTIALS, WS_MOM_PARTIALS, WS_MOMENTS, WS_FLAGGED_LIST, WS_FLAGGED_COUNT, WS_LINE_TOT, WS_EXTRACT_EVENTS, WS_BOX, WS_FINITE_FLAG,
   WS_COUNTERS, WS_ITERINFO, WS_STREAM_IN0, WS_STREAM_IN1, WS_STREAM_RES, WS_DUMP_E, WS_DUMP_P, WS_FIT_IN, WS_FIT_OUT, WS_SRC_E, WS_SRC_P, WS_TGT_E, WS_TGT_P, WS_FCOUNTS, WS_RESULTS, WS_INIT, WS_STREAM_INIT,
   WS_COUNT
 };
@@ -117,7 +117,7 @@
     {"NO_FUSED_COMPACT", true, kFlagNoFusedCompact}, {"NO_MIS_SELECT", true, kFlagNoMisSelect}, {"FUSED_EXTRACT", true, kFlagFusedExtract},
     {"NO_ROW_SELECT", true, kFlagNoRowSelect}, {"FUSED_ROWS", true, kFlagFusedRows}, {"NO_SPLIT_CURV", true, kFlagNoSplitCurv}, {"STAGE_ALWAYS", true, kFlagStageAlways},
     {"NO_MOMENTS", false, kRegFlagNoMoments}, {"NO_PACKED_GRID", false, kRegFlagNoPackedGrid}, {"NO_BIG_GRID", false, kRegFlagNoBigGrid},
-    {"NO_GRID_SIDE", false, kRegFlagNoGridSide}, {"DEBUG_POISON", false, kRegFlagPoison},
+    {"NO_GRID_SIDE", false, kRegFlagNoGridSide}, {"DEBUG_POISON", false, kRegFlagPoison}, {"WIDE_NN_LISTS", false, kRegFlagWideNnLists},
     {"QUEUE_TWO_STAGE", false, kRegFlagQueueTwoStage}, {"QUEUE_ONE_STAGE", false, kRegFlagQueueOneStage},
     {"NO_MIXED_ASSOC", false, kRegFlagNoMixedAssoc}, {"FORCE_RCCL", false, kRegFlagForceRccl},
     {"NO_COOP_LEFT", false, kRegFlagNoCoopLeft}, {"NO_REF_MOMENTS", false, kRegFlagNoRefMoments},
@@ -555,13 +555,16 @@
   ENSURE(ctx, WS_SCELLS_P, np * (size_t)(kGridCellsCap + 1) * sizeof(uint32_t));
   ENSURE(ctx, WS_SSORTED_E, np * es * sizeof(GridPoint));
   ENSURE(ctx, WS_SSORTED_P, np * ps * sizeof(GridPoint));
+  ENSURE(ctx, WS_SXYZ_P, np * ps * 3 * sizeof(double));
   ENSURE(ctx, WS_SORT_SCRATCH, np * (es > ps ? es : ps) * sizeof(GridPoint));
   ENSURE(ctx, WS_SORT_SCRATCH_SRC, grid_small(es > ps ? es : ps, C.flags) ? sizeof(GridPoint) : np * (es > ps ? es : ps) * sizeof(GridPoint));
   ENSURE(ctx, WS_ASSOC_E, 9 * np * es * sizeof(double));
-  ENSURE(ctx, WS_ASSOC_P, 7 * np * ps * sizeof(double));
+  ENSURE(ctx, WS_ASSOC_P, 4 * np * ps * sizeof(double));
   const size_t km_e = C.k_edge <= 5 ? 5 : (C.k_edge <= 8 ? 8 : kMaxK), km_p = C.k_plane <= 5 ? 5 : (C.k_plane <= 8 ? 8 : kMaxK);
   ENSURE(ctx, WS_NN_E, (1 + km_e) * np * es * sizeof(uint32_t));
-  ENSURE(ctx, WS_NN_P, (1 + km_p) * np * ps * sizeof(uint32_t));
+  const size_t tgt_cap_p = prebuilt ? prebuilt->cap[1] : ps;
+  B.nn_packed = (km_p == 5 && tgt_cap_p <= kLeanMaxPoints && !(C.flags & kRegFlagWideNnLists)) ? 1u : 0u;
+  ENSURE(ctx, WS_NN_P, (B.nn_packed ? 3 : 1 + km_p) * np * ps * sizeof(uint32_t));
   ENSURE(ctx, WS_RNN_E, (1 + km_e) * np * es * sizeof(uint32_t));
   ENSURE(ctx, WS_RNN_P, (1 + km_p) * np * ps * sizeof(uint32_t));
   ENSURE(ctx, WS_NEAREST_E, np * es * sizeof(uint32_t));
@@ -587,7 +590,7 @@
   }
   if (C.flags & kRegFlagPoison) {
     static const int kScratch[] = {WS_GRID_DESC_E, WS_GRID_DESC_P, WS_CELLS_E, WS_CELLS_P, WS_SORTED_E, WS_SORTED_P, WS_REL_E, WS_REL_P,
-                                   WS_SGRID_DESC_E, WS_SGRID_DESC_P, WS_SCELLS_E, WS_SCELLS_P, WS_SSORTED_E, WS_SSORTED_P, WS_SORT_SCRATCH, WS_SORT_SCRATCH_SRC,
+                                   WS_SGRID_DESC_E, WS_SGRID_DESC_P, WS_SCELLS_E, WS_SCELLS_P, WS_SSORTED_E, WS_SSORTED_P, WS_SXYZ_P, WS_SORT_SCRATCH, WS_SORT_SCRATCH_SRC,
                                    WS_ASSOC_E, WS_ASSOC_P, WS_NN_E, WS_NN_P, WS_RNN_E, WS_RNN_P, WS_NEAREST_E, WS_NEAREST_P, WS_REST_E,
                                    WS_REST_P, WS_EXACT_E, WS_EXACT_P, WS_NASSOC, WS_STATE, WS_PARTIALS, WS_MOM_PARTIALS, WS_MOMENTS,
                                    WS_FLAGGED_LIST, WS_FLAGGED_COUNT};
@@ -600,7 +603,8 @@
   B.grid_plane = GridSet{wsp<GridDesc>(ctx, WS_GRID_DESC_P), wsp<uint32_t>(ctx, WS_CELLS_P), wsp<GridPoint>(ctx, WS_SORTED_P), ps + kGridPad,
                          wsp<float>(ctx, WS_REL_P)};
   B.src_grid_edge = GridSet{wsp<GridDesc>(ctx, WS_SGRID_DESC_E), wsp<uint32_t>(ctx, WS_SCELLS_E), wsp<GridPoint>(ctx, WS_SSORTED_E), es, nullptr};
-  B.src_grid_plane = GridSet{wsp<GridDesc>(ctx, WS_SGRID_DESC_P), wsp<uint32_t>(ctx, WS_SCELLS_P), wsp<GridPoint>(ctx, WS_SSORTED_P), ps, nullptr};
+  B.src_grid_plane = GridSet{wsp<GridDesc>(ctx, WS_SGRID_DESC_P), wsp<uint32_t>(ctx, WS_SCELLS_P), wsp<GridPoint>(ctx, WS_SSORTED_P), ps, nullptr, 0u,
+                            wsp<double>(ctx, WS_SXYZ_P)};
   B.sort_scratch = wsp<GridPoint>(ctx, WS_SORT_SCRATCH);
   B.sort_scratch_src = wsp<GridPoint>(ctx, WS_SORT_SCRATCH_SRC);
   B.assoc = AssocBuffers{wsp<double>(ctx, WS_ASSOC_E), wsp<double>(ctx, WS_ASSOC_P), wsp<uint32_t>(ctx, WS_NN_E),
diff --git a/loam_amd/csrc/loamx_internal.h b/loam_amd/csrc/loamx_internal.h
--- a/loam_amd/csrc/loamx_internal.h
+++ b/loam_amd/csrc/loamx_internal.h
@@ -116,6 +116,7 @@
 constexpr uint32_t kRegFlagNoSmallSets = 8192u;
 constexpr uint32_t kRegFlagCheckFinite = 4096u;
 constexpr uint32_t kRegFlagNoExtractBoxes = 2048u;
+constexpr uint32_t kRegFlagWideNnLists = 16384u;
 constexpr uint32_t kRegFlagNoMixedAssoc = 128u;
 
 struct GridSet {
@@ -125,6 +126,7 @@
   size_t stride;
   float* rel;
   uint32_t cells_cap;
+  double* xyz = nullptr;
 };
 
 struct AssocBuffers {
@@ -198,6 +200,7 @@
   uint32_t knn_mode_edge, knn_mode_plane;
   uint32_t assoc_blocks_edge, assoc_blocks_plane;
   uint32_t want_nearest;
+  uint32_t nn_packed;
   uint32_t ref_moments;
   const unsigned long long* box_min;
   const unsigned long long* box_max;
diff --git a/loam_amd/csrc/register_kernels.hip b/loam_amd/csrc/register_kernels.hip
--- a/loam_amd/csrc/register_kernels.hip
+++ b/loam_amd/csrc/register_kernels.hip
@@ -199,6 +199,10 @@
       uint32_t rank = 0;
       for (uint32_t j = b; j < en; j++) rank += s_inv[j] < i ? 1u : 0u;
       sp[b + rank] = GridPoint{x, y, z, i, 0u};
+      if (gs.xyz) {
+        double* __restrict__ q = gs.xyz + (pair * gs.stride + b + rank) * 3;
+        q[0] = x, q[1] = y, q[2] = z;
+      }
     }
   } else if (PACKED) {
     const uint16_t* order = s_inv;
@@ -598,6 +602,10 @@
 #pragma unroll 4
   for (uint32_t j = b; j < en; j++) rank += src[j].orig < e.orig ? 1u : 0u;
   sp[b + rank] = e;
+  if (gs.xyz) {
+    double* __restrict__ q = gs.xyz + (pair * gs.stride + b + rank) * 3;
+    q[0] = e.x, q[1] = e.y, q[2] = e.z;
+  }
 }
 
 __global__ void state_init_kernel(RegBatch B, RegConfig C) {
@@ -651,6 +659,46 @@
   return pair < n_pairs;
 }
 
+template <bool PLANE, int KM>
+__device__ __forceinline__ bool nn_packed(const RegBatch& B) {
+  return PLANE && KM == 5 && B.nn_packed != 0u;
+}
+template <bool PLANE, int KM>
+__device__ __forceinline__ void nn_store(const RegBatch& B, uint32_t* __restrict__ nn, size_t field, size_t slot, uint32_t count,
+                                         const uint32_t (&pos)[KM]) {
+  if (nn_packed<PLANE, KM>(B)) {
+    nn[slot] = (count & 0xFFFFu) | (pos[0] << 16);
+    nn[field + slot] = (pos[1] & 0xFFFFu) | (pos[KM > 2 ? 2 : 0] << 16);
+    nn[2 * field + slot] = (pos[KM > 3 ? 3 : 0] & 0xFFFFu) | (pos[KM > 4 ? 4 : 0] << 16);
+    return;
+  }
+  nn[slot] = count;
+#pragma unroll
+  for (int j = 0; j < KM; j++) nn[(1 + j) * field + slot] = pos[j];
+}
+template <bool PLANE, int KM>
+__device__ __forceinline__ uint32_t nn_count(const RegBatch& B, uint32_t word0) {
+  if (!nn_packed<PLANE, KM>(B)) return word0;
+  return (word0 & 0xFFFFu) == 0xFFFFu ? 0xFFFFFFFFu : (word0 & 0xFFFFu);
+}
+template <bool PLANE, int KM>
+__device__ __forceinline__ uint32_t nn_position(const RegBatch& B, const uint32_t* __restrict__ nn, size_t field, size_t slot, int u) {
+  if (!nn_packed<PLANE, KM>(B)) return nn[(size_t)(1 + u) * field + slot];
+  const uint32_t w = nn[(size_t)((u + 1) >> 1) * field + slot];
+  return (u & 1) ? (w & 0xFFFFu) : (w >> 16);
+}
+__device__ __forceinline__ Vec3 src_planar_point(const RegBatch& B, size_t pair, uint32_t i) {
+  const double* __restrict__ q = B.src_grid_plane.xyz + (pair * B.src_grid_plane.stride + i) * 3;
+  return v3(q[0], q[1], q[2]);
+}
+template <bool PLANE>
+__device__ __forceinline__ Vec3 src_point(const RegBatch& B, size_t pair, uint32_t i) {
+  if (PLANE) return src_planar_point(B, pair, i);
+  const GridPoint* __restrict__ g = B.src_grid_edge.sorted + pair * B.src_grid_edge.stride + i;
+  return v3(g->x, g->y, g->z);
+}
+constexpr int kPlaneRecFields = 4;
+
 constexpr int kBruteTile = 256;
 constexpr size_t kBruteLdsBytes = (kBruteTile + kGridPad) * sizeof(GridPoint) + ((3 * (kBruteTile + kGridPad) * sizeof(float) + 31) / 32) * 32;
 
@@ -692,8 +740,7 @@
   const GridPoint* __restrict__ sp = gs.sorted + pair * gs.stride;
   Vec3 p = v3(0, 0, 0);
   if (has) {
-    const GridPoint sq = src_gs.sorted[pair * src_gs.stride + i];
-    p = pose_act(S.est, v3(sq.x, sq.y, sq.z));
+    p = pose_act(S.est, src_point<PLANE>(B, pair, i));
   }
   int k = PLANE ? C.k_plane : C.k_edge;
   k = k < KM ? k : KM;
@@ -797,9 +844,7 @@
   if (!has) return;
   const size_t field = B.n_pairs * stride, slot = pair * stride + i;
   uint32_t* __restrict__ nn = PLANE ? B.assoc.nn_plane : B.assoc.nn_edge;
-  nn[slot] = (uint32_t)kept;
-#pragma unroll
-  for (int j = 0; j < KM; j++) nn[(1 + j) * field + slot] = pos[j];
+  nn_store<PLANE, KM>(B, nn, field, slot, (uint32_t)kept, pos);
 }
 template <bool PLANE, int KM>
 __global__ __launch_bounds__(kAssocThreads) void associate_knn_brute_kernel(RegBatch B, RegConfig C, uint32_t blocks_per_pair) {
@@ -827,19 +872,16 @@
   const GridDesc g = gs.desc[pair];
   if (g.n_points <= kBruteMax) return;
   if (i >= n_src || i >= stride) return;
-  const GridPoint sq = src_gs.sorted[pair * src_gs.stride + i];
-  const Vec3 p = pose_act(S.est, v3(sq.x, sq.y, sq.z));
+  const Vec3 p = pose_act(S.est, src_point<PLANE>(B, pair, i));
   const uint32_t* __restrict__ cs = gs.cell_start + pair * (size_t)(kGridCellsCap + 1);
   const GridPoint* __restrict__ sp = gs.sorted + pair * gs.stride;
   uint32_t pos[KM];
   const float* __restrict__ rel = gs.rel + pair * 3 * gs.stride;
 #if LOAMX_KNN_REQUERY
-  const GridPoint* __restrict__ src_pts = src_gs.sorted + pair * src_gs.stride;
   auto requery = [&](const Vec3&) -> Vec3 {
     uint32_t ii = i;
     asm volatile("" : "+v"(ii));
-    const GridPoint s2 = src_pts[ii];
-    return pose_act(S.est, v3(s2.x, s2.y, s2.z));
+    return pose_act(S.est, src_point<PLANE>(B, pair, ii));
   };
   const int kept = knn_search_f32_round1<KM, false, decltype(requery)>(g, cs, sp, rel, (uint32_t)gs.stride, p, PLANE ? C.k_plane : C.k_edge,
                                              PLANE ? C.r_plane : C.r_edge, PLANE ? C.pass_plane : C.pass_edge, pos,
@@ -851,13 +893,11 @@
 #endif
   const size_t field = B.n_pairs * stride, slot = pair * stride + i;
   uint32_t* __restrict__ nn = PLANE ? B.assoc.nn_plane : B.assoc.nn_edge;
-  nn[slot] = kept < 0 ? 0xFFFFFFFFu : (uint32_t)kept;
   if (kept < 0) {
     const uint32_t at = atomicAdd(&B.assoc.n_assoc[8 * pair + (PLANE ? 3 : 2)], 1u);
     (PLANE ? B.assoc.rest_plane : B.assoc.rest_edge)[pair * stride + at] = i | (kept == -2 ? kQueueWide : kept == -3 ? kQueueTied : 0u);
   }
-#pragma unroll
-  for (int j = 0; j < KM; j++) nn[(1 + j) * field + slot] = pos[j];
+  nn_store<PLANE, KM>(B, nn, field, slot, kept < 0 ? 0xFFFFFFFFu : (uint32_t)kept, pos);
 }
 template <bool PLANE, int KM>
 __global__ __launch_bounds__(kAssocThreads, KM <= 5 ? LOAMX_ASSOC_WAVES5 : LOAMX_ASSOC_WAVES) void associate_knn_kernel(RegBatch B, RegConfig C,
@@ -924,8 +964,7 @@
     int kept = -1;
     const bool coop = !one_stage && queue_leftovers_coop(C, PLANE);
     if (one_stage || (!(entry & kQueueTied) && ((lean_set && !(entry & kQueueWide)) || ((entry & kQueueWide) && !coop)))) {
-      const GridPoint sq = src_gs.sorted[pair * src_gs.stride + i];
-      const Vec3 p = pose_act(S.est, v3(sq.x, sq.y, sq.z));
+      const Vec3 p = pose_act(S.est, src_point<PLANE>(B, pair, i));
       if (entry & kQueueWide)
         kept = knn_search_f32_round1<KM, true>(g, cs, sp, gs.rel + pair * 3 * gs.stride, (uint32_t)gs.stride, p, kq, max_dist, pass_max, pos,
                                                 s_rows + threadIdx.x, kRestThreads);
@@ -969,8 +1008,7 @@
   for (uint32_t t = t0; t < listed; t += dt) {
     const uint32_t qpos = left[t], i = rest[qpos] & kQueueIndex;
     const size_t slot = pair * stride + qpos;
-    const GridPoint sq = src_gs.sorted[pair * src_gs.stride + i];
-    const Vec3 p = pose_act(S.est, v3(sq.x, sq.y, sq.z));
+    const Vec3 p = pose_act(S.est, src_point<PLANE>(B, pair, i));
     uint32_t pos[KM];
     const int kept = knn_search_keyed<KM>(g, cs, sp, p, PLANE ? C.k_plane : C.k_edge, PLANE ? C.r_plane : C.r_edge,
                                           PLANE ? C.pass_plane : C.pass_edge, pos, s_rows + threadIdx.x, kRestThreads);
@@ -1176,8 +1214,7 @@
   for (uint32_t t = chunk0; t < listed; t += blocks_per_pair) {
     const uint32_t qpos = left[t], i = rest[qpos] & kQueueIndex;
     const size_t slot = pair * stride + qpos;
-    const GridPoint sq = src_gs.sorted[pair * src_gs.stride + i];
-    const Vec3 p = pose_act(S.est, v3(sq.x, sq.y, sq.z));
+    const Vec3 p = pose_act(S.est, src_point<PLANE>(B, pair, i));
     uint32_t pos[KM];
     int kept = knn_coop_search<KM>(g, cs, sp, p, kq, max_dist, pass_max, pos);
     if (kept == -2) {
@@ -1206,8 +1243,7 @@
   const GridPoint* __restrict__ sp = gs.sorted + pair * gs.stride;
   int k = PLANE ? C.k_plane : C.k_edge;
   k = k < KM ? k : KM;
-  const GridPoint sq = src_gs.sorted[pair * src_gs.stride + i];
-  const Vec3 p = pose_act(S.est, v3(sq.x, sq.y, sq.z));
+  const Vec3 p = pose_act(S.est, src_point<PLANE>(B, pair, i));
   KnnResult<KM> r;
   const int kept = knn_search(g, cs, sp, p, k, PLANE ? C.r_plane : C.r_edge, r, s_rows, rows_stride);
   uint32_t pos[KM];
@@ -1223,11 +1259,13 @@
   const size_t stride = PLANE ? B.planar_stride : B.edge_stride;
   const GridSet& gs = PLANE ? B.grid_plane : B.grid_edge;
   const GridSet& src_gs = PLANE ? B.src_grid_plane : B.src_grid_edge;
-  const GridPoint sq = src_gs.sorted[pair * src_gs.stride + i];
-  const Vec3 p = pose_act(S.est, v3(sq.x, sq.y, sq.z));
+  const GridPoint* __restrict__ sq = src_gs.sorted + pair * src_gs.stride + i;
+  const Vec3 p = pose_act(S.est, src_point<PLANE>(B, pair, i));
   const GridPoint* __restrict__ sp = gs.sorted + pair * gs.stride;
   const size_t field = B.n_pairs * stride, slot = pair * stride + i;
-  const int kept = (int)nnsrc[nidx];
+  const bool packed = !QUEUED && nn_packed<PLANE, KM>(B);
+  const uint32_t word0 = nnsrc[nidx];
+  const int kept = (int)(packed ? nn_count<PLANE, KM>(B, word0) : word0);
   const int kq = PLANE ? C.k_plane : C.k_edge;
   const int shift = KM - (kq < KM ? kq : KM);
   double prim[6] = {0, 0, 0, 0, 0, 0};
@@ -1235,7 +1273,20 @@
   bool valid = false;
   uint32_t at[KM];
 #pragma unroll
-  for (int j = 0; j < KM; j++) at[j] = shift + j < KM ? nnsrc[(size_t)(1 + shift + j) * field + nidx] : 0u;
+  for (int j = 0; j < KM; j++) at[j] = 0u;
+  if (packed) {
+    const uint32_t w1 = nnsrc[field + nidx], w2 = nnsrc[2 * field + nidx];
+    const uint32_t raw[5] = {word0 >> 16, w1 & 0xFFFFu, w1 >> 16, w2 & 0xFFFFu, w2 >> 16};
+#pragma unroll
+    for (int j = 0; j < KM; j++) {
+#pragma unroll
+      for (int u = j; u < 5; u++)
+        if (u == shift + j) at[j] = raw[u];
+    }
+  } else {
+#pragma unroll
+    for (int j = 0; j < KM; j++) at[j] = shift + j < KM ? nnsrc[(size_t)(1 + shift + j) * field + nidx] : 0u;
+  }
   if (!QUEUED && kept == -1) return false;
   GridPoint tp[KM];
 #pragma unroll
@@ -1259,12 +1310,19 @@
     }
   }
   double* __restrict__ rec = PLANE ? B.assoc.plane : B.assoc.edge;
-  rec[slot] = valid ? p.x : __longlong_as_double(0x7FF8000000000000ll);
-  rec[field + slot] = p.y;
-  rec[2 * field + slot] = p.z;
-#pragma unroll
-  for (int f = 0; f < (PLANE ? 4 : 6); f++) rec[(3 + f) * field + slot] = prim[f];
-  if (B.want_nearest) (PLANE ? B.assoc.nearest_plane : B.assoc.nearest_edge)[pair * stride + sq.orig] = valid ? nearest : 0xFFFFFFFFu;
+  if (PLANE) {
+    rec[slot] = valid ? prim[0] : __longlong_as_double(0x7FF8000000000000ll);
+#pragma unroll
+    for (int f = 1; f < kPlaneRecFields; f++) rec[f * field + slot] = prim[f];
+  } else {
+    rec[slot] = valid ? p.x : __longlong_as_double(0x7FF8000000000000ll);
+    rec[field + slot] = p.y;
+    rec[2 * field + slot] = p.z;
+#pragma unroll
+    for (int f = 0; f < 6; f++) rec[(3 + f) * field + slot] = prim[f];
+  }
+  if (B.want_nearest)
+    (PLANE ? B.assoc.nearest_plane : B.assoc.nearest_edge)[pair * stride + sq->orig] = valid ? nearest : 0xFFFFFFFFu;
   return valid;
 }
 
@@ -1397,8 +1455,10 @@
       } else {
         const uint32_t q = v - n_se;
         R.kind = 2;
-#pragma unroll
-        for (int f = 0; f < 7; f++) R.f[f] = Pl[f * pfield + q];
+        const Vec3 sp = src_planar_point(B, pair, q);
+        R.f[0] = sp.x, R.f[1] = sp.y, R.f[2] = sp.z;
+#pragma unroll
+        for (int f = 0; f < kPlaneRecFields; f++) R.f[3 + f] = Pl[f * pfield + q];
       }
     }
     return R;
@@ -1407,11 +1467,14 @@
 #pragma unroll 1
   for (int it = 0; it < kSweepItems; it++) {
     const Rec nxt = (it + 1 < kSweepItems) ? load_rec(base + (it + 1) * kSweepThreads + threadIdx.x) : Rec{{0, 0, 0, 0, 0, 0, 0, 0, 0}, 0};
-    if (cur.kind != 0 && cur.f[0] == cur.f[0]) {
+    const double mark = cur.kind == 2 ? cur.f[3] : cur.f[0];
+    if (cur.kind != 0 && mark == mark) {
       double prim[6];
 #pragma unroll
       for (int f = 0; f < 6; f++) prim[f] = cur.f[3 + f];
-      residual_accumulate(cur.kind == 2, v3(cur.f[0], cur.f[1], cur.f[2]), prim, x, acc);
+      Vec3 v = v3(cur.f[0], cur.f[1], cur.f[2]);
+      if (cur.kind == 2) v = pose_act(S.est, v);
+      residual_accumulate(cur.kind == 2, v, prim, x, acc);
     }
     cur = nxt;
   }
@@ -1443,7 +1506,7 @@
 constexpr uint32_t kEdgeCache = 320;
 constexpr uint32_t kListCache = 64;
 constexpr uint32_t kFlatCache = 192;
-__device__ __forceinline__ double light_eval(const RegBatch& B, size_t pair, const double x[7], uint32_t n_se, uint32_t n_sp,
+__device__ __forceinline__ double light_eval(const RegBatch& B, size_t pair, const double est[7], const double x[7], uint32_t n_se, uint32_t n_sp,
                                              const double* mom, LightLds& L, const double (*s_edge)[kEdgeCache], const uint32_t* s_listed,
                                              const double (*s_frec)[kFlatCache], uint32_t n_flat) {
   const int lane = threadIdx.x;
@@ -1476,8 +1539,8 @@
       const uint32_t* __restrict__ fl = B.flagged_list + (pair * B.mom_blocks_per_pair * 4 + lb) * (size_t)(kSweepChunk / 4);
       for (uint32_t k = ((uint32_t)lane + 64u - (off & 63u)) & 63u; k < cnt; k += 64) {
         const uint32_t q = fl[k];
-        const double prim[6] = {Pl[3 * pfield + q], Pl[4 * pfield + q], Pl[5 * pfield + q], Pl[6 * pfield + q], 0.0, 0.0};
-        residual_accumulate(true, v3(Pl[q], Pl[pfield + q], Pl[2 * pfield + q]), prim, x, acc);
+        const double prim[6] = {Pl[q], Pl[pfield + q], Pl[2 * pfield + q], Pl[3 * pfield + q], 0.0, 0.0};
+        residual_accumulate(true, pose_act(est, src_planar_point(B, pair, q)), prim, x, acc);
       }
       off += cnt;
     }
@@ -1565,7 +1628,7 @@
   return v;
 }
 
-__device__ __forceinline__ double stream_eval_wave(const RegBatch& B, size_t pair, const double x[7], uint32_t n_se, uint32_t n_sp) {
+__device__ __forceinline__ double stream_eval_wave(const RegBatch& B, size_t pair, const double est[7], const double x[7], uint32_t n_se, uint32_t n_sp) {
   const int lane = threadIdx.x;
   const size_t efield = B.n_pairs * B.edge_stride, pfield = B.n_pairs * B.planar_stride;
   const double* __restrict__ E = B.assoc.edge + pair * B.edge_stride;
@@ -1585,8 +1648,8 @@
   for (uint32_t q = lane; q < n_sp; q += 64) {
     const double f0 = Pl[q];
     if (f0 == f0) {
-      const double prim[6] = {Pl[3 * pfield + q], Pl[4 * pfield + q], Pl[5 * pfield + q], Pl[6 * pfield + q], 0.0, 0.0};
-      residual_accumulate(true, v3(f0, Pl[pfield + q], Pl[2 * pfield + q]), prim, x, acc);
+      const double prim[6] = {f0, Pl[pfield + q], Pl[2 * pfield + q], Pl[3 * pfield + q], 0.0, 0.0};
+      residual_accumulate(true, pose_act(est, src_planar_point(B, pair, q)), prim, x, acc);
     }
   }
   double mine = 0.0;
@@ -1754,19 +1817,21 @@
         for (uint32_t t = 1; t < tiles; t++) lb = s_pref[t] <= e ? t : lb;
         const uint32_t k = e - s_pref[lb];
         const uint32_t q = B.flagged_list[(pair * B.mom_blocks_per_pair * 4 + lb) * (size_t)(kSweepChunk / 4) + k];
-#pragma unroll
-        for (int f = 0; f < 7; f++) s_frec[f][e] = Pl[f * pfield + q];
+        const Vec3 mv = pose_act(S.est, src_planar_point(B, pair, q));
+        s_frec[0][e] = mv.x, s_frec[1][e] = mv.y, s_frec[2][e] = mv.z;
+#pragma unroll
+        for (int f = 0; f < kPlaneRecFields; f++) s_frec[3 + f][e] = Pl[f * pfield + q];
       }
       n_flat = total;
     }
   }
   uint32_t lm_active = 1u;
-  double x[7];
-#pragma unroll
-  for (int i = 0; i < 7; i++) x[i] = S.lm.xeval[i];
+  double x[7], est[7];
+#pragma unroll
+  for (int i = 0; i < 7; i++) x[i] = S.lm.xeval[i], est[i] = S.est[i];
   wave_lds_fence();
   for (int k = 0; k < 5 && lm_active; k++) {
-    const double v = stream ? stream_eval_wave(B, pair, x, n_se, n_sp) : light_eval(B, pair, x, n_se, n_sp, s_mom, L, s_edge, s_listed, s_frec, n_flat);
+    const double v = stream ? stream_eval_wave(B, pair, est, x, n_se, n_sp) : light_eval(B, pair, est, x, n_se, n_sp, s_mom, L, s_edge, s_listed, s_frec, n_flat);
     if (lane < kAccSize) s_acc[lane] = 0.0 + v;
     wave_lds_fence();
     if (lane == 0) {
@@ -1834,8 +1899,10 @@
   auto load_rec = [&](uint32_t q) {
     Rec R;
     R.in = q < n_sp;
-#pragma unroll
-    for (int f = 0; f < 7; f++) R.f[f] = R.in ? Pl[f * pfield + q] : 0.0;
+    const Vec3 sp = R.in ? src_planar_point(B, pair, q) : v3(0, 0, 0);
+    R.f[0] = sp.x, R.f[1] = sp.y, R.f[2] = sp.z;
+#pragma unroll
+    for (int f = 0; f < kPlaneRecFields; f++) R.f[3 + f] = R.in ? Pl[f * pfield + q] : 0.0;
     return R;
   };
   constexpr int kIters = kSweepChunk / kSweepThreads;
@@ -1847,8 +1914,8 @@
 #pragma unroll
     for (int j = 0; j < kMomDim; j++) c[j] = 0.0;
     bool flagged = false;
-    if (cur.in && cur.f[0] == cur.f[0]) {
-      const Vec3 v = v3(cur.f[0], cur.f[1], cur.f[2]);
+    if (cur.in && cur.f[3] == cur.f[3]) {
+      const Vec3 v = pose_act(S.est, v3(cur.f[0], cur.f[1], cur.f[2]));
       plane_coeffs(v, v3(cur.f[3], cur.f[4], cur.f[5]), cur.f[6], c);
       double sref = c[0];
       if (ref_on) {
@@ -1985,25 +2052,41 @@
   const uint32_t* __restrict__ src;
   if (t < n_src) {
     i = t, at = t, src = nn;
-    if (nn[t] == 0xFFFFFFFFu) return;
+    if (nn_count<PLANE, KM>(B, nn[t]) == 0xFFFFFFFFu) return;
   } else {
     at = t - n_src, i = rest[at] & kQueueIndex, src = rnn;
   }
   const uint32_t orig = src_gs.sorted[i].orig;
   const int kq = PLANE ? C.k_plane : C.k_edge, kk = kq < KM ? kq : KM, shift = KM - kk;
-  const uint32_t kept = src[at];
+  const bool round1 = t < n_src;
+  const uint32_t kept = round1 ? nn_count<PLANE, KM>(B, src[at]) : src[at];
   D.nn_count[orig] = kept;
   for (int j = 0; j < kk; j++) {
-    const uint32_t pos = src[(size_t)(1 + shift + j) * stride + at];
+    const uint32_t pos = round1 ? nn_position<PLANE, KM>(B, src, stride, at, shift + j) : src[(size_t)(1 + shift + j) * stride + at];
     D.nn_idx[(size_t)orig * (size_t)kq + j] = (uint32_t)j < kept && pos < gs.stride ? gs.sorted[pos].orig : 0xFFFFFFFFu;
   }
   const double* __restrict__ rec = PLANE ? B.assoc.plane : B.assoc.edge;
   const double f0 = rec[i];
   D.valid[orig] = f0 == f0 ? 1 : 0;
-  const GridPoint sq = src_gs.sorted[i];
-  const Vec3 p = pose_act(B.state[0].est, v3(sq.x, sq.y, sq.z));
-  D.moved[3 * (size_t)orig] = p.x, D.moved[3 * (size_t)orig + 1] = rec[stride + i], D.moved[3 * (size_t)orig + 2] = rec[2 * stride + i];
-  for (int f = 0; f < (PLANE ? 4 : 6); f++) D.prim[(size_t)orig * (PLANE ? 4 : 6) + f] = rec[(size_t)(3 + f) * stride + i];
+  const Vec3 p = pose_act(B.state[0].est, src_point<PLANE>(B, 0, i));
+  D.moved[3 * (size_t)orig] = p.x, D.moved[3 * (size_t)orig + 1] = PLANE ? p.y : rec[stride + i], D.moved[3 * (size_t)orig + 2] = PLANE ? p.z : rec[2 * stride + i];
+  for (int f = 0; f < (PLANE ? 4 : 6); f++) D.prim[(size_t)orig * (PLANE ? 4 : 6) + f] = rec[(size_t)(PLANE ? f : 3 + f) * stride + i];
+  if (PLANE && !(f0 == f0)) {
+    double nx = 0.0;
+    if ((int)kept >= C.min_plane_pts) {
+      Vec3 ordered[KM], nrm;
+      double d;
+      for (int j = 0; j < KM; j++) ordered[j] = v3(0, 0, 0);
+      for (int j = 0; j < kk && j < (int)kept; j++) {
+        const uint32_t pos = round1 ? nn_position<PLANE, KM>(B, src, stride, at, shift + j) : src[(size_t)(1 + shift + j) * stride + at];
+        const GridPoint tp = gs.sorted[pos < gs.stride ? pos : 0u];
+        ordered[j] = v3(tp.x, tp.y, tp.z);
+      }
+      (void)fit_plane<KM>(ordered, (int)kept, nrm, d);
+      nx = nrm.x;
+    }
+    D.prim[(size_t)orig * 4] = nx;
+  }
 }
 
 }
@@ -2294,8 +2377,8 @@
   const uint32_t n = B.n_src_planar[pair * B.in_pitch];
   if (i >= n || i >= B.planar_stride || !B.state[pair].active) return;
   const size_t field = B.n_pairs * B.planar_stride, slot = pair * B.planar_stride + i;
-  bool same = it > 0, queued = B.assoc.nn_plane[slot] == 0xFFFFFFFFu;
-  for (int f = 0; f < 6; f++) {
+  bool same = it > 0, queued = nn_count<true, 5>(B, B.assoc.nn_plane[slot]) == 0xFFFFFFFFu;
+  for (int f = 0; f < (B.nn_packed ? 3 : 6); f++) {
     const uint32_t v = B.assoc.nn_plane[f * field + slot];
     if (prev[f * field + slot] != v) same = false;
     prev[f * field + slot] = v;
```
